# pswpswpsw/nif

Hardware: AMD Instinct MI355X
Metric: train-step points/sec (1D-wave, batch=1M per GPU) (higher is better)
Workload: dtype f32

## Files before the change

### nif_amd/csrc/k_nets.hip

```cpp
#include "nif_internal.h"
#include "k_pnet_bf16.h"


__global__ void k_pack(const float* __restrict__ theta, MatRef m, int NBI, int NBO, float* __restrict__ WF,
                       float* __restrict__ WB) {
  const long per_plane = (long)NBI * NBO * 1024;
  const long total = per_plane * (m.r + 1);
  for (long idx = (long)blockIdx.x * blockDim.x + threadIdx.x; idx < total; idx += (long)gridDim.x * blockDim.x) {
    const int k = (int)(idx / per_plane);
    long rem = idx - (long)k * per_plane;
    const int c = rem & 3;
    const int lane = (rem >> 2) & 63;
    const int vq = (rem >> 8) & 3;
    const int blk = (int)(rem >> 10);
    const int v = 4 * vq + c;
    {
      const int ob = blk / NBI, ib = blk % NBI;
      const int in = 32 * ib + fmap(v, lane >> 5), out = 32 * ob + (lane & 31);
      WF[idx] = (in < m.nin && out < m.nout) ? theta[matref_index(m, k, in, out)] : 0.f;
    }
    {
      const int ib = blk / NBO, ob = blk % NBO;
      const int in = 32 * ib + (lane & 31), out = 32 * ob + fmap(v, lane >> 5);
      WB[idx] = (in < m.nin && out < m.nout) ? theta[matref_index(m, k, in, out)] : 0.f;
    }
  }
}

void launch_pack(const float* theta, const MatRef& m, int NBI, int NBO, f32x4* WF, f32x4* WB, hipStream_t st) {
  const long total = (long)NBI * NBO * 1024 * (m.r + 1);
  int grid = (int)((total + 255) / 256);
  if (grid > 2048) grid = 2048;
  hipLaunchKernelGGL(k_pack, dim3(grid), dim3(256), 0, st, theta, m, NBI, NBO, (float*)WF, (float*)WB);
}

template <int NB>
__device__ __forceinline__ void pnet_first(const PNetArgs& A, long ptc, int hf, f32x16 (&h)[NB], f32x16 (&d)[NB]) {
  const float* prow = A.xin + ptc * A.ncol + A.col0;
#pragma unroll
  for (int b = 0; b < NB; ++b)
#pragma unroll
    for (int v = 0; v < 16; ++v) {
      const int f = 32 * b + fmap(v, hf);
      float a = 0.f;
      if (f < A.nst) {
        float acc = 0.f;
        for (int dd = 0; dd < A.pi; ++dd) acc = fmaf(prow[dd], A.theta[A.first_w + (long)dd * A.nst + f], acc);
        a = A.omega * acc + A.theta[A.first_b + f];
      }
      h[b][v] = a;
    }
  act_tile<NB>(A.act, h, h, d, A.nst, hf);
}

__host__ __device__ inline int pnet_plane_floats(const PNetArgs& A, int NB) {
  const int nm = A.lst * (A.res ? 2 : 1);
  return NB == 1 ? nm * PBF_FWD_U4 * 4 : ((NB == 2 && A.pbf2) ? nm * 4 * PBF_FWD_U4 * 4 : 0);
}
__host__ __device__ inline int pnet_tail_floats(const PNetArgs& A) { return A.r + (A.ll_kind ? A.r + A.r * A.r : 0); }

template <int NB, bool TRAIN, int ACT>
__global__ __launch_bounds__(256) void k_pnet(PNetArgs A) {
  const int lane = threadIdx.x & 63, wid = threadIdx.x >> 6;
  const int p = lane & 31, hf = lane >> 5;
  const long ntiles = (A.B + 31) / 32;
  const int nm = A.lst * (A.res ? 2 : 1);
  const long plane = (long)NB * NB * 256;
  extern __shared__ __attribute__((aligned(16))) float pn_lds[];
  float* zl_lds = pn_lds;
  float* tailv = pn_lds + (A.ll_kind ? 4 * A.r * 32 : 0) + ((psmall_floats(A, NB) + 3) & ~3) + pnet_plane_floats(A, NB);
  for (int e = threadIdx.x; e < A.r; e += 256) tailv[e] = A.theta[A.bott_b + e];
  if (A.ll_kind) {
    for (int e = threadIdx.x; e < A.r; e += 256) tailv[A.r + e] = A.theta[A.last_b + e];
    for (int e = threadIdx.x; e < A.r * A.r; e += 256) tailv[2 * A.r + e] = A.theta[A.last_w + e];
  }
  const PSmall S = psmall_stage<NB>(A, pn_lds + (A.ll_kind ? 4 * A.r * 32 : 0), threadIdx.x, 256);
  pbf16x8* bpl = reinterpret_cast<pbf16x8*>(pn_lds + (A.ll_kind ? 4 * A.r * 32 : 0) + ((psmall_floats(A, NB) + 3) & ~3));
  const bool bf2 = NB == 2 && A.pbf2;
  if constexpr (NB == 1) {
    for (int m = 0; m < nm; ++m) {
      const long w_off = A.res ? ((m & 1) ? A.hid_w2[m >> 1] : A.hid_w[m >> 1]) : A.hid_w[m];
      pbf_build(bpl + m * PBF_FWD_U4, nullptr, A.theta, w_off, A.nst, threadIdx.x, 256);
    }
  } else if constexpr (NB == 2) {
    if (bf2)
      for (int m = 0; m < nm; ++m) {
        const long w_off = A.res ? ((m & 1) ? A.hid_w2[m >> 1] : A.hid_w[m >> 1]) : A.hid_w[m];
        pbfn_build_fwd<2>(bpl + m * 4 * PBF_FWD_U4, A.theta, w_off, A.nst, threadIdx.x, 256);
      }
  }
  __syncthreads();
  for (long tile = (long)blockIdx.x * 4 + wid; tile < ntiles; tile += (long)gridDim.x * 4) {
  long pt = tile * 32 + p;
  const long ptc = pt < A.B ? pt : A.B - 1;

  f32x16 h[NB], d[NB], T[NB];
  {
    const float* prow = A.xin + ptc * A.ncol + A.col0;
#pragma unroll
    for (int b = 0; b < NB; ++b) {
      f32x16 acc;
#pragma unroll
      for (int v = 0; v < 16; ++v) acc[v] = 0.f;
      for (int dd = 0; dd < A.pi; ++dd) acc += prow[dd] * psmall_get(S.fw + dd * NB * 32, b, hf);
      h[b] = A.omega * acc + psmall_get(S.fb, b, hf);
    }
    act_tile_sel<NB, ACT>(A.act, h, h, d, A.nst, hf);
  }
  if (TRAIN) stash_store<NB>(A.stash + (long)(nm + 1) * A.slot_stride, tile, d, p, hf);

  for (int i = 0; i < A.lst; ++i) {
    if (!A.res) {
      if (TRAIN) stash_store<NB>(A.stash + (long)i * A.slot_stride, tile, h, p, hf);
      if constexpr (NB == 1) pbf_dense_fwd(bpl + i * PBF_FWD_U4, h[0], T[0], lane);
      else if (NB == 2 && bf2) pbfn_dense_fwd<NB>(bpl + i * (NB * NB * PBF_FWD_U4), h, T, lane);
      else dense_mfma<NB, NB>(A.WF + (long)i * plane, h, T, lane);
#pragma unroll
      for (int b = 0; b < NB; ++b) T[b] = A.omega * T[b] + psmall_get(S.hb + i * NB * 32, b, hf);
      act_tile_sel<NB, ACT>(A.act, T, T, d, A.nst, hf);
#pragma unroll
      for (int b = 0; b < NB; ++b) h[b] = A.siren ? T[b] : h[b] + T[b];
      if (TRAIN) stash_store<NB>(A.stash + (long)(nm + 2 + i) * A.slot_stride, tile, d, p, hf);
    } else {
      f32x16 t[NB];
      if (TRAIN) stash_store<NB>(A.stash + (long)(2 * i) * A.slot_stride, tile, h, p, hf);
      if constexpr (NB == 1) pbf_dense_fwd(bpl + (2 * i) * PBF_FWD_U4, h[0], T[0], lane);
      else if (NB == 2 && bf2) pbfn_dense_fwd<NB>(bpl + (2 * i) * (NB * NB * PBF_FWD_U4), h, T, lane);
      else dense_mfma<NB, NB>(A.WF + (long)(2 * i) * plane, h, T, lane);
#pragma unroll
      for (int b = 0; b < NB; ++b) T[b] = A.omega * T[b] + psmall_get(S.hb + i * NB * 32, b, hf);
      act_tile_sel<NB, ACT>(A.act, T, t, d, A.nst, hf);
      if (TRAIN) {
        stash_store<NB>(A.stash + (long)(nm + 2 + 2 * i) * A.slot_stride, tile, d, p, hf);
        stash_store<NB>(A.stash + (long)(2 * i + 1) * A.slot_stride, tile, t, p, hf);
      }
      if constexpr (NB == 1) pbf_dense_fwd(bpl + (2 * i + 1) * PBF_FWD_U4, t[0], T[0], lane);
      else if (NB == 2 && bf2) pbfn_dense_fwd<NB>(bpl + (2 * i + 1) * (NB * NB * PBF_FWD_U4), t, T, lane);
      else dense_mfma<NB, NB>(A.WF + (long)(2 * i + 1) * plane, t, T, lane);
#pragma unroll
      for (int b = 0; b < NB; ++b) {
        const f32x16 lin = A.omega * T[b] + psmall_get(S.hb2 + i * NB * 32, b, hf);
        T[b] = A.siren ? lin : h[b] + lin;
      }
      act_tile_sel<NB, ACT>(A.act, T, T, d, A.nst, hf);
#pragma unroll
      for (int b = 0; b < NB; ++b) h[b] = A.siren ? 0.5f * (h[b] + T[b]) : T[b];
      if (TRAIN) stash_store<NB>(A.stash + (long)(nm + 2 + 2 * i + 1) * A.slot_stride, tile, d, p, hf);
    }
  }
  if (TRAIN) stash_store<NB>(A.stash + (long)nm * A.slot_stride, tile, h, p, hf);
  float* zl = zl_lds + (long)wid * A.r * 32;
  for (int c = 0; c < A.r; ++c) {
    float s = 0.f;
#pragma unroll
    for (int b = 0; b < NB; ++b) {
      const f32x16 w = psmall_get(S.bw + c * NB * 32, b, hf);
#pragma unroll
      for (int v = 0; v < 16; ++v) s = fmaf(h[b][v], w[v], s);
    }
    s += __shfl_xor(s, 32);
    s += tailv[c];
    if (A.ll_kind) {
      if (hf == 0) { zl[c * 32 + p] = s; A.ZL[(tile * A.zl_rows + c) * 32 + p] = s; }
    } else if (hf == 0) {
      A.Z[(tile * A.r + c) * 32 + p] = s;
    }
  }
  if (A.ll_kind) {
    const float* lw = tailv + 2 * A.r;
    for (int c = hf; c < A.r; c += 2) {
      float s = tailv[A.r + c];
#pragma unroll 4
      for (int kk = 0; kk < A.r; ++kk) s = fmaf(zl[kk * 32 + p], lw[kk * A.r + c], s);
      A.Z[(tile * A.r + c) * 32 + p] = s;
    }
  }
  }
}

template <int NB>
__global__ __launch_bounds__(256) void k_pnet_bwd(PNetArgs A) {
  const int lane = threadIdx.x & 63, wid = threadIdx.x >> 6;
  const int p = lane & 31, hf = lane >> 5;
  const long ntiles = (A.B + 31) / 32;
  const long tile = (long)blockIdx.x * 4 + wid;
  if (tile >= ntiles) return;
  const int nm = A.lst * (A.res ? 2 : 1);
  const long plane = (long)NB * NB * 256;

  f32x16 gh[NB], d[NB], ga[NB], U[NB];
#pragma unroll
  for (int b = 0; b < NB; ++b)
#pragma unroll
    for (int v = 0; v < 16; ++v) gh[b][v] = 0.f;
  for (int c = 0; c < A.r; ++c) {
    const float dz = A.DZ[(tile * A.r + c) * 32 + p];
#pragma unroll
    for (int b = 0; b < NB; ++b)
#pragma unroll
      for (int v = 0; v < 16; ++v) {
        const int f = 32 * b + fmap(v, hf);
        if (f < A.nst) gh[b][v] = fmaf(dz, A.theta[A.bott_w + (long)f * A.r + c], gh[b][v]);
      }
  }
  for (int i = A.lst - 1; i >= 0; --i) {
    if (!A.res) {
      float* da = A.stash + (long)(nm + 2 + i) * A.slot_stride;
      stash_load<NB>(da, tile, d, p, hf);
#pragma unroll
      for (int b = 0; b < NB; ++b) ga[b] = gh[b] * d[b];
      stash_store<NB>(da, tile, ga, p, hf);
      dense_mfma<NB, NB>(A.WB + (long)i * plane, ga, U, lane);
#pragma unroll
      for (int b = 0; b < NB; ++b) gh[b] = A.siren ? A.omega * U[b] : gh[b] + A.omega * U[b];
    } else {
      float* da2 = A.stash + (long)(nm + 2 + 2 * i + 1) * A.slot_stride;
      float* da1 = A.stash + (long)(nm + 2 + 2 * i) * A.slot_stride;
      stash_load<NB>(da2, tile, d, p, hf);
      const float half = A.siren ? 0.5f : 1.0f;
#pragma unroll
      for (int b = 0; b < NB; ++b) ga[b] = half * gh[b] * d[b];
      stash_store<NB>(da2, tile, ga, p, hf);
      dense_mfma<NB, NB>(A.WB + (long)(2 * i + 1) * plane, ga, U, lane);
      f32x16 skip[NB];
#pragma unroll
      for (int b = 0; b < NB; ++b) skip[b] = A.siren ? 0.5f * gh[b] : ga[b];
      stash_load<NB>(da1, tile, d, p, hf);
#pragma unroll
      for (int b = 0; b < NB; ++b) ga[b] = A.omega * U[b] * d[b];
      stash_store<NB>(da1, tile, ga, p, hf);
      dense_mfma<NB, NB>(A.WB + (long)(2 * i) * plane, ga, U, lane);
#pragma unroll
      for (int b = 0; b < NB; ++b) gh[b] = skip[b] + A.omega * U[b];
    }
  }
  float* da0 = A.stash + (long)(nm + 1) * A.slot_stride;
  stash_load<NB>(da0, tile, d, p, hf);
#pragma unroll
  for (int b = 0; b < NB; ++b) ga[b] = gh[b] * d[b];
  stash_store<NB>(da0, tile, ga, p, hf);
}

void launch_pnet(const PNetArgs& a_, int NSTB, bool train, hipStream_t st) {
  PNetArgs a = a_;
  const long ntiles = (a.B + 31) / 32;
  long nblk = (ntiles + 3) / 4;
  static const long cap = [] { const char* e = getenv("NIF_PNET_BLOCKS"); return e ? atol(e) : 2048L; }();
  if (nblk > cap) nblk = cap;
  const int nmat = a.lst * (a.res ? 2 : 1);
  const size_t shm0 = ((a.ll_kind ? (size_t)4 * a.r * 32 : 0) + (size_t)((psmall_floats(a, NSTB) + 3) & ~3)) * sizeof(float);
  static const bool bf2_on = [] { const char* e = getenv("NIF_PNET_BF2"); return !(e && e[0] == '0'); }();
  const size_t tailb = (size_t)pnet_tail_floats(a) * sizeof(float);
  a.pbf2 = (NSTB == 2 && bf2_on && shm0 + tailb + (size_t)nmat * 4 * PBF_FWD_U4 * 16 <= 64u * 1024u) ? 1 : 0;
  if (a.pbf2 && nblk > 512) nblk = 512;
  dim3 grid((unsigned)nblk), block(256);
  const size_t shm = shm0 + (size_t)pnet_plane_floats(a, NSTB) * sizeof(float) + tailb;
#define PNL(NB_, TR_, ACT_)                                                                                             \
  {                                                                                                                     \
    if (shm > 48 * 1024)                                                                                                \
      (void)hipFuncSetAttribute((const void*)k_pnet<NB_, TR_, ACT_>, hipFuncAttributeMaxDynamicSharedMemorySize, (int)shm); \
    hipLaunchKernelGGL((k_pnet<NB_, TR_, ACT_>), grid, block, shm, st, a);                                              \
  }
#define PNA(NB_, TR_)                              \
  if (a.act == ACT_SWISH) PNL(NB_, TR_, ACT_SWISH) \
  else if (a.act == ACT_SINE) PNL(NB_, TR_, ACT_SINE) \
  else PNL(NB_, TR_, -1)
#define PN(NB_) \
  if (train) { PNA(NB_, true) } else { PNA(NB_, false) }
  if (NSTB == 1) { PN(1) } else if (NSTB == 2) { PN(2) } else { PN(4) }
#undef PN
#undef PNA
#undef PNL
}
void launch_pnet_bwd(const PNetArgs& a, int NSTB, hipStream_t st) {
  const long ntiles = (a.B + 31) / 32;
  dim3 grid((unsigned)((ntiles + 3) / 4)), block(256);
  if (NSTB == 1) hipLaunchKernelGGL((k_pnet_bwd<1>), grid, block, 0, st, a);
  else if (NSTB == 2) hipLaunchKernelGGL((k_pnet_bwd<2>), grid, block, 0, st, a);
  else hipLaunchKernelGGL((k_pnet_bwd<4>), grid, block, 0, st, a);
}

__device__ __forceinline__ float hyp(const SNetArgs& A, int k, long slot) {
  return k < A.r ? A.theta[A.off_Wh + (long)k * A.po + slot] : A.theta[A.off_bh + slot];
}

template <int NB, bool TRAIN, int ACT>
__global__ __launch_bounds__(256, (NB <= 2 ? 2 : 1)) void k_snet(SNetArgs A) {
  extern __shared__ float smem[];
  const int lane = threadIdx.x & 63, wid = threadIdx.x >> 6;
  const int p = lane & 31, hf = lane >> 5;
  const long ntiles = (A.B + 31) / 32;
  const long tile = (long)blockIdx.x * 4 + wid;
  const bool active = tile < ntiles;
  float loss_lane = 0.f;
  float* dzs = smem + (long)wid * (2 * A.r * 64);
  float* sks = dzs + A.r * 64;
  float* lsum = smem + 4L * (2 * A.r * 64);

  if (active) {
    const long pt = tile * 32 + p;
    const bool valid = pt < A.B;
    const long ptc = valid ? pt : A.B - 1;
    const long plane = (long)NB * NB * 256;
    const int n = A.n, r = A.r;
    const float* xrow = A.xin + ptc * A.ncol + A.col0;
    const float* zt_base = A.Z + tile * r * 32 + p;
    float* IN0 = A.stash;
    float* DA0 = A.stash + (long)(A.nh + 1) * A.slot_stride;
    if (TRAIN)
      for (int k = 0; k < r; ++k) dzs[k * 64 + lane] = 0.f;

    f32x16 h[NB], d[NB], acc[NB], T[NB], ublk[NB];
#pragma unroll
    for (int b = 0; b < NB; ++b)
#pragma unroll
      for (int v = 0; v < 16; ++v) acc[b][v] = 0.f;
    for (int k = 0; k <= r; ++k) {
      const float zt = k < r ? zt_base[k * 32] : 1.0f;
#pragma unroll
      for (int b = 0; b < NB; ++b)
#pragma unroll
        for (int v = 0; v < 16; ++v) {
          const int f = 32 * b + fmap(v, hf);
          if (f < n) {
            float s = 0.f;
            for (int dd = 0; dd < A.si; ++dd) s = fmaf(xrow[dd], hyp(A, k, slot_w1(A) + (long)dd * n + f), s);
            acc[b][v] = fmaf(zt, fmaf(A.omega, s, hyp(A, k, slot_b1(A) + f)), acc[b][v]);
          }
        }
    }
    act_tile_sel<NB, ACT>(A.act, acc, h, d, n, hf);
    if (TRAIN) stash_store<NB>(DA0, tile, d, p, hf);

    for (int j = 0; j < A.nh; ++j) {
      if (TRAIN) stash_store<NB>(IN0 + (long)j * A.slot_stride, tile, h, p, hf);
#pragma unroll
      for (int b = 0; b < NB; ++b)
#pragma unroll
        for (int v = 0; v < 16; ++v) acc[b][v] = 0.f;
      for (int k = 0; k <= r; ++k) {
        const float zt = k < r ? zt_base[k * 32] : 1.0f;
        dense_mfma<NB, NB>(A.WF + ((long)j * (r + 1) + k) * plane, h, T, lane);
#pragma unroll
        for (int b = 0; b < NB; ++b)
#pragma unroll
          for (int v = 0; v < 16; ++v) {
            const int f = 32 * b + fmap(v, hf);
            const float hb = f < n ? hyp(A, k, slot_bh(A, j) + f) : 0.f;
            acc[b][v] = fmaf(zt, fmaf(A.omega, T[b][v], hb), acc[b][v]);
          }
      }
      const bool res_first = A.res && !(j & 1);
      const bool res_second = A.res && (j & 1);
      if (res_first) {
#pragma unroll
        for (int b = 0; b < NB; ++b) ublk[b] = h[b];
      }
      act_tile_sel<NB, ACT>(A.act, acc, T, d, n, hf);
#pragma unroll
      for (int b = 0; b < NB; ++b) {
        f32x16 hn = T[b];
        if (A.nif_skip) hn += h[b];
        if (res_second) hn = 0.5f * (ublk[b] + hn);
        h[b] = hn;
      }
      if (TRAIN) stash_store<NB>(DA0 + (long)(j + 1) * A.slot_stride, tile, d, p, hf);
    }

    if (TRAIN) stash_store<NB>(IN0 + (long)A.nh * A.slot_stride, tile, h, p, hf);
    f32x16 gh[NB];
#pragma unroll
    for (int b = 0; b < NB; ++b)
#pragma unroll
      for (int v = 0; v < 16; ++v) gh[b][v] = 0.f;
    const float wsamp = (valid ? (A.sw ? A.sw[ptc] : 1.0f) : 0.0f);
    float se = 0.f;
    for (int o = 0; o < A.so; ++o) {
      f32x16 wg[NB];
#pragma unroll
      for (int b = 0; b < NB; ++b)
#pragma unroll
        for (int v = 0; v < 16; ++v) wg[b][v] = 0.f;
      float part = 0.f, bias = 0.f;
      for (int k = 0; k <= r; ++k) {
        const float zt = k < r ? zt_base[k * 32] : 1.0f;
        float sk = 0.f;
#pragma unroll
        for (int b = 0; b < NB; ++b)
#pragma unroll
          for (int v = 0; v < 16; ++v) {
            const int f = 32 * b + fmap(v, hf);
            const float w = f < n ? hyp(A, k, slot_wl(A) + (long)f * A.so + o) : 0.f;
            sk = fmaf(h[b][v], w, sk);
            wg[b][v] = fmaf(zt, w, wg[b][v]);
          }
        part = fmaf(zt, sk, part);
        bias = fmaf(zt, hyp(A, k, slot_bl(A) + o), bias);
        if (TRAIN && k < r) sks[k * 64 + lane] = sk;
      }
      part += __shfl_xor(part, 32);
      const float uo = part + bias;
      if (valid && hf == 0 && A.u_out) A.u_out[pt * A.so + o] = uo;
      if (TRAIN) {
        const float e = uo - A.y[ptc * A.so + o];
        NIF_LOSS_ACC(A.loss_kind, e, se, dfac)
        const float du = dfac * wsamp * A.inv_bg / (float)A.so;
        if (hf == 0) A.DU[(tile * A.so + o) * 32 + p] = du;
#pragma unroll
        for (int b = 0; b < NB; ++b) gh[b] += du * wg[b];
        for (int k = 0; k < r; ++k) {
          float t = du * sks[k * 64 + lane];
          if (hf == 0) t = fmaf(du, A.theta[A.off_Wh + (long)k * A.po + slot_bl(A) + o], t);
          dzs[k * 64 + lane] += t;
        }
// ... 95 lines not shown
```

### nif_amd/csrc/k_pnetbw.hip

```cpp
#include "nif_internal.h"
#include "k_pnet_bf16.h"

struct PbwArgs {
  PNetArgs p;
  float* partial; long pstride;
  const float* touch; long touch_floats;
};

__device__ __forceinline__ f32x4 lds4(const float* q) { return *reinterpret_cast<const f32x4*>(q); }

__device__ __forceinline__ int pswz(int f, int p) { return f * 32 + ((((p >> 2) ^ (f & 7))) << 2) + (p & 3); }
__device__ __forceinline__ int pswz4(int f, int c) { return f * 32 + ((c ^ (f & 7)) << 2); }
__device__ __forceinline__ void tile_store(float* __restrict__ t, const f32x16& h, int p, int hf) {
#pragma unroll
  for (int v = 0; v < 16; ++v) t[pswz(fmap(v, hf), p)] = h[v];
}

typedef __bf16 pbw_bf16x8 __attribute__((ext_vector_type(8)));
__device__ __forceinline__ void grad_mfma(const float* IN, const float* DA, f32x16& C, int i, int hf, int in_rows = 32) {
  f32x4 a[4], b[4];
#pragma unroll
  for (int q = 0; q < 4; ++q) {
    a[q] = lds4(IN + pswz4(i < in_rows ? i : 0, 4 * hf + q));
    if (i >= in_rows) { a[q][0] = 0.f; a[q][1] = 0.f; a[q][2] = 0.f; a[q][3] = 0.f; }
    b[q] = lds4(DA + pswz4(i, 4 * hf + q));
  }
#pragma unroll
  for (int hh = 0; hh < 2; ++hh) {
    pbw_bf16x8 ah, al, bh, bl;
#pragma unroll
    for (int e = 0; e < 8; ++e) {
      const float x = a[2 * hh + (e >> 2)][e & 3], y = b[2 * hh + (e >> 2)][e & 3];
      const __bf16 x0 = (__bf16)x, y0 = (__bf16)y;
      ah[e] = x0; al[e] = (__bf16)(x - (float)x0);
      bh[e] = y0; bl[e] = (__bf16)(y - (float)y0);
    }
    C = __builtin_amdgcn_mfma_f32_32x32x16_bf16(ah, bl, C, 0, 0, 0);
    C = __builtin_amdgcn_mfma_f32_32x32x16_bf16(al, bh, C, 0, 0, 0);
    C = __builtin_amdgcn_mfma_f32_32x32x16_bf16(ah, bh, C, 0, 0, 0);
  }
}
__device__ __forceinline__ float col_sum(const float* DA, int i, int hf) {
  float s = 0.f;
#pragma unroll
  for (int q = 0; q < 4; ++q) { const f32x4 b = lds4(DA + pswz4(i, 4 * hf + q)); s += (b[0] + b[1]) + (b[2] + b[3]); }
  return s;
}

#ifndef NIF_PBW_DZR
#define NIF_PBW_DZR 8
#endif
#ifndef NIF_PBW_WAVES
#define NIF_PBW_WAVES 8
#endif
template <int NM, bool RES, int ACT, bool SMALL>
__global__ __launch_bounds__(64 * NIF_PBW_WAVES) void k_pnet_bwg(PbwArgs G) {
  const PNetArgs& A = G.p;
  extern __shared__ __attribute__((aligned(16))) float lds[];
  constexpr int WV = NIF_PBW_WAVES;
  __shared__ float red[(WV - 1) * 64];
  const int lane = threadIdx.x & 63, wid = threadIdx.x >> 6;
  const int p = lane & 31, hf = lane >> 5, i = p;
  const long ntiles = (A.B + 31) / 32;
  constexpr int WLDS = (NM + 2) * 1024 + 256;
  float* hs = lds + (long)wid * WLDS;
  float* gaT = hs + (NM + 1) * 1024;
  float* xT = gaT + 1024;

  f32x16 C[NM], C1, Cb, CB1;
  float gbh[NM], gb0 = 0.f, gbb = 0.f;
#pragma unroll
  for (int e = 0; e < 16; ++e) { C1[e] = 0.f; Cb[e] = 0.f; CB1[e] = 0.f; }
#pragma unroll
  for (int m = 0; m < NM; ++m) {
    gbh[m] = 0.f;
#pragma unroll
    for (int e = 0; e < 16; ++e) C[m][e] = 0.f;
  }
  for (int q = lane; q < 256; q += 64) xT[q] = 0.f;
  const PSmall S = psmall_stage<1>(A, lds + (long)WV * WLDS, threadIdx.x, 64 * WV);
  f32x4* wpl = reinterpret_cast<f32x4*>(lds + (long)WV * WLDS + ((psmall_floats(A, 1) + 3) & ~3));
  pbf16x8* bpl = reinterpret_cast<pbf16x8*>(wpl);
#pragma unroll
  for (int m = 0; m < NM; ++m) {
    const long w_off = RES ? (m == 0 ? A.hid_w[0] : A.hid_w2[0]) : A.hid_w[m];
    pbf_build(bpl + m * (PBF_FWD_U4 + PBF_BWD_U4), bpl + m * (PBF_FWD_U4 + PBF_BWD_U4) + PBF_FWD_U4, A.theta, w_off, A.nst,
              threadIdx.x, 64 * WV);
  }
  auto dense_f = [&](int m, const f32x16 (&x)[1], f32x16 (&y)[1]) { pbf_dense_fwd(bpl + m * (PBF_FWD_U4 + PBF_BWD_U4), x[0], y[0], lane); };
  auto dense_b = [&](int m, const f32x16 (&x)[1], f32x16 (&y)[1]) { pbf_dense_bwd(bpl + m * (PBF_FWD_U4 + PBF_BWD_U4) + PBF_FWD_U4, x[0], y[0], lane); };
  __syncthreads();

  for (long tile = (long)blockIdx.x * WV + wid; tile < ntiles; tile += (long)gridDim.x * WV) {
    const long pt = tile * 32 + p;
    const long ptc = pt < A.B ? pt : A.B - 1;
    const float* prow = A.xin + ptc * A.ncol + A.col0;
    float dzr[NIF_PBW_DZR];
    if (!SMALL) {
      const float* dzg = A.DZ + tile * A.r * 32;
      const int nd = A.r * 32;
#pragma unroll
      for (int q = 0; q < NIF_PBW_DZR; ++q) { const int e = lane + 64 * q; dzr[q] = e < nd ? dzg[e] : 0.f; }
    }
    f32x16 h[1], T[1], d[NM + 1][1];
    {
      f32x16 acc;
#pragma unroll
      for (int v = 0; v < 16; ++v) acc[v] = 0.f;
      for (int dd = 0; dd < A.pi; ++dd) acc += prow[dd] * psmall_get(S.fw + dd * 32, 0, hf);
      h[0] = A.omega * acc + psmall_get(S.fb, 0, hf);
    }
    act_tile_sel<1, ACT>(A.act, h, h, d[0], A.nst, hf);
    float* park = hs + NM * 1024;
    if (SMALL) {
#pragma unroll
      for (int v = 0; v < 16; ++v) park[v * 64 + lane] = d[0][0][v];
    }
    if (!SMALL && hf == 0) {
      for (int dd = 0; dd < A.pi; ++dd) xT[pswz(dd, p)] = prow[dd];
      xT[pswz(A.pi, p)] = 1.0f;
    }
    if (!RES) {
#pragma unroll
      for (int m = 0; m < NM; ++m) {
        tile_store(hs + m * 1024, h[0], p, hf);
        dense_f(m, h, T);
        T[0] = A.omega * T[0] + psmall_get(S.hb + m * 32, 0, hf);
        act_tile_sel<1, ACT>(A.act, T, T, d[m + 1], A.nst, hf);
        h[0] = A.siren ? T[0] : h[0] + T[0];
      }
    } else {
      f32x16 t[1];
      tile_store(hs, h[0], p, hf);
      dense_f(0, h, T);
      T[0] = A.omega * T[0] + psmall_get(S.hb, 0, hf);
      act_tile_sel<1, ACT>(A.act, T, t, d[1], A.nst, hf);
      tile_store(hs + 1024, t[0], p, hf);
      dense_f(1, t, T);
      {
        const f32x16 lin = A.omega * T[0] + psmall_get(S.hb2, 0, hf);
        T[0] = A.siren ? lin : h[0] + lin;
      }
      act_tile_sel<1, ACT>(A.act, T, T, d[NM], A.nst, hf);
      h[0] = A.siren ? 0.5f * (h[0] + T[0]) : T[0];
    }
    if (!SMALL) tile_store(hs + NM * 1024, h[0], p, hf);
    f32x16 gh[1], ga[1], U[1];
#pragma unroll
    for (int v = 0; v < 16; ++v) gh[0][v] = 0.f;
    if (!SMALL) {
#pragma unroll
      for (int q = 0; q < NIF_PBW_DZR; ++q) gaT[pswz(2 * q + hf, p)] = dzr[q];
#pragma unroll
      for (int q = NIF_PBW_DZR; q < 16; ++q) {
        const int e = lane + 64 * q;
        gaT[pswz(2 * q + hf, p)] = e < A.r * 32 ? A.DZ[tile * A.r * 32 + e] : 0.f;
      }
      for (int c = 0; c < A.r; ++c) gh[0] += gaT[pswz(c, p)] * psmall_get(S.bw + c * 32, 0, hf);
    } else {
      gh[0] += A.DZ[tile * 32 + p] * psmall_get(S.bw, 0, hf);
    }
    if (SMALL) {
      const float dz = A.DZ[tile * 32 + p];
      Cb += dz * h[0];
      gbb += hf == 0 ? dz : 0.f;
    } else {
      grad_mfma(hs + NM * 1024, gaT, Cb, i, hf);
      gbb += col_sum(gaT, i, hf);
    }
    float tv[4] = {0.f, 0.f, 0.f, 0.f};
    if (G.touch) {
      const float* tb = G.touch + tile * G.touch_floats + lane * 16;
#pragma unroll
      for (int q = 0; q < 4; ++q) tv[q] = tb[q * 1024 < G.touch_floats ? q * 1024 : 0];
    }
    if (!RES) {
#pragma unroll
      for (int m = NM - 1; m >= 0; --m) {
        ga[0] = gh[0] * d[m + 1][0];
        tile_store(gaT, ga[0], p, hf);
        grad_mfma(hs + m * 1024, gaT, C[m], i, hf);
        gbh[m] += col_sum(gaT, i, hf);
        dense_b(m, ga, U);
        gh[0] = A.siren ? A.omega * U[0] : gh[0] + A.omega * U[0];
      }
    } else {
      const float half = A.siren ? 0.5f : 1.0f;
      ga[0] = half * gh[0] * d[NM][0];
      tile_store(gaT, ga[0], p, hf);
      grad_mfma(hs + 1024, gaT, C[NM - 1], i, hf);
      gbh[NM - 1] += col_sum(gaT, i, hf);
      dense_b(1, ga, U);
      f32x16 skip;
      skip = A.siren ? 0.5f * gh[0] : ga[0];
      ga[0] = A.omega * U[0] * d[1][0];
      tile_store(gaT, ga[0], p, hf);
      grad_mfma(hs, gaT, C[0], i, hf);
      gbh[0] += col_sum(gaT, i, hf);
      dense_b(0, ga, U);
      gh[0] = skip + A.omega * U[0];
    }
    if (SMALL) {
#pragma unroll
      for (int v = 0; v < 16; ++v) ga[0][v] = gh[0][v] * park[v * 64 + lane];
    } else {
      ga[0] = gh[0] * d[0][0];
    }
    if (SMALL) {
      C1 += prow[0] * ga[0];
      CB1 += ga[0];
    } else {
      tile_store(gaT, ga[0], p, hf);
      grad_mfma(xT, gaT, C1, i, hf, 8);
    }
    asm volatile("" ::"v"(tv[0]), "v"(tv[1]), "v"(tv[2]), "v"(tv[3]));
  }

  float* prow_out = G.partial + (long)blockIdx.x * G.pstride;
  auto sum8 = [&](float v) -> float {
    if (wid > 0) red[(wid - 1) * 64 + lane] = v;
    __syncthreads();
    if (wid == 0) {
#pragma unroll
      for (int w = 0; w < WV - 1; ++w) v += red[w * 64 + lane];
    }
    __syncthreads();
    return v;
  };
  __syncthreads();
  auto sum16 = [&](f32x16 v) -> f32x16 {
    if (wid > 0) {
#pragma unroll
      for (int e = 0; e < 16; ++e) lds[((wid - 1) * 16 + e) * 64 + lane] = v[e];
    }
    __syncthreads();
    if (wid == 0) {
#pragma unroll
      for (int w = 0; w < WV - 1; ++w)
#pragma unroll
        for (int e = 0; e < 16; ++e) v[e] += lds[(w * 16 + e) * 64 + lane];
    }
    __syncthreads();
    return v;
  };
#pragma unroll
  for (int m = 0; m < NM; ++m) {
    const long w_off = RES ? (m == 0 ? A.hid_w[0] : A.hid_w2[0]) : A.hid_w[m];
    const long b_off = RES ? (m == 0 ? A.hid_b[0] : A.hid_b2[0]) : A.hid_b[m];
    {
      const f32x16 vs = sum16(C[m]);
#pragma unroll
      for (int e = 0; e < 16; ++e) {
        const int in = fmap(e, hf), out = i;
        if (wid == 0 && in < A.nst && out < A.nst) prow_out[w_off + (long)in * A.nst + out] = A.omega * vs[e];
      }
    }
    float vb = gbh[m];
    vb += __shfl_xor(vb, 32);
    vb = sum8(vb);
    if (wid == 0 && hf == 0 && i < A.nst) prow_out[b_off + i] = vb;
  }
  if (SMALL) {
    auto lanes32 = [&](f32x16 v) -> f32x16 {
#pragma unroll
      for (int off = 16; off > 0; off >>= 1)
#pragma unroll
        for (int e = 0; e < 16; ++e) v[e] += __shfl_xor(v[e], off);
      return v;
    };
    const f32x16 s1 = sum16(lanes32(C1)), s0 = sum16(lanes32(CB1)), sb = sum16(lanes32(Cb));
#pragma unroll
    for (int e = 0; e < 16; ++e) {
      const int f = fmap(e, hf);
      if (wid == 0 && p == 0 && f < A.nst) {
        prow_out[A.first_w + f] = A.omega * s1[e];
        prow_out[A.first_b + f] = s0[e];
        prow_out[A.bott_w + f] = sb[e];
      }
    }
    float v = gbb;
#pragma unroll
    for (int off = 32; off > 0; off >>= 1) v += __shfl_xor(v, off);
    v = sum8(v);
    if (wid == 0 && lane == 0) prow_out[A.bott_b] = v;
    return;
  }
  const f32x16 s1 = sum16(C1), sb = sum16(Cb);
#pragma unroll
  for (int e = 0; e < 16; ++e) {
    const float v1 = s1[e];
    const float vb = sb[e];
    const int row = fmap(e, hf);
    if (wid == 0) {
      if (row < A.pi && i < A.nst) prow_out[A.first_w + (long)row * A.nst + i] = A.omega * v1;
      if (row == A.pi && i < A.nst) prow_out[A.first_b + i] = v1;
      if (row < A.nst && i < A.r) prow_out[A.bott_w + (long)row * A.r + i] = vb;
    }
  }
  (void)gb0;
  {
    float v = gbb;
    v += __shfl_xor(v, 32);
    v = sum8(v);
    if (wid == 0 && hf == 0 && i < A.r) prow_out[A.bott_b + i] = v;
  }
}

bool pnet_bwg_supported(const PNetArgs& a) {
  const int nm = a.lst * (a.res ? 2 : 1);
  return a.nst <= 32 && a.pi <= 6 && a.r <= 32 && nm >= 1 && nm <= 2 && (!a.res || a.lst == 1);
}

void launch_pnet_bwg(const PNetArgs& a, float* partial, long pstride, int rows, hipStream_t st, const float* touch,
                     long touch_floats) {
  PbwArgs G; G.p = a; G.partial = partial; G.pstride = pstride; G.touch = touch; G.touch_floats = touch_floats;
  const int nm = a.lst * (a.res ? 2 : 1);
  dim3 grid(rows), block(64 * NIF_PBW_WAVES);
  const size_t shm = ((size_t)NIF_PBW_WAVES * ((nm + 2) * 1024 + 256) + (size_t)((psmall_floats(a, 1) + 3) & ~3) +
                      (size_t)nm * 2560) * sizeof(float);
#define PBW1(NM_, RES_, ACT_, SM_)                                                                                  \
  {                                                                                                                 \
    (void)hipFuncSetAttribute((const void*)k_pnet_bwg<NM_, RES_, ACT_, SM_>, hipFuncAttributeMaxDynamicSharedMemorySize, (int)shm); \
    hipLaunchKernelGGL((k_pnet_bwg<NM_, RES_, ACT_, SM_>), grid, block, shm, st, G);                                \
  }
#define PBW(NM_, RES_, ACT_)                                                                                        \
  {                                                                                                                 \
    if (a.pi == 1 && a.r == 1) PBW1(NM_, RES_, ACT_, true) else PBW1(NM_, RES_, ACT_, false)                        \
  }
#define PBWA(NM_, RES_)                                                       \
  if (a.act == ACT_SWISH) PBW(NM_, RES_, ACT_SWISH)                           \
  else if (a.act == ACT_SINE) PBW(NM_, RES_, ACT_SINE)                        \
  else PBW(NM_, RES_, -1)
  if (a.res) { PBWA(2, true) }
  else if (nm == 1) { PBWA(1, false) }
  else { PBWA(2, false) }
#undef PBWA
#undef PBW
#undef PBW1
}
```

### nif_amd/csrc/k_snet4.hip

```cpp
#include "k_snet4_dev.h"

__global__ void k_pack16b(const float* __restrict__ theta, MatRef m, long mstride, int NBL, __bf16* __restrict__ WF,
                          __bf16* __restrict__ WB, long fstride, long bstride, float scale, int mode, const float* __restrict__ pscale) {
  m.base_k += (long)blockIdx.y * mstride; m.base_last += (long)blockIdx.y * mstride;
  WF += (long)blockIdx.y * fstride; WB += (long)blockIdx.y * bstride;
  const int NCH = NBL / 2;
  const int nsf = mode == 3 ? 2 : (mode ? 1 : 3), nsb = (mode == 1 || mode == 2) ? 1 : 2;
  const long fwd_plane = (long)NCH * NBL * nsf * 64 * 8, bwd_plane = (long)NCH * NBL * nsb * 64 * 8;
  const long total_f = fwd_plane * (m.r + 1), total_b = bwd_plane * (m.r + 1);
  for (long idx = (long)blockIdx.x * blockDim.x + threadIdx.x; idx < total_f + total_b; idx += (long)gridDim.x * blockDim.x) {
    const bool fwd = idx < total_f;
    const long e = fwd ? idx : idx - total_f;
    const int ns = fwd ? nsf : nsb;
    const long per_plane = fwd ? fwd_plane : bwd_plane;
    const int k = (int)(e / per_plane);
    long rem = e - (long)k * per_plane;
    const int t = rem & 7; rem >>= 3;
    const int lane = rem & 63; rem >>= 6;
    const int s = (int)(rem % ns); rem /= ns;
    const int blk = (int)(rem % NBL);
    const int ks = (int)(rem / NBL);
    const int slot = 16 * (2 * ks + (t >> 2)) + 4 * (lane >> 4) + (t & 3);
    const int row = 16 * blk + (lane & 15);
    const int in = fwd ? slot : row, out = fwd ? row : slot;
    float x = (in < m.nin && out < m.nout) ? scale * theta[matref_index(m, k, in, out)] : 0.f;
    if (mode == 3) {
      x *= pscale[(blockIdx.y * (m.r + 1) + k) * 2];
      const _Float16 h0 = (_Float16)__builtin_amdgcn_fmed3f(x, -65504.0f, 65504.0f);
      const _Float16 h1 = (_Float16)(x - (float)h0);
      reinterpret_cast<_Float16*>(fwd ? WF : WB)[e] = s == 0 ? h0 : h1;
      continue;
    }
    if (mode == 2) {
      reinterpret_cast<_Float16*>(fwd ? WF : WB)[e] = (_Float16)__builtin_amdgcn_fmed3f(x, -65504.0f, 65504.0f);
      continue;
    }
    const __bf16 x0 = (__bf16)x;
    const float r1 = x - (float)x0;
    const __bf16 x1 = (__bf16)r1;
    const __bf16 x2 = (__bf16)(r1 - (float)x1);
    (fwd ? WF : WB)[e] = s == 0 ? x0 : (s == 1 ? x1 : x2);
  }
}
__global__ void k_plane_scales(const float* __restrict__ theta, MatRef m, long mstride, float scale, float* __restrict__ pscale) {
  m.base_k += (long)blockIdx.y * mstride; m.base_last += (long)blockIdx.y * mstride;
  const int k = blockIdx.x;
  float mx = 0.f;
  for (int idx = threadIdx.x; idx < m.nin * m.nout; idx += blockDim.x) {
    const int in = idx / m.nout, out = idx - in * m.nout;
    mx = fmaxf(mx, fabsf(scale * theta[matref_index(m, k, in, out)]));
  }
  __shared__ float red[256];
  red[threadIdx.x] = mx;
  __syncthreads();
  for (int o = 128; o > 0; o >>= 1) {
    if ((int)threadIdx.x < o) red[threadIdx.x] = fmaxf(red[threadIdx.x], red[threadIdx.x + o]);
    __syncthreads();
  }
  if (threadIdx.x == 0) {
    mx = red[0];
    int ex = 0;
    if (mx > 0.f && mx < 3.0e38f) (void)frexpf(mx, &ex); else ex = 14;
    int sh = 14 - ex;
    sh = sh > 60 ? 60 : (sh < -60 ? -60 : sh);
    pscale[(blockIdx.y * (m.r + 1) + k) * 2] = ldexpf(1.0f, sh);
    pscale[(blockIdx.y * (m.r + 1) + k) * 2 + 1] = ldexpf(1.0f, -sh);
  }
}
__global__ __launch_bounds__(256) void k_pack16b_dual(const float* __restrict__ theta, MatRef m, long mstride, int NBL,
                                                     __bf16* __restrict__ WF, __bf16* __restrict__ WB, long fstride, long bstride,
                                                     _Float16* __restrict__ WFx, _Float16* __restrict__ WBx, long fxstride, long bxstride,
                                                     float scale, float* __restrict__ pscale) {
  m.base_k += (long)blockIdx.y * mstride; m.base_last += (long)blockIdx.y * mstride;
  WF += (long)blockIdx.y * fstride; WB += (long)blockIdx.y * bstride;
  WFx += (long)blockIdx.y * fxstride; WBx += (long)blockIdx.y * bxstride;
  const int NCH = NBL / 2;
  const long fwd0 = (long)NCH * NBL * 3 * 64 * 8, bwd0 = (long)NCH * NBL * 2 * 64 * 8, px = bwd0;
  const long tot0 = (fwd0 + bwd0) * (m.r + 1), totx = 2 * px * (m.r + 1);
  __shared__ float red[256];
  int k_have = -1;
  float s_have = 1.0f;
  for (long idx = (long)blockIdx.x * blockDim.x + threadIdx.x; idx < tot0 + totx; idx += (long)gridDim.x * blockDim.x) {
    const bool half = idx >= tot0;
    const long i2 = half ? idx - tot0 : idx;
    const long tf = half ? px * (m.r + 1) : fwd0 * (m.r + 1);
    const bool fwd = i2 < tf;
    const long e = fwd ? i2 : i2 - tf;
    const int ns = half ? 2 : (fwd ? 3 : 2);
    const long per_plane = half ? px : (fwd ? fwd0 : bwd0);
    const int k = (int)(e / per_plane);
    long rem = e - (long)k * per_plane;
    const int t = rem & 7; rem >>= 3;
    const int lane = rem & 63; rem >>= 6;
    const int s = (int)(rem % ns); rem /= ns;
    const int blk = (int)(rem % NBL);
    const int ks = (int)(rem / NBL);
    const int slot = 16 * (2 * ks + (t >> 2)) + 4 * (lane >> 4) + (t & 3);
    const int row = 16 * blk + (lane & 15);
    const int in = fwd ? slot : row, out = fwd ? row : slot;
    float x = (in < m.nin && out < m.nout) ? scale * theta[matref_index(m, k, in, out)] : 0.f;
    if (half) {
      if (k != k_have) {
        float mx = 0.f;
        for (int q = threadIdx.x; q < m.nin * m.nout; q += 256) {
          const int qi = q / m.nout, qo = q - qi * m.nout;
          mx = fmaxf(mx, fabsf(scale * theta[matref_index(m, k, qi, qo)]));
        }
        __syncthreads();
        red[threadIdx.x] = mx;
        __syncthreads();
        for (int o = 128; o > 0; o >>= 1) {
          if ((int)threadIdx.x < o) red[threadIdx.x] = fmaxf(red[threadIdx.x], red[threadIdx.x + o]);
          __syncthreads();
        }
        mx = red[0];
        int ex = 0;
        if (mx > 0.f && mx < 3.0e38f) (void)frexpf(mx, &ex); else ex = 14;
        int sh = 14 - ex;
        sh = sh > 60 ? 60 : (sh < -60 ? -60 : sh);
        s_have = ldexpf(1.0f, sh); k_have = k;
        if (fwd && e == (long)k * per_plane && pscale) {
          pscale[(blockIdx.y * (m.r + 1) + k) * 2] = s_have;
          pscale[(blockIdx.y * (m.r + 1) + k) * 2 + 1] = ldexpf(1.0f, -sh);
        }
      }
      x *= s_have;
      const _Float16 h0 = (_Float16)__builtin_amdgcn_fmed3f(x, -65504.0f, 65504.0f);
      const _Float16 h1 = (_Float16)(x - (float)h0);
      (fwd ? WFx : WBx)[e] = s == 0 ? h0 : h1;
      continue;
    }
    const __bf16 x0 = (__bf16)x;
    const float r1 = x - (float)x0;
    const __bf16 x1 = (__bf16)r1;
    const __bf16 x2 = (__bf16)(r1 - (float)x1);
    (fwd ? WF : WB)[e] = s == 0 ? x0 : (s == 1 ? x1 : x2);
  }
}
void launch_pack16b_dual(const float* theta, const MatRef& m0, long mstride, int nmat, int NBL, void* WF, void* WB, long fstride_elems,
                         long bstride_elems, void* WFx, void* WBx, long fxstride_elems, long bxstride_elems, float scale, float* pscale,
                         hipStream_t st) {
  const long total = (long)(NBL / 2) * NBL * (5 + 4) * 64 * 8 * (m0.r + 1);
  int grid = (int)((total + 255) / 256);
  if (grid > 4096) grid = 4096;
  hipLaunchKernelGGL(k_pack16b_dual, dim3(grid, nmat), dim3(256), 0, st, theta, m0, mstride, NBL, (__bf16*)WF, (__bf16*)WB, fstride_elems,
                     bstride_elems, (_Float16*)WFx, (_Float16*)WBx, fxstride_elems, bxstride_elems, scale, pscale);
}
void launch_pack16b(const float* theta, const MatRef& m, int NBL, void* WF, void* WB, float scale, hipStream_t st, int mode) {
  launch_pack16b_batch(theta, m, 0, 1, NBL, WF, WB, 0, 0, scale, st, mode);
}
void launch_pack16b_batch(const float* theta, const MatRef& m0, long mstride, int nmat, int NBL, void* WF, void* WB,
                          long fstride_elems, long bstride_elems, float scale, hipStream_t st, int mode, float* pscale) {
  const long total = (long)(NBL / 2) * NBL * 5 * 64 * 8 * (m0.r + 1);
  int grid = (int)((total + 255) / 256);
  if (grid > 4096) grid = 4096;
  if (mode == 3) hipLaunchKernelGGL(k_plane_scales, dim3(m0.r + 1, nmat), dim3(256), 0, st, theta, m0, mstride, scale, pscale);
  hipLaunchKernelGGL(k_pack16b, dim3(grid, nmat), dim3(256), 0, st, theta, m0, mstride, NBL, (__bf16*)WF, (__bf16*)WB,
                     fstride_elems, bstride_elems, scale, mode, pscale);
}

__global__ void k_pack_phi(const float* __restrict__ theta, long w_off, int n, int sop, int NBL, __bf16* __restrict__ WPF,
                           __bf16* __restrict__ WPB) {
  const int NCH = NBL / 2;
  const long total_f = (long)NCH * 2 * 3 * 64 * 8, total_b = (long)NBL * 2 * 64 * 8;
  for (long idx = (long)blockIdx.x * blockDim.x + threadIdx.x; idx < total_f + total_b; idx += (long)gridDim.x * blockDim.x) {
    const bool fwd = idx < total_f;
    long rem = fwd ? idx : idx - total_f;
    const int t = rem & 7; rem >>= 3;
    const int lane = rem & 63; rem >>= 6;
    const int ns = fwd ? 3 : 2;
    const int sp = (int)(rem % ns); rem /= ns;
    int in, out;
    if (fwd) {
      const int ob = (int)(rem % 2), ks = (int)(rem / 2);
      in = 16 * (2 * ks + (t >> 2)) + 4 * (lane >> 4) + (t & 3);
      out = 16 * ob + (lane & 15);
    } else {
      const int ib = (int)rem;
      in = 16 * ib + (lane & 15);
      out = 16 * (t >> 2) + 4 * (lane >> 4) + (t & 3);
    }
    const float x = (in < n && out < sop) ? theta[w_off + (long)in * sop + out] : 0.f;
    const __bf16 x0 = (__bf16)x;
    const float r1 = x - (float)x0;
    const __bf16 x1 = (__bf16)r1;
    const __bf16 x2 = (__bf16)(r1 - (float)x1);
    (fwd ? WPF : WPB)[fwd ? idx : idx - total_f] = sp == 0 ? x0 : (sp == 1 ? x1 : x2);
  }
}
long snet4_phi_fwd_elems(int n) { return (long)(snet3_nbl(n) / 2) * 2 * 3 * 64 * 8; }
long snet4_phi_bwd_elems(int n) { return (long)snet3_nbl(n) * 2 * 64 * 8; }
void launch_pack_phi(const float* theta, long w_off, int n, int sop, void* WPF, void* WPB, hipStream_t st) {
  hipLaunchKernelGGL(k_pack_phi, dim3(64), dim3(256), 0, st, theta, w_off, n, sop, snet3_nbl(n), (__bf16*)WPF, (__bf16*)WPB);
}

int snet4_nsm_ll(int si, int sop, int nh, int n, int sou, int rl) {
  return snet3_nsm(si, sop, nh, n) + ((sou + 3) & ~3) + ((rl * rl + 3) & ~3);
}
__global__ void k_ll_slots(const float* __restrict__ theta, LLSlotMap m, float* __restrict__ slots) {
  for (int sgi = blockIdx.y; sgi < m.nseg; sgi += gridDim.y)
    for (long e = (long)blockIdx.x * blockDim.x + threadIdx.x; e < m.seg[sgi].len; e += (long)gridDim.x * blockDim.x)
      slots[m.seg[sgi].dst + e] = theta[m.seg[sgi].src + e];
}
void launch_ll_slots(const float* theta, const LLSlotMap& m, float* slots, hipStream_t st) {
  hipLaunchKernelGGL(k_ll_slots, dim3(16, m.nseg), dim3(256), 0, st, theta, m, slots);
}
bool snet4_supported(const SNetArgs& a) {
  const int NBL = snet3_nbl(a.n);
  if (a.n > 128 || (NBL & 1) || a.nh < 1) return false;
  if (a.ll && a.so > 32) return false;
  return snet4_shmem(a, NBL) <= 160u * 1024u;
}
long snet4_fwd_elems(int n, int r) { const int NBL = snet3_nbl(n); return (long)(NBL / 2) * NBL * 3 * 64 * 8 * (r + 1); }
long snet4_bwd_elems(int n, int r) { const int NBL = snet3_nbl(n); return (long)(NBL / 2) * NBL * 2 * 64 * 8 * (r + 1); }

bool snet4_sign_ring(const SNetArgs& a) { return !a.nif_skip; }
bool snet4_writes_da_bf16(const SNetArgs& a) { return a.da_bf16 != 0 && a.prec == 1 && snet3_nbl(a.n) != 6; }
bool snet4_writes_h_ph16(const SNetArgs& a) { return a.h_ph16 != 0 && a.prec == 1 && snet3_nbl(a.n) == 8 && !a.res && !a.nif_skip; }
int launch_snet4(const SNetArgs& a, bool train, bool query_only, hipStream_t st) {
  const int NBL = snet3_nbl(a.n);
  const long nt16 = 2 * ((a.B + 31) / 32);
  const long ngroups = (nt16 + 3) / 4;
  long cap = NBL <= 4 ? 256 * NIF_S4_OCC : 256 * NIF_S4_OCC_WIDE;
  if (NBL == 8 && a.ll && train && !a.res) cap = 256 * NIF_S4_OCC_LL8;
  if (a.wg_cap > 0 && a.wg_cap < cap) cap = a.wg_cap;
  const int nblk = (int)(ngroups < cap ? ngroups : cap);
  if (query_only) return nblk;
  dim3 grid(nblk), block(256);
  const size_t shm = snet4_shmem(a, NBL);
  SNetArgs h = a;
  const int pr = snet4_pr(a);
  if (a.prec != 0) { h.WF4 = a.WF4h; h.WB4 = a.WB4h; }
  if (pr == 2) {
    launch_snet4_f16(h, train, nblk, shm, st);
    return nblk;
  }
  if (pr == 3) {
    h.WF4 = a.WF4x; h.WB4 = a.WB4x;
    launch_snet4_x16(h, train, nblk, shm, st);
    return nblk;
  }
#define S4L(NBL_, TR_, ACT_, MODE_, SGN_, LL_, PR_)                                                                    \
  {                                                                                                                 \
    if (shm > 48 * 1024)                                                                                            \
      (void)hipFuncSetAttribute((const void*)k_snet4<NBL_, TR_, ACT_, MODE_, SGN_, LL_, PR_>,                            \
                                hipFuncAttributeMaxDynamicSharedMemorySize, (int)shm);                              \
    hipLaunchKernelGGL((k_snet4<NBL_, TR_, ACT_, MODE_, SGN_, LL_, PR_>), grid, block, shm, st, h);                      \
  }
#define S4M(NBL_, LL_, PR_)                                                                                         \
  if (a.nif_skip) { if (train) S4L(NBL_, true, -1, 2, false, LL_, PR_) else S4L(NBL_, false, -1, 2, false, LL_, PR_) }    \
  else if (a.res) { if (train) S4L(NBL_, true, ACT_SINE, 1, true, LL_, PR_) else S4L(NBL_, false, ACT_SINE, 1, false, LL_, PR_) } \
  else if (train) S4L(NBL_, true, ACT_SINE, 0, true, LL_, PR_)                                                      \
  else S4L(NBL_, false, ACT_SINE, 0, false, LL_, PR_)
#define S4N(NBL_, LL_, PR_)                                                 \
  if (a.res) { if (train) S4L(NBL_, true, ACT_SINE, 1, true, LL_, PR_) else S4L(NBL_, false, ACT_SINE, 1, false, LL_, PR_) } \
  else if (train) S4L(NBL_, true, ACT_SINE, 0, true, LL_, PR_)                                                      \
  else S4L(NBL_, false, ACT_SINE, 0, false, LL_, PR_)
#define S4(NBL_)                                                            \
  if (a.ll && a.prec == 1) { S4N(NBL_, true, true) }                        \
  else if (a.prec == 1) { S4M(NBL_, false, true) }                          \
  else if (a.nif_skip) { if (train) S4L(NBL_, true, -1, 2, false, false, false) else S4L(NBL_, false, -1, 2, false, false, false) } \
  else return -1;
#ifdef NIF_S4_DEV
  if (train) S4L(4, true, ACT_SINE, 0, true, false, false) else S4L(4, false, ACT_SINE, 0, false, false, false)
#else
  switch (NBL) {
    case 2: S4(2) break;
    case 4: S4(4) break;
    case 6: S4(6) break;
    default: S4(8) break;
  }
#endif
#undef S4
#undef S4N
#undef S4M
#undef S4L
  return nblk;
}
```

### nif_amd/csrc/nif_api.hip

```cpp
#include "../../include/nif_hip.h"
#include "nif_internal.h"
#include <cstdlib>

#include <cmath>
#include <cstdio>
#include <cstring>
#include <memory>
#include <string>
#include <vector>

#include "nif_ctx.h"

#define NIF_ACT_SLABS 32
static inline bool act_on(const nif_ctx* c) { return c->act_l1 != 0.f || c->act_l2 != 0.f; }
struct RegsOff {
  nif_ctx* c; float jac_l1, act_l1, act_l2;
  RegsOff(nif_ctx* c_, bool on) : c(on ? c_ : nullptr) {
    if (!c) return;
    jac_l1 = c->jac_l1; act_l1 = c->act_l1; act_l2 = c->act_l2;
    c->jac_l1 = 0.f; c->act_l1 = 0.f; c->act_l2 = 0.f;
  }
  ~RegsOff() { if (c) { c->jac_l1 = jac_l1; c->act_l1 = act_l1; c->act_l2 = act_l2; } }
  RegsOff(const RegsOff&) = delete;
  RegsOff& operator=(const RegsOff&) = delete;
};
static int jac_reg_pass(nif_ctx* c, const float* xin, long B, long Bg, const int* mu_blk = nullptr);
struct SobPlan { int ns, nsc; int seeds[3]; int par[3]; int gcol[3]; bool any_par;
                 int gstride, nx_all, ny, no_primal; unsigned ymask;
                 int hess; };
static int sob_par_pass(nif_ctx* c, const float* xin, long B, long Bg, const SobPlan& sp, const SNetArgs& sa);
static int fill_snet_ll_sob(nif_ctx* c, SNetArgs& sa, const float* xin, long B, bool f32_planes = false);

#ifndef NIF_PIPE_CHUNK_DEFAULT
#define NIF_PIPE_CHUNK_DEFAULT 131072L
#endif

static thread_local std::string g_err;
int nif_fail(int code, const std::string& msg) { g_err = msg; return code; }

extern "C" const char* nif_last_error(void) { return g_err.c_str(); }
extern "C" int nif_abi_version(void) { return NIF_ABI_VERSION; }
extern "C" int nif_device_count(void) {
  int n = 0;
  if (hipGetDeviceCount(&n) != hipSuccess) return 0;
  return n;
}

static void add_desc(nif_ctx* c, const char* name, long& off, int rows, int cols) {
  nif_tensor_desc d;
  memset(&d, 0, sizeof(d));
  snprintf(d.name, sizeof(d.name), "%s", name);
  d.offset = off; d.rows = rows; d.cols = cols;
  c->layout.push_back(d);
  off += (long)rows * (cols ? cols : 1);
}

static int build_layout(nif_ctx* c) {
  long off = 0;
  char nm[48];
  c->first_w = off; add_desc(c, "pnet_first_w", off, c->pi, c->nst);
  c->first_b = off; add_desc(c, "pnet_first_b", off, c->nst, 0);
  for (int i = 0; i < c->lst; ++i) {
    snprintf(nm, sizeof(nm), "pnet_h%d_w", i); c->hid_w[i] = off; add_desc(c, nm, off, c->nst, c->nst);
    snprintf(nm, sizeof(nm), "pnet_h%d_b", i); c->hid_b[i] = off; add_desc(c, nm, off, c->nst, 0);
    if (c->cfg.p_resblock) {
      snprintf(nm, sizeof(nm), "pnet_h%d_w2", i); c->hid_w2[i] = off; add_desc(c, nm, off, c->nst, c->nst);
      snprintf(nm, sizeof(nm), "pnet_h%d_b2", i); c->hid_b2[i] = off; add_desc(c, nm, off, c->nst, 0);
    }
  }
  c->bott_w = off; add_desc(c, "pnet_bottleneck_w", off, c->nst, c->r);
  c->bott_b = off; add_desc(c, "pnet_bottleneck_b", off, c->r, 0);
  c->last_w = off; add_desc(c, "pnet_last_w", off, c->r, (int)c->po);
  c->last_b = off; add_desc(c, "pnet_last_b", off, (int)c->po, 0);
  if (c->kind == NIF_KIND_LASTLAYER) {
    const int nout = (int)c->po * c->so;
    c->s_first_w = off; add_desc(c, "snet_first_w", off, c->si, c->n);
    c->s_first_b = off; add_desc(c, "snet_first_b", off, c->n, 0);
    for (int i = 0; i < c->L; ++i) {
      snprintf(nm, sizeof(nm), "snet_h%d_w", i); c->s_hid_w[i] = off; add_desc(c, nm, off, c->n, c->n);
      snprintf(nm, sizeof(nm), "snet_h%d_b", i); c->s_hid_b[i] = off; add_desc(c, nm, off, c->n, 0);
      if (c->cfg.s_resblock) {
        snprintf(nm, sizeof(nm), "snet_h%d_w2", i); c->s_hid_w2[i] = off; add_desc(c, nm, off, c->n, c->n);
        snprintf(nm, sizeof(nm), "snet_h%d_b2", i); c->s_hid_b2[i] = off; add_desc(c, nm, off, c->n, 0);
      }
    }
    c->s_bott_w = off; add_desc(c, "snet_bottleneck_w", off, c->n, nout);
    c->s_bott_b = off; add_desc(c, "snet_bottleneck_b", off, nout, 0);
    c->ll_bias = off; add_desc(c, "last_layer_bias", off, c->so, 0);
  }
  c->P = off;
  return 0;
}

static int create_buffers(nif_ctx* c) {
  const int nh = c->nh, nm = c->nm;
  HIPCHK(hipSetDevice(c->dev));
  HIPCHK(hipStreamCreateWithFlags(&c->st, hipStreamNonBlocking));
  const long pn = c->P + 2;
  for (DevBuf<float>* b : {&c->theta, &c->grad, &c->m, &c->v}) { const int rc = b->alloc(pn); if (rc) return rc; }
  for (float* b : {c->m.p, c->v.p, c->grad.p}) HIPCHK(hipMemset(b, 0, sizeof(float) * (size_t)pn));
  int rc = NIF_OK;
  const long pk_p = (long)(nm > 0 ? nm : 1) * c->NSTB * c->NSTB * 256;
  long pk_s = (long)(nh > 0 ? nh : 1) * (c->r + 1) * c->NB * c->NB * 256;
  {
    const long pk16 = (long)(nh > 0 ? nh : 1) * (c->r + 1) * snet3_plane_floats(c->n) / 4;
    if (pk16 > pk_s) pk_s = pk16;
  }
  if (!rc) rc = c->pWF.alloc(pk_p);
  if (!rc) rc = c->pWB.alloc(pk_p);
  if (!rc) rc = c->sWF.alloc(pk_s);
  if (!rc) rc = c->sWB.alloc(pk_s);
  if (nh > 0 && !(snet3_nbl(c->n) & 1) && c->n <= 128) {
    const int rr = c->kind == NIF_KIND_LASTLAYER ? 0 : c->r;
    if (!rc) rc = c->sWF4.alloc((long)nh * snet4_fwd_elems(c->n, rr) * 2);
    if (!rc) rc = c->sWB4.alloc((long)nh * snet4_bwd_elems(c->n, rr) * 2);
    if (c->kind != NIF_KIND_NIF) {
      if (!rc) rc = c->sWF4x.alloc((long)nh * snet4_bwd_elems(c->n, rr) * 2);
      if (!rc) rc = c->sWB4x.alloc((long)nh * snet4_bwd_elems(c->n, rr) * 2);
      if (!rc) rc = c->sWscale.alloc((long)nh * (rr + 1) * 2);
    }
    if (c->cfg.mixed_policy != NIF_POLICY_FLOAT32) {
      if (!rc) rc = c->sWF4h.alloc((long)nh * (snet4_fwd_elems(c->n, rr) / 3) * 2);
      if (!rc) rc = c->sWB4h.alloc((long)nh * (snet4_bwd_elems(c->n, rr) / 2) * 2);
    }
    if (c->kind == NIF_KIND_LASTLAYER && !rc) rc = c->ll_wpf.alloc((long)snet4_phi_fwd_elems(c->n) * 2);
    if (c->kind == NIF_KIND_LASTLAYER && !rc) rc = c->ll_wpb.alloc((long)snet4_phi_bwd_elems(c->n) * 2);
  }
  if (c->kind == NIF_KIND_LASTLAYER && nh > 0 && c->n <= 128 && !rc)
    rc = c->ll_slots.alloc((long)c->si * c->n + (long)nh * c->n * c->n + (long)c->n * c->so * c->r +
                           c->n + (long)nh * c->n + c->so * c->r + c->so + c->r * c->r + 64);
  const long pk_l = (long)(nh > 0 ? nh : 1) * c->NB * c->NB * 256;
  if (!rc && c->kind == NIF_KIND_LASTLAYER) rc = c->lWF.alloc(pk_l);
  if (!rc && c->kind == NIF_KIND_LASTLAYER) rc = c->lWB.alloc(pk_l);
  return rc;
}

extern "C" int nif_create(const nif_cfg* cfg, int device_id, nif_ctx** out) {
  if (!cfg || !out) return fail(NIF_ERR_INVALID, "null argument");
  if (cfg->abi_version != NIF_ABI_VERSION) return fail(NIF_ERR_INVALID, "abi_version mismatch");
  int ndev = 0;
  if (hipGetDeviceCount(&ndev) != hipSuccess || ndev <= 0)
    return fail(NIF_ERR_NODEVICE, "no HIP device visible: libnif_hip has no CPU fallback");
  if (device_id < 0 || device_id >= ndev) return fail(NIF_ERR_INVALID, "device_id out of range");
  hipDeviceProp_t prop;
  HIPCHK(hipGetDeviceProperties(&prop, device_id));
  if (strncmp(prop.gcnArchName, "gfx950", 6) != 0)
    return fail(NIF_ERR_NODEVICE, std::string("device is ") + prop.gcnArchName + ", libnif_hip is built for gfx950 only");
  if (cfg->kind != NIF_KIND_NIF && cfg->kind != NIF_KIND_MULTISCALE && cfg->kind != NIF_KIND_LASTLAYER)
    return fail(NIF_ERR_INVALID, "unknown model kind");
  if (cfg->mixed_policy != NIF_POLICY_FLOAT32 && cfg->mixed_policy != NIF_POLICY_MIXED_BF16 && cfg->mixed_policy != NIF_POLICY_MIXED_F16)
    return fail(NIF_ERR_INVALID, "unknown mixed_policy");
  for (int i = 0; i < 7; ++i) if (cfg->reserved[i] != 0) return fail(NIF_ERR_INVALID, "reserved fields must be zero");
  if (cfg->p_act < 0 || cfg->p_act > NIF_ACT_HARD_SIGMOID || cfg->s_act < 0 || cfg->s_act > NIF_ACT_HARD_SIGMOID)
    return fail(NIF_ERR_INVALID, "unknown activation id (nif_act)");
  if (cfg->kind == NIF_KIND_LASTLAYER && cfg->latent_dim * cfg->so_dim > 64)
    return fail(NIF_ERR_INVALID, "last-layer class: latent_dim * output_dim must be <= 64");
  if (cfg->pi_dim < 1 || cfg->si_dim < 1 || cfg->so_dim < 1 || cfg->latent_dim < 1)
    return fail(NIF_ERR_INVALID, "dims must be >= 1");
  if (cfg->n_sx < 1 || cfg->n_sx > 128 || cfg->n_st < 1 || cfg->n_st > 128)
    return fail(NIF_ERR_INVALID, "units must be in [1,128]");
  if (cfg->latent_dim > 64) return fail(NIF_ERR_INVALID, "latent_dim must be <= 64");
  if (cfg->pi_dim > 16 || cfg->si_dim > 16 || cfg->so_dim > 16)
    return fail(NIF_ERR_INVALID, "input/output dims must be <= 16");
  const int nh = cfg->l_sx * (cfg->s_resblock ? 2 : 1);
  const int nm = cfg->l_st * (cfg->p_resblock ? 2 : 1);
  if (cfg->l_sx < 0 || nh > NIF_MAX_HID || cfg->l_st < 0 || cfg->l_st > NIF_MAX_HID)
    return fail(NIF_ERR_INVALID, "too many layers");
  if (cfg->kind == NIF_KIND_NIF && (cfg->s_resblock || cfg->p_resblock || cfg->p_act == NIF_ACT_SINE))
    return fail(NIF_ERR_INVALID, "class NIF has no resblock / sine ParameterNet");
  if (cfg->p_resblock && cfg->kind == NIF_KIND_NIF) return fail(NIF_ERR_INVALID, "bad cfg");

  std::unique_ptr<nif_ctx> own(new nif_ctx());
  nif_ctx* c = own.get();
  c->cfg = *cfg;
  { const char* e = getenv("NIF_FP32_MFMA"); c->opt_fp32_mfma = e && e[0] == '1'; }
  { const char* e = getenv("NIF_FUSE_GW"); c->opt_fuse_gw = !(e && e[0] == '0'); }
  { const char* e = getenv("NIF_SMALL_STEP"); c->opt_small_step = !(e && e[0] == '0'); }
  { const char* e = getenv("NIF_FUSE_TAIL"); c->opt_fuse_tail = !(e && e[0] == '0'); }
  { const char* e = getenv("NIF_PIPE_CHUNK"); if (e && e[0]) c->opt_pipe_chunk = atol(e); }
  { const char* e = getenv("NIF_SIDE_PNET"); if (e && e[0]) c->opt_side_pnet = e[0] != '0'; }
  { const char* e = getenv("NIF_PIPE_WGS"); if (e && e[0]) c->opt_pipe_wgs = atoi(e); }
  c->dev = device_id;
  c->kind = cfg->kind; c->pi = cfg->pi_dim; c->si = cfg->si_dim; c->so = cfg->so_dim;
  c->n = cfg->n_sx; c->L = cfg->l_sx; c->nst = cfg->n_st; c->lst = cfg->l_st; c->r = cfg->latent_dim;
  c->nh = nh; c->nm = nm;
  c->NB = c->n <= 32 ? 1 : (c->n <= 64 ? 2 : 4);
  c->NSTB = c->nst <= 32 ? 1 : (c->nst <= 64 ? 2 : 4);
  c->po = (long)nh * c->n * c->n + (long)(c->si + c->so + 1 + nh) * c->n + c->so;
  if (c->kind == NIF_KIND_LASTLAYER) c->po = c->r;
  c->RB = (c->r + 31) / 32;
  build_layout(c);
  c->pstride = (c->P + 1 + 63) / 64 * 64;
  if (create_buffers(c) != NIF_OK) return fail(NIF_ERR_HIP, "nif_create: " + g_err);
  *out = own.release();
  return NIF_OK;
}

nif_ctx::~nif_ctx() {
  (void)hipSetDevice(dev);
  nif_f64_release(this);
  if (comm) (void)nif_comm_destroy(this);
  for (hipStream_t s : {st2, st_copy, st}) if (s) { (void)hipStreamSynchronize(s); (void)hipStreamDestroy(s); }
  for (hipEvent_t e : {ev_copied[0], ev_copied[1], ev_consumed[0], ev_consumed[1], ev_start, ev_done, t0, t1}) if (e) (void)hipEventDestroy(e);
  for (hipEvent_t e : ev_chunk) (void)hipEventDestroy(e);
  for (hipEvent_t e : ev_pool) (void)hipEventDestroy(e);
  for (const Rec& r : recs) { (void)hipEventDestroy(r.a); (void)hipEventDestroy(r.b); }
  for (hipGraphExec_t ex : graphs) if (ex) (void)hipGraphExecDestroy(ex);
}
extern "C" int nif_destroy(nif_ctx* c) {
  if (!c) return NIF_OK;
  hipSetDevice(c->dev);
  if (c->st) hipStreamSynchronize(c->st);
  delete c;
  return NIF_OK;
}

extern "C" int nif_param_count(nif_ctx* c, int64_t* n) { if (!c || !n) return fail(NIF_ERR_INVALID, "null"); *n = c->P; return NIF_OK; }
extern "C" int nif_po_dim(nif_ctx* c, int64_t* po) { if (!c || !po) return fail(NIF_ERR_INVALID, "null"); *po = c->po; return NIF_OK; }
extern "C" int nif_param_layout(nif_ctx* c, nif_tensor_desc* descs, int32_t* n_inout) {
  if (!c || !n_inout) return fail(NIF_ERR_INVALID, "null");
  const int need = (int)c->layout.size();
  if (!descs || *n_inout < need) { *n_inout = need; return descs ? fail(NIF_ERR_INVALID, "descs too small") : NIF_OK; }
  memcpy(descs, c->layout.data(), sizeof(nif_tensor_desc) * need);
  *n_inout = need;
  return NIF_OK;
}

extern "C" int nif_set_params(nif_ctx* c, const float* host, int64_t n) {
  if (!c || !host) return fail(NIF_ERR_INVALID, "null");
  if (n != c->P) return fail(NIF_ERR_INVALID, "parameter count mismatch");
  HIPCHK(hipSetDevice(c->dev));
  TAIL_FLUSH(c)
  HIPCHK(hipMemcpyAsync(c->theta, host, sizeof(float) * n, hipMemcpyHostToDevice, c->st));
  HIPCHK(hipStreamSynchronize(c->st));
  c->have_params = true; c->packed = false; c->packed32 = false; c->packed_p32 = false;
  return NIF_OK;
}
extern "C" int nif_get_params(nif_ctx* c, float* host, int64_t n) {
  if (!c || !host) return fail(NIF_ERR_INVALID, "null");
  if (n != c->P) return fail(NIF_ERR_INVALID, "parameter count mismatch");
  HIPCHK(hipSetDevice(c->dev));
  TAIL_FLUSH(c)
  HIPCHK(hipMemcpyAsync(host, c->theta, sizeof(float) * n, hipMemcpyDeviceToHost, c->st));
  HIPCHK(hipStreamSynchronize(c->st));
  return NIF_OK;
}
extern "C" int nif_get_opt_state(nif_ctx* c, float* mh, float* vh, int64_t n, int64_t* step) {
  if (!c || !mh || !vh || !step) return fail(NIF_ERR_INVALID, "null");
  if (n != c->P) return fail(NIF_ERR_INVALID, "parameter count mismatch");
  HIPCHK(hipSetDevice(c->dev));
  TAIL_FLUSH(c)
  HIPCHK(hipMemcpyAsync(mh, c->m, sizeof(float) * n, hipMemcpyDeviceToHost, c->st));
  HIPCHK(hipMemcpyAsync(vh, c->v, sizeof(float) * n, hipMemcpyDeviceToHost, c->st));
  HIPCHK(hipStreamSynchronize(c->st));
  *step = c->step;
  return NIF_OK;
}
extern "C" int nif_set_opt_state(nif_ctx* c, const float* mh, const float* vh, int64_t n, int64_t step) {
  if (!c || !mh || !vh) return fail(NIF_ERR_INVALID, "null");
  if (n != c->P) return fail(NIF_ERR_INVALID, "parameter count mismatch");
  HIPCHK(hipSetDevice(c->dev));
  TAIL_FLUSH(c)
  HIPCHK(hipMemcpyAsync(c->m, mh, sizeof(float) * n, hipMemcpyHostToDevice, c->st));
  HIPCHK(hipMemcpyAsync(c->v, vh, sizeof(float) * n, hipMemcpyHostToDevice, c->st));
  HIPCHK(hipStreamSynchronize(c->st));
  c->step = step;
  c->slots_fresh = step == 0;
  for (int64_t i = 0; i < n && c->slots_fresh; ++i) c->slots_fresh = mh[i] == 0.f && vh[i] == 0.f;
  return NIF_OK;
}

extern "C" int nif_dev_alloc(nif_ctx* c, int64_t bytes, void** dptr) {
  if (!c || !dptr || bytes < 0) return fail(NIF_ERR_INVALID, "bad argument");
  HIPCHK(hipSetDevice(c->dev));
  TAIL_FLUSH(c)
  HIPCHK(hipMalloc(dptr, bytes > 0 ? (size_t)bytes : 4));
  return NIF_OK;
}
extern "C" int nif_dev_free(nif_ctx* c, void* dptr) {
  if (!c) return fail(NIF_ERR_INVALID, "null");
  HIPCHK(hipSetDevice(c->dev));
  TAIL_FLUSH(c)
  HIPCHK(hipStreamSynchronize(c->st));
  if (dptr) HIPCHK(hipFree(dptr));
  return NIF_OK;
}
extern "C" int nif_h2d(nif_ctx* c, void* dst, const void* src, int64_t bytes) {
  if (!c || !dst || !src) return fail(NIF_ERR_INVALID, "null");
  HIPCHK(hipSetDevice(c->dev));
  TAIL_FLUSH(c)
  HIPCHK(hipMemcpyAsync(dst, src, (size_t)bytes, hipMemcpyHostToDevice, c->st));
  HIPCHK(hipStreamSynchronize(c->st));
  return NIF_OK;
}
extern "C" int nif_d2h(nif_ctx* c, void* dst, const void* src, int64_t bytes) {
  if (!c || !dst || !src) return fail(NIF_ERR_INVALID, "null");
  HIPCHK(hipSetDevice(c->dev));
  TAIL_FLUSH(c)
  HIPCHK(hipMemcpyAsync(dst, src, (size_t)bytes, hipMemcpyDeviceToHost, c->st));
  HIPCHK(hipStreamSynchronize(c->st));
  return NIF_OK;
}
extern "C" int nif_sync(nif_ctx* c) {
  if (!c) return fail(NIF_ERR_INVALID, "null");
  HIPCHK(hipSetDevice(c->dev));
  TAIL_FLUSH(c)
  HIPCHK(hipStreamSynchronize(c->st));
  return NIF_OK;
}
extern "C" int nif_host_alloc(nif_ctx* c, int64_t bytes, void** hptr) {
  if (!c || !hptr || bytes < 0) return fail(NIF_ERR_INVALID, "bad argument");
  HIPCHK(hipSetDevice(c->dev));
  TAIL_FLUSH(c)
  HIPCHK(hipHostMalloc(hptr, bytes > 0 ? (size_t)bytes : 4, hipHostMallocDefault));
  return NIF_OK;
}
extern "C" int nif_host_free(nif_ctx* c, void* hptr) {
  if (!c) return fail(NIF_ERR_INVALID, "null");
  HIPCHK(hipSetDevice(c->dev));
  TAIL_FLUSH(c)
  if (c->st_copy) HIPCHK(hipStreamSynchronize(c->st_copy));
  if (hptr) HIPCHK(hipHostFree(hptr));
  return NIF_OK;
}
static int ensure_copy_stream(nif_ctx* c) {
  if (c->st_copy) return NIF_OK;
  HIPCHK(hipStreamCreateWithFlags(&c->st_copy, hipStreamNonBlocking));
  for (int s = 0; s < 2; ++s) {
    HIPCHK(hipEventCreateWithFlags(&c->ev_copied[s], hipEventDisableTiming));
// ... 63 lines not shown
    DevBuf<float>* ws[] = {&c->Z, &c->DZ, &c->DU, &c->ZL, &c->PHI, &c->DPHI, &c->DA, &c->DZL};
    const long wsz[] = {(long)c->r * newcap, (long)c->r * newcap, (long)c->so * newcap, (long)32 * c->RB * newcap,
                        (long)c->r * c->so * newcap, (long)c->r * c->so * newcap, (long)c->r * newcap, (long)c->r * newcap};
    int rc = NIF_OK;
    for (int i = 0; i < (ll ? 8 : 4) && !rc; ++i) rc = ws[i]->reserve(c, wsz[i]);
    if (!rc && newcap > c->cap) { rc = c->stash_s.release(c); if (!rc) rc = c->stash_p.release(c); }
    if (!rc && train) {
      c->slot_s = (long)c->NB * 32 * newcap;
      c->slot_p = (long)c->NSTB * 32 * newcap;
      long s_floats = c->slot_s * 2 * (c->nh + 1);
      const long ring6 = snet6_ring_floats(newcap, c->nh);
      if (ring6 > s_floats) s_floats = ring6;
      rc = c->stash_s.reserve(c, s_floats);
      if (!rc) rc = c->stash_p.reserve(c, c->slot_p * (2 * c->nm + 2));
      if (!rc && c->NB * 32 > ((c->n + 15) / 16) * 16)
        rc = hipMemsetAsync(c->stash_s, 0, sizeof(float) * (size_t)s_floats, c->st) == hipSuccess ? NIF_OK : fail(NIF_ERR_HIP, "hipMemsetAsync(stash_s)");
    }
    if (rc) {
      for (DevBuf<float>* b : ws) b->drop();
      c->stash_s.drop(); c->stash_p.drop();
      c->cap = 0;
      return rc;
    }
    c->cap = newcap;
  }
  return train ? ensure_rows(c, B) : NIF_OK;
}

static MatRef dense_ref(long w_off, int nin, int nout) { MatRef m; m.r = 0; m.base_k = 0; m.kstride = 0; m.base_last = w_off; m.ld = nout; m.nin = nin; m.nout = nout; return m; }
static MatRef vec_ref(long b_off, int nout) { MatRef m; m.r = 0; m.base_k = 0; m.kstride = 0; m.base_last = b_off; m.ld = 0; m.nin = 1; m.nout = nout; return m; }
static MatRef hyper_ref(const nif_ctx* c, long slot, int ld, int nin, int nout) {
  MatRef m; m.r = c->r; m.base_k = c->last_w + slot; m.kstride = c->po; m.base_last = c->last_b + slot; m.ld = ld; m.nin = nin; m.nout = nout; return m;
}
static long hyper_wslot(const nif_ctx* c, int l) { return l == 0 ? 0 : (long)c->si * c->n + (long)(l - 1) * c->n * c->n; }
static long hyper_bslot(const nif_ctx* c, int l) { return hyper_wslot(c, c->nh + 1) + (long)c->n * c->so + (long)l * c->n; }
static MatRef hyper_w(const nif_ctx* c, int l) {
  const int nin = l == 0 ? c->si : c->n, nout = l == c->nh + 1 ? c->so : c->n;
  return hyper_ref(c, hyper_wslot(c, l), nout, nin, nout);
}
static MatRef hyper_b(const nif_ctx* c, int l) { return hyper_ref(c, hyper_bslot(c, l), 0, 1, l == c->nh + 1 ? c->so : c->n); }

static void mlp_mat(bool res, const long* w, const long* b, const long* w2, const long* b2, int j, long* w_off, long* b_off) {
  const int i = res ? j / 2 : j;
  const bool second = res && (j & 1);
  *w_off = second ? w2[i] : w[i]; *b_off = second ? b2[i] : b[i];
}
static void pnet_mat(const nif_ctx* c, int j, long* w_off, long* b_off) { mlp_mat(c->cfg.p_resblock, c->hid_w, c->hid_b, c->hid_w2, c->hid_b2, j, w_off, b_off); }
static void snet_mat(const nif_ctx* c, int j, long* w_off, long* b_off) { mlp_mat(c->cfg.s_resblock, c->s_hid_w, c->s_hid_b, c->s_hid_w2, c->s_hid_b2, j, w_off, b_off); }
static int policy_prec(const nif_ctx* c) { return c->cfg.mixed_policy == NIF_POLICY_MIXED_BF16 ? 1 : (c->cfg.mixed_policy == NIF_POLICY_MIXED_F16 ? 2 : 0); }

static void fill_pnet(const nif_ctx* c, PNetArgs& a, const float* xin, long B) {
  memset(&a, 0, sizeof(a));
  a.theta = c->theta; a.xin = xin; a.ncol = c->pi + c->si; a.col0 = 0; a.B = B;
  a.pi = c->pi; a.nst = c->nst; a.lst = c->lst; a.r = c->r;
  a.act = c->cfg.p_act; a.res = c->cfg.p_resblock; a.siren = (c->cfg.p_act == NIF_ACT_SINE);
  a.omega = a.siren ? c->cfg.p_omega0 : 1.0f;
  a.first_w = c->first_w; a.first_b = c->first_b;
  for (int i = 0; i < c->lst; ++i) { a.hid_w[i] = c->hid_w[i]; a.hid_b[i] = c->hid_b[i]; a.hid_w2[i] = c->hid_w2[i]; a.hid_b2[i] = c->hid_b2[i]; }
  a.bott_w = c->bott_w; a.bott_b = c->bott_b; a.last_w = c->last_w; a.last_b = c->last_b;
  a.ll_kind = (c->kind == NIF_KIND_LASTLAYER); a.zl_rows = 32 * c->RB;
  a.WF = c->pWF; a.WB = c->pWB; a.stash = c->stash_p; a.slot_stride = c->slot_p;
  a.Z = c->Z; a.DZ = a.ll_kind ? c->DZL : c->DZ; a.ZL = c->ZL;
}
static void ensure_ll_mlp_planes(nif_ctx* c) {
  if (c->ll_mlp_packed) return;
  const long plane_l = (long)c->NB * c->NB * 256;
  for (int j = 0; j < c->nh; ++j) {
    long w_off, b_off; snet_mat(c, j, &w_off, &b_off);
    launch_pack(c->theta, dense_ref(w_off, c->n, c->n), c->NB, c->NB, c->lWF + j * plane_l, c->lWB + j * plane_l, c->st);
  }
  c->ll_mlp_packed = true;
}
static void fill_snet_mlp(const nif_ctx* c, PNetArgs& a, const float* xin, int ncol, int col0, long B) {
  memset(&a, 0, sizeof(a));
  a.theta = c->theta; a.xin = xin; a.ncol = ncol; a.col0 = col0; a.B = B;
  a.pi = c->si; a.nst = c->n; a.lst = c->L; a.r = c->r * c->so;
  a.act = NIF_ACT_SINE; a.res = c->cfg.s_resblock; a.siren = 1; a.omega = c->cfg.s_omega0;
  a.first_w = c->s_first_w; a.first_b = c->s_first_b;
  for (int i = 0; i < c->L; ++i) { a.hid_w[i] = c->s_hid_w[i]; a.hid_b[i] = c->s_hid_b[i]; a.hid_w2[i] = c->s_hid_w2[i]; a.hid_b2[i] = c->s_hid_b2[i]; }
  a.bott_w = c->s_bott_w; a.bott_b = c->s_bott_b; a.ll_kind = 0;
  a.WF = c->lWF; a.WB = c->lWB; a.stash = c->stash_s; a.slot_stride = c->slot_s;
  a.Z = c->PHI; a.DZ = c->DPHI; a.ZL = nullptr;
}
static void fill_ll(const nif_ctx* c, LLArgs& a, long B) {
  memset(&a, 0, sizeof(a));
  a.theta = c->theta; a.bias_off = c->ll_bias; a.last_w = c->last_w; a.loss_kind = c->loss_kind;
  a.PHI = c->PHI; a.Z = c->Z; a.B = B; a.r = c->r; a.so = c->so;
  a.DU = c->DU; a.DPHI = c->DPHI; a.DA = c->DA; a.DZL = c->DZL; a.loss_partial = c->loss_partial;
}
static void fill_snet_ll(const nif_ctx* c, SNetArgs& a, const float* xin, int ncol, int col0, long B) {
  memset(&a, 0, sizeof(a));
  const int sop = c->so * c->r;
  a.theta = c->ll_slots; a.xin = xin; a.ncol = ncol; a.col0 = col0; a.B = B; a.loss_kind = c->loss_kind;
  a.si = c->si; a.so = sop; a.n = c->n; a.nh = c->nh; a.r = 0; a.po = 0;
  a.act = NIF_ACT_SINE; a.res = c->cfg.s_resblock; a.nif_skip = 0; a.omega = c->cfg.s_omega0;
  a.off_Wh = 0; a.off_bh = 0;
  a.Z = c->Z; a.WF4 = c->sWF4; a.WB4 = c->sWB4; a.stash = c->stash_s; a.slot_stride = c->slot_s;
  a.DU = c->DU; a.DZ = nullptr; a.dring = c->dring;
  a.ll = 1; a.rl = c->r; a.so_u = c->so; a.DPHI = c->DPHI; a.DA_ll = c->DA; a.DZL = c->DZL;
  a.WPF = c->ll_wpf; a.WPB = c->ll_wpb;
  a.prec = c->opt_fp32_mfma ? 0 : policy_prec(c);
  a.WF4h = c->sWF4h; a.WB4h = c->sWB4h;
  a.WF4x = c->sWF4x; a.WB4x = c->sWB4x; a.wscale = c->sWscale;
  a.nsm = snet4_nsm_ll(c->si, sop, c->nh, c->n, c->so, c->r);
  a.tl = c->tl;
}
static void fill_snet(const nif_ctx* c, SNetArgs& a, const float* xin, int ncol, int col0, long B) {
  memset(&a, 0, sizeof(a));
  a.theta = c->theta; a.xin = xin; a.ncol = ncol; a.col0 = col0; a.B = B; a.loss_kind = c->loss_kind;
  a.si = c->si; a.so = c->so; a.n = c->n; a.nh = c->nh; a.r = c->r; a.po = c->po;
  a.act = c->kind == NIF_KIND_NIF ? c->cfg.s_act : NIF_ACT_SINE;
  a.res = c->cfg.s_resblock; a.nif_skip = (c->kind == NIF_KIND_NIF);
  a.omega = c->kind == NIF_KIND_NIF ? 1.0f : c->cfg.s_omega0;
  a.off_Wh = c->last_w; a.off_bh = c->last_b;
  a.Z = c->Z; a.WF = c->sWF; a.WB = c->sWB; a.stash = c->stash_s; a.slot_stride = c->slot_s;
  a.DU = c->DU; a.DZ = c->DZ;
  a.nsm = snet3_nsm(c->si, c->so, c->nh, c->n);
  a.WF4 = c->use_snet4 ? c->sWF4 : nullptr; a.WB4 = c->use_snet4 ? c->sWB4 : nullptr;
  a.WF4x = c->use_snet4 ? c->sWF4x : nullptr; a.WB4x = c->use_snet4 ? c->sWB4x : nullptr; a.wscale = c->sWscale;
  a.prec = c->opt_fp32_mfma ? 0 : policy_prec(c);
  if (!c->use_snet4) a.prec = a.prec == 2 ? 0 : a.prec;
  a.WF4h = c->use_snet4 ? c->sWF4h : nullptr; a.WB4h = c->use_snet4 ? c->sWB4h : nullptr;
  a.dring = c->dring;
  a.tl = c->tl;
}

static int ensure_packed32(nif_ctx* c) {
  if (c->packed32 || c->kind == NIF_KIND_LASTLAYER) return NIF_OK;
  ProfScope ps_(c, NIF_PROF_PACK);
  const bool fmt16 = c->use_snet3 || c->jac_ok;
  const long plane_s = fmt16 ? snet3_plane_floats(c->n) / 4 : (long)c->NB * c->NB * 256;
  for (int j = 0; j < c->nh; ++j) {
    f32x4* wf = c->sWF + (long)j * (c->r + 1) * plane_s;
    f32x4* wb = c->sWB + (long)j * (c->r + 1) * plane_s;
    if (fmt16) launch_pack16(c->theta, hyper_w(c, 1 + j), snet3_nbl(c->n), wf, wb, c->st);
    else launch_pack(c->theta, hyper_w(c, 1 + j), c->NB, c->NB, wf, wb, c->st);
  }
  HIPCHK(hipGetLastError());
  c->packed32 = true;
  return NIF_OK;
}
static int ensure_packed_p32(nif_ctx* c) {
  if (c->packed_p32) return NIF_OK;
  ProfScope ps_(c, NIF_PROF_PACK);
  const long plane_p = (long)c->NSTB * c->NSTB * 256;
  for (int j = 0; j < c->nm; ++j) {
    long w_off, b_off; pnet_mat(c, j, &w_off, &b_off);
    launch_pack(c->theta, dense_ref(w_off, c->nst, c->nst), c->NSTB, c->NSTB, c->pWF + j * plane_p, c->pWB + j * plane_p, c->st);
  }
  HIPCHK(hipGetLastError());
  c->packed_p32 = true;
  return NIF_OK;
}
static int ensure_packed(nif_ctx* c) {
  if (!c->have_params) return fail(NIF_ERR_STATE, "parameters not set (call nif_set_params first)");
  if (c->packed) return NIF_OK;
  c->packed_p32 = false;
  if (c->NSTB > 1) { const int rcp = ensure_packed_p32(c); if (rcp) return rcp; }
  ProfScope ps_(c, NIF_PROF_PACK);
  if (c->kind == NIF_KIND_LASTLAYER) {
    c->ll_packed32 = false;
    c->ll_mlp_packed = false;
    {
      SNetArgs probe; fill_snet_ll(c, probe, nullptr, 0, 0, 32);
      static const bool ll_old = [] { const char* e = getenv("NIF_LL_MLP"); return e && e[0] == '1'; }();
      c->use_ll4 = c->sWF4 && c->ll_slots && c->ll_wpf && c->ll_wpb && !ll_old && snet4_supported(probe);
    }
    if (c->ll_slots) {
      const int n = c->n, nh = c->nh, sop = c->so * c->r;
      LLSlotMap m; m.nseg = 0;
      auto seg = [&](long src, long dst, long len) { m.seg[m.nseg].src = src; m.seg[m.nseg].dst = dst; m.seg[m.nseg].len = len; ++m.nseg; };
      const long s_wl = (long)c->si * n + (long)nh * n * n, s_b1 = s_wl + (long)n * sop, s_bh = s_b1 + n, s_bl = s_bh + (long)nh * n;
      seg(c->s_first_w, 0, (long)c->si * n);
      seg(c->s_bott_w, s_wl, (long)n * sop);
      seg(c->s_first_b, s_b1, n);
      for (int j = 0; j < nh; ++j) {
        long w_off, b_off; snet_mat(c, j, &w_off, &b_off);
        seg(b_off, s_bh + (long)j * n, n);
        if (c->use_ll4 && c->sWF4x)
          launch_pack16b_dual(c->theta, dense_ref(w_off, n, n), 0, 1, snet3_nbl(n),
                              (char*)c->sWF4 + (size_t)j * snet4_fwd_elems(n, 0) * 2, (char*)c->sWB4 + (size_t)j * snet4_bwd_elems(n, 0) * 2, 0, 0,
                              (char*)c->sWF4x + (size_t)j * snet4_bwd_elems(n, 0) * 2, (char*)c->sWB4x + (size_t)j * snet4_bwd_elems(n, 0) * 2,
                              0, 0, c->cfg.s_omega0, c->sWscale + (size_t)j * 2, c->st);
        else if (c->use_ll4)
          launch_pack16b(c->theta, dense_ref(w_off, n, n), snet3_nbl(n),
                         (char*)c->sWF4 + (size_t)j * snet4_fwd_elems(n, 0) * 2, (char*)c->sWB4 + (size_t)j * snet4_bwd_elems(n, 0) * 2,
                         c->cfg.s_omega0, c->st);
        if (c->use_ll4 && c->sWF4h)
          launch_pack16b(c->theta, dense_ref(w_off, n, n), snet3_nbl(n),
                         (char*)c->sWF4h + (size_t)j * (snet4_fwd_elems(n, 0) / 3) * 2, (char*)c->sWB4h + (size_t)j * (snet4_bwd_elems(n, 0) / 2) * 2,
                         c->cfg.s_omega0, c->st, policy_prec(c));
      }
      seg(c->s_bott_b, s_bl, sop);
      seg(c->ll_bias, s_bl + sop, c->so);
      seg(c->last_w, s_bl + sop + c->so, (long)c->r * c->r);
      launch_ll_slots(c->theta, m, c->ll_slots, c->st);
      if (c->use_ll4) launch_pack_phi(c->theta, c->s_bott_w, n, sop, c->ll_wpf, c->ll_wpb, c->st);
    }
    HIPCHK(hipGetLastError());
    c->packed = true;
    return NIF_OK;
  }
  SNetArgs probe; fill_snet(c, probe, nullptr, 0, 0, 32);
  c->use_snet3 = snet3_supported(probe);
  c->jac_ok = jac_supported(probe);
  const bool fp32_only = c->opt_fp32_mfma;
  c->use_snet4 = c->sWF4 && !fp32_only && snet4_supported(probe);
  c->packed32 = false;
  if (c->use_snet4 && c->nh > 0 && c->sWF4x)
    launch_pack16b_dual(c->theta, hyper_w(c, 1), hyper_wslot(c, 2) - hyper_wslot(c, 1), c->nh, snet3_nbl(c->n),
                        c->sWF4, c->sWB4, snet4_fwd_elems(c->n, c->r), snet4_bwd_elems(c->n, c->r),
                        c->sWF4x, c->sWB4x, snet4_bwd_elems(c->n, c->r), snet4_bwd_elems(c->n, c->r), probe.omega, c->sWscale, c->st);
  else if (c->use_snet4 && c->nh > 0)
    launch_pack16b_batch(c->theta, hyper_w(c, 1), hyper_wslot(c, 2) - hyper_wslot(c, 1), c->nh, snet3_nbl(c->n),
                         c->sWF4, c->sWB4, snet4_fwd_elems(c->n, c->r), snet4_bwd_elems(c->n, c->r), probe.omega, c->st);
  if (c->use_snet4 && c->nh > 0 && c->sWF4h)
    launch_pack16b_batch(c->theta, hyper_w(c, 1), hyper_wslot(c, 2) - hyper_wslot(c, 1), c->nh, snet3_nbl(c->n),
                         c->sWF4h, c->sWB4h, snet4_fwd_elems(c->n, c->r) / 3, snet4_bwd_elems(c->n, c->r) / 2, probe.omega, c->st,
                         policy_prec(c));
  HIPCHK(hipGetLastError());
  c->packed = true;
  if (!c->use_snet4) return ensure_packed32(c);
  return NIF_OK;
}

extern "C" int nif_forward_dev(nif_ctx* c, const float* xin, int64_t B, float* u) {
  if (!c || !xin || !u || B <= 0) return fail(NIF_ERR_INVALID, "bad argument");
  HIPCHK(hipSetDevice(c->dev));
  TAIL_FLUSH(c)
  int rc = ensure_packed(c); if (rc) return rc;
  rc = ensure_capacity(c, B, false); if (rc) return rc;
  PNetArgs pa; fill_pnet(c, pa, xin, B);
  { ProfScope p_(c, NIF_PROF_PNET_FWD); launch_pnet(pa, c->NSTB, false, c->st); }
  if (c->kind == NIF_KIND_LASTLAYER) {
    ProfScope p_(c, NIF_PROF_SNET_FWD);
    if (c->use_ll4) {
      SNetArgs sa; fill_snet_ll(c, sa, xin, c->pi + c->si, c->pi, B);
      sa.u_out = u;
      if (launch_snet4(sa, false, false, c->st) < 0) return fail(NIF_ERR_STATE, "internal: no k_snet4 form for this net (SIREN planes not packed as half pairs)");
      HIPCHK(hipGetLastError());
      return NIF_OK;
    }
    ensure_ll_mlp_planes(c); PNetArgs ma; fill_snet_mlp(c, ma, xin, c->pi + c->si, c->pi, B);
    launch_pnet(ma, c->NB, false, c->st);
    LLArgs la; fill_ll(c, la, B); la.u_out = u;
    launch_ll_out(la, false, c->st);
    HIPCHK(hipGetLastError());
    return NIF_OK;
  }
  SNetArgs sa; fill_snet(c, sa, xin, c->pi + c->si, c->pi, B);
  sa.u_out = u;
  {
    ProfScope p_(c, NIF_PROF_SNET_FWD);
    if (c->use_snet4) { if (launch_snet4(sa, false, false, c->st) < 0) return fail(NIF_ERR_STATE, "internal: no k_snet4 form for this net (SIREN planes not packed as half pairs)"); }
    else if (c->use_snet3) launch_snet3(sa, false, false, nullptr, c->st);
    else launch_snet(sa, c->NB, false, c->st);
  }
  HIPCHK(hipGetLastError());
  return NIF_OK;
}

static int stage(nif_ctx* c, DevBuf<float>& buf, const float* host, long n) {
  int rc = buf.reserve(c, n); if (rc) return rc;
  if (host) HIPCHK(hipMemcpyAsync(buf, host, sizeof(float) * (size_t)n, hipMemcpyHostToDevice, c->st));
  return NIF_OK;
}

extern "C" int nif_forward(nif_ctx* c, const float* xin, int64_t B, float* u) {
  if (!c || !xin || !u || B <= 0) return fail(NIF_ERR_INVALID, "bad argument");
  HIPCHK(hipSetDevice(c->dev));
  TAIL_FLUSH(c)
  HIPCHK(hipStreamSynchronize(c->st));
  int rc = stage(c, c->d_a, xin, B * (c->pi + c->si)); if (rc) return rc;
  rc = stage(c, c->d_d, nullptr, B * c->so); if (rc) return rc;
  rc = nif_forward_dev(c, c->d_a, B, c->d_d); if (rc) return rc;
  HIPCHK(hipMemcpyAsync(u, c->d_d, sizeof(float) * (size_t)(B * c->so), hipMemcpyDeviceToHost, c->st));
  HIPCHK(hipStreamSynchronize(c->st));
  return NIF_OK;
}

extern "C" int nif_jacobian(nif_ctx* c, const float* xin, int64_t B, const int32_t* y_idx, int32_t ny,
                            const int32_t* x_idx, int32_t nx, float* y_out, float* dydx_out) {
  if (!c || !xin || !y_idx || !x_idx || !y_out || !dydx_out || B <= 0 || ny <= 0 || nx <= 0)
    return fail(NIF_ERR_INVALID, "bad argument");
  for (int i = 0; i < ny; ++i)
    if (y_idx[i] < 0 || y_idx[i] >= c->so) return fail(NIF_ERR_INVALID, "y_index out of range");
  for (int j = 0; j < nx; ++j)
    if (x_idx[j] < 0 || x_idx[j] >= c->pi + c->si) return fail(NIF_ERR_INVALID, "x_index out of range");
  HIPCHK(hipSetDevice(c->dev));
  TAIL_FLUSH(c)
  HIPCHK(hipStreamSynchronize(c->st));
  int rc = ensure_packed(c); if (rc) return rc;
  rc = ensure_packed32(c); if (rc) return rc;
  rc = ensure_packed_p32(c); if (rc) return rc;
  const bool ll = c->kind == NIF_KIND_LASTLAYER;
  if (!ll && !c->jac_ok) return fail(NIF_ERR_INVALID, "JacobianLayer: one weight plane and the small hyper-vectors of this shape exceed the 160 KB LDS of a CU");
  rc = ensure_capacity(c, B, false); if (rc) return rc;
  const long ntiles = (B + 31) / 32;
  const int ncol = c->pi + c->si;
  rc = stage(c, c->d_a, xin, B * ncol); if (rc) return rc;
  rc = stage(c, c->d_d, nullptr, B * c->so); if (rc) return rc;
  rc = stage(c, c->d_b, nullptr, B * c->so * nx); if (rc) return rc;
  const long zd_sz = ntiles * 32 * (long)c->r * (ll ? c->so : 1);
  rc = c->d_c.reserve(c, 3 * zd_sz); if (rc) return rc;
  PNetArgs pa; fill_pnet(c, pa, c->d_a, B);
  if (ll) {
    rc = nif_forward_dev(c, c->d_a, B, c->d_d); if (rc) return rc;
    ensure_ll_mlp_planes(c); PNetArgs ma; fill_snet_mlp(c, ma, c->d_a, ncol, c->pi, B);
    if (c->use_ll4) launch_pnet(ma, c->NB, false, c->st);
    for (int j = 0; j < nx; ++j) {
      if (x_idx[j] >= c->pi) {
        PNetArgs mj = ma; mj.Z = c->DPHI;
        launch_mlp_jac(mj, c->NB, x_idx[j] - c->pi, c->d_c, c->st);
        launch_ll_jac_out(c->PHI, c->Z, c->d_c, nullptr, B, c->r, c->so, nx, j, c->d_b, c->st);
      } else {
        PNetArgs pj = pa; pj.Z = c->DA;
        launch_mlp_jac(pj, c->NSTB, x_idx[j], c->d_c, c->st);
        launch_ll_jac_out(c->PHI, c->Z, nullptr, c->d_c, B, c->r, c->so, nx, j, c->d_b, c->st);
      }
    }
  } else {
    launch_pnet(pa, c->NSTB, false, c->st);
    SNetArgs sa; fill_snet(c, sa, c->d_a, ncol, c->pi, B);
    for (int x0 = 0; x0 < nx; x0 += 3) {
      int seeds[3] = {0, 0, 0};
      const float* zd[3] = {nullptr, nullptr, nullptr};
      const int ns = nx - x0 < 3 ? nx - x0 : 3;
      for (int d = 0; d < ns; ++d) {
        const int col = x_idx[x0 + d];
        if (col >= c->pi) { seeds[d] = col - c->pi; }
        else {
          seeds[d] = -1;
          PNetArgs pj = pa; pj.Z = c->DZ;
          launch_mlp_jac(pj, c->NSTB, col, c->d_c + d * zd_sz, c->st);
          zd[d] = c->d_c + d * zd_sz;
        }
      }
      sa.u_out = x0 == 0 ? c->d_d : nullptr;
      launch_jac(sa, ns, seeds, zd, nx, x0, c->d_b, c->st);
    }
  }
  HIPCHK(hipGetLastError());
  std::vector<float> full((size_t)B * c->so * nx);
  HIPCHK(hipMemcpyAsync(y_out, c->d_d, sizeof(float) * (size_t)(B * c->so), hipMemcpyDeviceToHost, c->st));
  HIPCHK(hipMemcpyAsync(full.data(), c->d_b, sizeof(float) * full.size(), hipMemcpyDeviceToHost, c->st));
  HIPCHK(hipStreamSynchronize(c->st));
  for (int64_t a_ = 0; a_ < B; ++a_)
    for (int i = 0; i < ny; ++i)
      for (int j = 0; j < nx; ++j) dydx_out[(a_ * ny + i) * nx + j] = full[((size_t)a_ * c->so + y_idx[i]) * nx + j];
  return NIF_OK;
}

static int hessian_core(nif_ctx* c, const float* xin_dev, int64_t B, const int32_t* y_idx, int32_t ny, const int32_t* x_idx,
                        int32_t nx, float* y_dev, float* dydx_dev, float* d2_dev) {
  bool anyp = false;
  for (int j = 0; j < nx; ++j) anyp = anyp || x_idx[j] < c->pi;
  int rc = ensure_packed(c); if (rc) return rc;
  rc = ensure_capacity(c, B, false); if (rc) return rc;
  const int ncol = c->pi + c->si;
  const long ntl = (B + 31) / 32;
  HessIdx I; I.ny = ny;
  for (int i = 0; i < 16; ++i) I.y_idx[i] = i < ny ? y_idx[i] : 0;
  PNetArgs pa; fill_pnet(c, pa, xin_dev, B);
  launch_pnet(pa, c->NSTB, false, c->st);
  std::vector<int> xc, xp;
  for (int j = 0; j < nx; ++j) (x_idx[j] >= c->pi ? xc : xp).push_back(j);
// ... 344 lines not shown
      spar.zl_rows = 32 * c->RB;
      for (int e = 0; e < nhead; ++e) { spar.parc[e] = sp->par[nsc + e]; spar.pcol[e] = sp->gcol[nsc + e]; }
    }
    ProfScope p_(c, NIF_PROF_SNET);
    launch_sob(sa, true, nsc, sp->seeds, gt, wj, c->dring, nullptr, false, c->st, &spar);
  } else if (c->use_ll4) {
    SNetArgs sa; fill_snet_ll(c, sa, xin, ncol, c->pi, B);
    sa.y = y; sa.sw = sw; sa.loss_partial = c->loss_partial; sa.inv_bg = 1.0f / (float)Bg;
    {
      const int nbl = snet3_nbl(c->n);
      ll_dab = sa.prec == 1 && (nbl == 2 || nbl == 4 || nbl == 8) && gw_da_bf16_ok(c->NB, c->NB, 0);
      sa.da_bf16 = ll_dab ? 1 : 0;
      if (snet4_writes_da_bf16(sa) != ll_dab) return fail(NIF_ERR_STATE, "internal: dL/da stash format of producer and plan disagree");
      sa.h_ph16 = (ll_dab && nbl == 8 && !c->cfg.s_resblock && gw_in_ph16_ok(c->NB, c->NB, 0)) ? 1 : 0;
      ll_ph = snet4_writes_h_ph16(sa);
      if (ll_ph != (sa.h_ph16 != 0)) return fail(NIF_ERR_STATE, "internal: layer-input stash format of producer and plan disagree");
    }
    int rc = ll4_plan(c, sa, &nloss); if (rc) return rc;
    ProfScope p_(c, NIF_PROF_SNET);
    if (launch_snet4(sa, true, false, c->st) < 0) return fail(NIF_ERR_STATE, "internal: no k_snet4 form for this net (SIREN planes not packed as half pairs)");
  } else {
    ProfScope p_(c, NIF_PROF_SNET);
    launch_pnet(ma, c->NB, true, c->st);
    launch_ll_out(la, true, c->st);
    launch_pnet_bwd(ma, c->NB, c->st);
  }
  int n_act = 0;
  if (act_on(c)) {
    const long nlp = (B + 255) / 256;
    int rc = c->act_loss.reserve(c, nlp); if (rc) return rc;
    const bool l1 = c->act_l2 == 0.f;
    n_act = launch_ll_actreg(c->Z, c->theta + c->last_w, c->r, B, (l1 ? c->act_l1 : c->act_l2) / (float)Bg, l1, c->DA, c->DZL, c->act_loss, c->st);
  }
  const int rows = rows_for(c, ntiles);
  { ProfScope p_(c, NIF_PROF_PNET_BWD);
    if (fused_p) launch_pnet_bwg(pa, c->partial, c->pstride, rows, c->st);
    else launch_pnet_bwd(pa, c->NSTB, c->st); }
  {
    ProfScope p_(c, NIF_PROF_GW);
    const GwArgs base = gw_base(c, ntiles, B, c->partial);
    GwArgs sbase = base;
    if (nsc > 0) gw_add_tangents(sbase, nsc, sp->seeds);
    const int nms = c->nh;
    float* sST = c->stash_s;
    GwArgs g = sbase;
    g.DA = sST + (long)(nms + 1) * c->slot_s; g.xin = xin; g.ncol = ncol; g.col0 = c->pi; g.nd = c->si; g.scale = ma.omega;
    if (ns > 0 && sp->hess) g.ntiles = ntiles * 3;
    g.W = dense_ref(c->s_first_w, c->si, c->n); g.Bv = vec_ref(c->s_first_b, c->n);
    launch_gw_first(g, c->NB, rows, c->st);
    for (int mi = 0; mi < nms; ++mi) {
      g = sbase; g.IN = sST + (long)mi * c->slot_s; g.DA = sST + (long)(nms + 2 + mi) * c->slot_s; g.scale = ma.omega;
      long w_off, b_off; snet_mat(c, mi, &w_off, &b_off);
      g.W = dense_ref(w_off, c->n, c->n); g.Bv = vec_ref(b_off, c->n);
      g.da_bf16 = ll_dab ? 1 : 0;
      g.in_ph16 = ll_ph ? 1 : 0;
      if (launch_gw_mfma(g, c->NB, c->NB, rows, c->st) < 0) return fail(NIF_ERR_STATE, "internal: bf16 dL/da stash rows without a reader of that form");
    }
    g = sbase; g.IN = sST + (long)nms * c->slot_s; g.SM = c->DPHI; g.nc = c->r * c->so;
    g.W = dense_ref(c->s_bott_w, c->n, c->r * c->so); g.Bv = vec_ref(c->s_bott_b, c->r * c->so);
    launch_gw_out(g, c->NB, rows, c->st);
    g = base; g.IN = sST + (long)nms * c->slot_s; g.SM = c->DU; g.nc = c->so;
    g.W = dense_ref(0, 0, c->so); g.Bv = vec_ref(c->ll_bias, c->so);
    launch_gw_out(g, c->NB, rows, c->st);
    if (!fused_p) gw_pnet_stack(c, base, xin, c->stash_p, c->DZL, pa.omega, rows, c->st);
    g = base; g.IN = c->ZL; g.SM = c->DA; g.nc = c->r;
    g.W = dense_ref(c->last_w, c->r, c->r); g.Bv = vec_ref(c->last_b, c->r);
    launch_gw_out(g, c->RB, rows, c->st);
  }
  {
    ProfScope pr_(c, NIF_PROF_REDUCE);
    launch_reduce(c->partial, c->pstride, rows, c->loss_partial, nloss, c->grad, c->P, c->st);
  }
  if (n_act > 0) launch_add_sum(c->act_loss, n_act, c->grad + c->P, c->st);
  if (c->jac_l1 != 0.f) { int rc = jac_reg_pass(c, xin, B, Bg); if (rc) return rc; }
  if (nhead > 0) {
    { const int rca = ensure_jac_tmp(c); if (rca) return rca; }
    MuBlk mu;
    const long rr = (long)c->r * c->r;
    for (int e = 0; e < nhead; ++e) {
      mu.blk[sp->par[nsc + e]] = e;
      GwArgs g = gw_base(c, ntiles, B, c->partial);
      g.IN = c->ztl_par + (long)e * ntiles * 32 * 32 * c->RB; g.SM = c->dat_par + (long)e * ntiles * 32 * c->r; g.nc = c->r;
      g.W = dense_ref(c->last_w, c->r, c->r); g.Bv = vec_ref(c->last_b, c->r);
      launch_gw_out(g, c->RB, rows, c->st);
      launch_reduce(c->partial + c->last_w, c->pstride, rows, nullptr, 0, c->jac_tmp, rr, c->st);
      launch_axpy_cols(c->grad + c->last_w, c->jac_tmp, rr, c->P - c->last_w, c->st);
    }
    HIPCHK(hipGetLastError());
    return jac_reg_pass(c, xin, B, Bg, mu.blk);
  }
  HIPCHK(hipGetLastError());
  return NIF_OK;
}

static int snet_plan(nif_ctx* c, SNetArgs& sa, int ns, const int* seeds, int* nloss, const SobPlan* sp = nullptr) {
  int rc;
  if (ns > 0) {
    SobPar spq{};
    if (sp) spq = sob_par_of(*sp);
    const int nblk = launch_sob(sa, true, ns, seeds, nullptr, 0.f, nullptr, nullptr, true, c->st, sp ? &spq : nullptr);
    if (nblk < 0)
      return fail(NIF_ERR_INVALID, "Sobolev step: the kernel's working set of this shape (units, latent_dim, parameter columns) does not fit the 160 KB LDS of a CU");
    const long need = (long)nblk * 4 * sob_ring_floats_per_wave(c->n, c->nh);
    rc = c->dring.reserve(c, need); if (rc) return rc;
    *nloss = nblk;
  } else if (c->use_snet3 || c->use_snet4) {
    int waves = 4;
    const int nblk = c->use_snet4 ? launch_snet4(sa, true, true, c->st) : launch_snet3(sa, true, true, &waves, c->st);
    const long need = (long)nblk * waves * snet3_ring_floats_per_wave(c->n, c->nh);
    rc = c->dring.reserve(c, need); if (rc) return rc;
    *nloss = nblk;
  }
  sa.dring = c->dring;
  return NIF_OK;
}

static long pipe_chunk_points(const nif_ctx* c, long B) {
  long ch = c->opt_pipe_chunk;
  if (ch < 0) ch = 0;
  if (ch <= 0) return 0;
  ch = (ch + 2047) / 2048 * 2048;
  return ch;
}

static int ensure_pipe(nif_ctx* c, int nchunk) {
  if (!c->st2) {
    HIPCHK(hipStreamCreateWithFlags(&c->st2, hipStreamNonBlocking));
    HIPCHK(hipEventCreateWithFlags(&c->ev_start, hipEventDisableTiming));
    HIPCHK(hipEventCreateWithFlags(&c->ev_done, hipEventDisableTiming));
  }
  while ((int)c->ev_chunk.size() < nchunk) {
    hipEvent_t e;
    HIPCHK(hipEventCreateWithFlags(&e, hipEventDisableTiming));
    c->ev_chunk.push_back(e);
  }
  return c->chunk_grad.reserve(c, (long)nchunk * c->pstride);
}

static int step_chunk(nif_ctx* c, const float* xin0, const float* y0, const float* sw0, long off, long B, long Bg, int ns,
                      const int* seeds, const float* gt, float wj, hipStream_t sa_st, hipStream_t sb_st, hipStream_t pb_st,
                      float* partial, float* loss_partial, int* nloss_out, int chunk_idx, bool whole, SNetArgs* sa_out = nullptr,
                      const SobPlan* sp = nullptr) {
  int rc;
  const int ncol = c->pi + c->si;
  const long ntiles = (B + 31) / 32, t0 = off / 32;
  const float* xin = xin0 + off * ncol;
  const float* y = y0 + off * c->so;
  const float* sw = sw0 ? sw0 + off : nullptr;
  PNetArgs pa; fill_pnet(c, pa, xin, B);
  pa.Z = c->Z + t0 * 32 * c->r; pa.DZ = c->DZ + t0 * 32 * c->r;
  if (pa.stash) pa.stash += t0 * 32 * 32 * c->NSTB;
  const bool fused_p = !pnet_force_stash() && pnet_bwg_supported(pa);
  if (!fused_p) { const int rcp = ensure_packed_p32(c); if (rcp) return rcp; }
  { ProfScope p_(c, NIF_PROF_PNET_FWD, sa_st); launch_pnet(pa, c->NSTB, !fused_p, sa_st); }
  SNetArgs sa; fill_snet(c, sa, xin, ncol, c->pi, B);
  sa.Z = pa.Z; sa.DZ = pa.DZ; sa.DU = c->DU + t0 * 32 * c->so;
  sa.stash = c->stash_s + t0 * 32 * 32 * c->NB;
  sa.y = y; sa.sw = sw; sa.u_out = nullptr; sa.loss_partial = loss_partial; sa.inv_bg = 1.0f / (float)Bg;
  if (!whole) sa.wg_cap = c->opt_pipe_wgs;
  int nloss = (int)((ntiles + 3) / 4);
  rc = snet_plan(c, sa, ns, seeds, &nloss, sp); if (rc) return rc;
  const bool fused_gw = ns == 0 && whole && c->use_snet4 && c->opt_fuse_gw && snet6_supported(sa) &&
                        snet6_rows(sa) == rows_for(c, ntiles);
  if (fused_gw) nloss = snet6_rows(sa);
  *nloss_out = nloss;
  {
    const int nbl = snet3_nbl(c->n);
    bool dab = sa.prec == 1 && (nbl == 2 || nbl == 4 || nbl == 8) && gw_da_bf16_ok(c->NB, c->NB, c->r);
    if (ns > 0) dab = dab && sobw_supported(sa, ns, sp && sp->any_par);
    else dab = dab && c->use_snet4 && !fused_gw;
    sa.da_bf16 = dab ? 1 : 0;
    sa.h_ph16 = (dab && ns == 0 && nbl == 8 && !c->cfg.s_resblock && !sa.nif_skip && gw_in_ph16_ok(c->NB, c->NB, c->r)) ? 1 : 0;
  }
  const bool wrote_da_bf16 = ns > 0 ? sob_writes_da_bf16(sa, ns, sp && sp->any_par)
                                    : (!fused_gw && c->use_snet4 && snet4_writes_da_bf16(sa));
  if (wrote_da_bf16 != (sa.da_bf16 != 0)) return fail(NIF_ERR_STATE, "internal: dL/da stash format of producer and plan disagree");
  const bool wrote_h_ph16 = ns == 0 && !fused_gw && c->use_snet4 && snet4_writes_h_ph16(sa);
  if (wrote_h_ph16 != (sa.h_ph16 != 0)) return fail(NIF_ERR_STATE, "internal: layer-input stash format of producer and plan disagree");
  {
    ProfScope p_(c, NIF_PROF_SNET, sa_st);
    if (ns > 0) {
      SobPar spar{};
      if (sp) spar = sob_par_of(*sp);
      if (sp && sp->any_par) { spar.ZT = c->zt_par; spar.DZT = c->dzt_par; }
      launch_sob(sa, true, ns, seeds, gt, wj, c->dring, nullptr, false, sa_st, sp ? &spar : nullptr);
    }
    else if (fused_gw) launch_snet6(sa, partial, c->pstride, sa_st);
    else if (c->use_snet4) { if (launch_snet4(sa, true, false, sa_st) < 0) return fail(NIF_ERR_STATE, "internal: no k_snet4 form for this net (SIREN planes not packed as half pairs)"); }
    else if (c->use_snet3) launch_snet3(sa, true, false, nullptr, sa_st);
    else launch_snet(sa, c->NB, true, sa_st);
  }
  if (act_on(c)) {
    const long nlp = (B + 255) / 256;
    rc = c->act_loss.reserve(c, nlp); if (rc) return rc;
    const bool l1 = c->act_l2 == 0.f;
    launch_actreg_points(l1, c->theta, c->last_w, c->last_b, c->r, c->po, sa.Z, B, (l1 ? c->act_l1 : c->act_l2) / (float)Bg, sa.DZ,
                         c->act_loss, sa_st);
  }
  if (sb_st != sa_st || pb_st != sa_st) {
    HIPCHK(hipEventRecord(c->ev_chunk[chunk_idx], sa_st));
    if (sb_st != sa_st) HIPCHK(hipStreamWaitEvent(sb_st, c->ev_chunk[chunk_idx], 0));
    if (pb_st != sa_st && pb_st != sb_st) HIPCHK(hipStreamWaitEvent(pb_st, c->ev_chunk[chunk_idx], 0));
  }
  const int rows = rows_for(c, ntiles);
  { ProfScope p_(c, NIF_PROF_PNET_BWD, pb_st);
    static const bool touch_on = [] { const char* e = getenv("NIF_PBW_TOUCH"); return !(e && e[0] == '0'); }();
    const float* touch = (touch_on && whole && pb_st == sb_st && !fused_gw) ? sa.stash + (long)(c->nh + 1) * c->slot_s : nullptr;
    if (fused_p) launch_pnet_bwg(pa, partial, c->pstride, rows, pb_st, touch, (long)c->NB * 1024);
    else launch_pnet_bwd(pa, c->NSTB, pb_st); }
  ProfScope pgw(c, NIF_PROF_GW, sb_st);
  const GwArgs base = gw_base(c, ntiles, B, partial);
  if (!fused_gw) {
    GwArgs sbase = base;
    gw_add_tangents(sbase, ns, seeds);
    long first_ntiles = sbase.ntiles;
    if (sp) first_ntiles = ntiles * (1 + sp->nsc);
    if (sp && sp->hess) first_ntiles = ntiles * 3;
    if (gw_hyper_snet_stack(c, sbase, sa, xin, sa.Z, 0, first_ntiles, wrote_da_bf16, wrote_h_ph16, rows, sb_st) < 0)
      return fail(NIF_ERR_STATE, "internal: bf16 dL/da stash rows without a reader of that form");
  }
  if (!fused_p) gw_pnet_stack(c, base, xin, pa.stash, pa.DZ, pa.omega, rows, pb_st);
  if (sa_out) *sa_out = sa;
  HIPCHK(hipGetLastError());
  return NIF_OK;
}

static int ensure_small_tables(nif_ctx* c, const PNetArgs& pa, const SNetArgs& sa) {
  if (c->small_idx) return NIF_OK;
  if (c->capturing) return fail(NIF_ERR_STATE, "small-batch step tables inside a graph capture (nif_graph_begin builds them)");
  std::vector<int> idx, desc;
  small_tables(pa, sa, idx, desc);
  DevBuf<int> d_idx, d_desc;
  int rc = d_idx.alloc((long)idx.size()); if (rc) return rc;
  rc = d_desc.alloc((long)desc.size()); if (rc) return rc;
  HIPCHK(hipMemcpy(d_idx, idx.data(), idx.size() * sizeof(int), hipMemcpyHostToDevice));
  HIPCHK(hipMemcpy(d_desc, desc.data(), desc.size() * sizeof(int), hipMemcpyHostToDevice));
  c->small_idx = std::move(d_idx); c->small_desc = std::move(d_desc);
  return NIF_OK;
}
int nif_tail_flush(nif_ctx* c) {
  if (!c || !c->tail_pending) return NIF_OK;
  c->tail_pending = false;
  HIPCHK(hipSetDevice(c->dev));
  launch_reduce(c->partial, c->pstride, c->tail_rows, c->loss_partial, c->tail_nloss, c->grad, c->P, c->st);
  HIPCHK(hipGetLastError());
  return NIF_OK;
}
static bool tail_can_defer(const nif_ctx* c) {
  if (!c->opt_fuse_tail || c->comm || c->capturing || c->prof_on) return false;
  if ((c->reg_l1 != 0.f || c->reg_l2 != 0.f) && c->reg_hi > c->reg_lo) return false;
  if (c->sreg_l1 != 0.f || c->sreg_l2 != 0.f) return false;
  return true;
}
int nif_metric_flush(nif_ctx* c) {
  if (!c || !c->metric_pending) return NIF_OK;
  HIPCHK(hipSetDevice(c->dev));
  TAIL_FLUSH(c)
  c->metric_pending = false;
  launch_metric(c->grad, c->P, c->metric_pending_w, c->metric, c->st);
  HIPCHK(hipGetLastError());
  return NIF_OK;
}
static int loss_grad_core(nif_ctx* c, const float* xin, const float* y, const float* sw, int64_t B, int64_t Bg, int ns,
                          const int* seeds, const float* gt, float wj, const SobPlan* sp = nullptr) {
  HIPCHK(hipSetDevice(c->dev));
  TAIL_FLUSH(c)
  c->last_step_small = false;
  if (ns == 0 && c->opt_small_step && B <= NIF_SMALL_MAX_B && c->kind != NIF_KIND_LASTLAYER && !act_on(c) && !c->opt_fp32_mfma) {
    if (!c->have_params) return fail(NIF_ERR_STATE, "parameters not set (call nif_set_params first)");
    PNetArgs pa; fill_pnet(c, pa, xin, B);
    SNetArgs sa; fill_snet(c, sa, xin, c->pi + c->si, c->pi, B);
    if (small_supported(pa, sa) && small_rows(B) <= 256) {
      int rc = ensure_rows(c, B); if (rc) return rc;
      const int rows = small_rows(B);
      if (rows > c->rows_cap()) return fail(NIF_ERR_STATE, "internal: partial-row buffer too small for the small-batch step");
      if (rows > c->loss_partial.n) return fail(NIF_ERR_STATE, "internal: loss partial buffer too small for the small-batch step");
      c->reg_applied = false;
      sa.y = y; sa.sw = sw; sa.loss_partial = c->loss_partial; sa.inv_bg = 1.0f / (float)Bg;
      rc = ensure_small_tables(c, pa, sa); if (rc) return rc;
      const bool mp = c->metric_pending && c->metric != nullptr;
      { ProfScope p_(c, NIF_PROF_SNET);
        launch_small(pa, sa, c->partial, c->pstride, c->P, c->small_idx, c->small_desc, mp ? c->metric : nullptr, c->metric_pending_w,
                     c->grad + c->P, c->st); }
      if (mp) c->metric_pending = false;
      c->last_step_small = true;
      if (c->jac_l1 == 0.f && tail_can_defer(c)) { c->tail_pending = true; c->tail_rows = rows; c->tail_nloss = rows; }
      else { ProfScope pr_(c, NIF_PROF_REDUCE); launch_reduce(c->partial, c->pstride, rows, c->loss_partial, rows, c->grad, c->P, c->st); }
      if (c->jac_l1 != 0.f) { rc = jac_reg_pass(c, xin, B, Bg); if (rc) return rc; }
      HIPCHK(hipGetLastError());
      return NIF_OK;
    }
  }
  int rc = nif_metric_flush(c); if (rc) return rc;
  rc = ensure_packed(c); if (rc) return rc;
  const long ntiles = (B + 31) / 32;
  if (ns > 0) { rc = ensure_packed32(c); if (rc) return rc; }
  if (ns > 0) {
    if (c->kind != NIF_KIND_LASTLAYER && !c->jac_ok)
      return fail(NIF_ERR_INVALID, "Sobolev training: one weight plane and the small hyper-vectors of this shape exceed the 160 KB LDS of a CU");
    if (c->cfg.s_resblock && (c->nh & 1)) return fail(NIF_ERR_INVALID, "resblock ShapeNet with an odd matrix count");
  }
  rc = ensure_capacity(c, ntiles * 32 * (1 + ns), true); if (rc) return rc;
  if (sp && sp->any_par) {
    PNetArgs pa; fill_pnet(c, pa, xin, B);
    rc = ensure_zt_par(c, pa, ntiles, true); if (rc) return rc;
  }
  c->reg_applied = false;
  if (c->kind == NIF_KIND_LASTLAYER) return loss_grad_ll(c, xin, y, sw, B, Bg, ns, sp, gt, wj);
  const long chunk = (ns == 0 && c->use_snet3 && !act_on(c) && c->jac_l1 == 0.f) ? pipe_chunk_points(c, B) : 0;
  if (chunk <= 0 || chunk >= B) {
    int nloss = 0;
    SNetArgs sae;
    const bool side = c->opt_side_pnet && B >= 65536;
    if (side) { rc = ensure_pipe(c, 1); if (rc) return rc; }
    rc = step_chunk(c, xin, y, sw, 0, B, Bg, ns, seeds, gt, wj, c->st, c->st, side ? c->st2 : c->st, c->partial, c->loss_partial,
                    &nloss, 0, true, &sae, sp);
    if (rc) return rc;
    if (side) {
      HIPCHK(hipEventRecord(c->ev_done, c->st2));
      HIPCHK(hipStreamWaitEvent(c->st, c->ev_done, 0));
    }
    const int rows = rows_for(c, ntiles);
    if (ns == 0 && !act_on(c) && c->jac_l1 == 0.f && !(sp && sp->any_par) && tail_can_defer(c)) {
      c->tail_pending = true; c->tail_rows = rows; c->tail_nloss = nloss;
      HIPCHK(hipGetLastError());
      return NIF_OK;
    }
    ProfScope pr_(c, NIF_PROF_REDUCE);
    launch_reduce(c->partial, c->pstride, rows, c->loss_partial, nloss, c->grad, c->P, c->st);
    if (act_on(c)) {
      const long need = (long)NIF_ACT_SLABS * (c->r + 1) * c->po;
      rc = c->act_part.reserve(c, need); if (rc) return rc;
      const bool l1 = c->act_l2 == 0.f;
      launch_actreg_planes(l1, c->theta, c->last_w, c->last_b, c->r, c->po, c->Z, B, NIF_ACT_SLABS, c->act_part, c->st);
      launch_actreg_apply(c->act_part, NIF_ACT_SLABS, c->r, c->po, (l1 ? c->act_l1 : c->act_l2) / (float)Bg, c->last_w, c->last_b,
                          c->act_loss, (int)((B + 255) / 256), c->grad, c->P, c->st);
    }
    if (c->jac_l1 != 0.f) { rc = jac_reg_pass(c, xin, B, Bg); if (rc) return rc; }
    if (sp && sp->any_par) { rc = sob_par_pass(c, xin, B, Bg, *sp, sae); if (rc) return rc; }
    HIPCHK(hipGetLastError());
    return NIF_OK;
  }
  const int nchunk = (int)((B + chunk - 1) / chunk);
  rc = ensure_pipe(c, nchunk); if (rc) return rc;
  HIPCHK(hipEventRecord(c->ev_start, c->st));
  HIPCHK(hipStreamWaitEvent(c->st2, c->ev_start, 0));
  const long lp_stride = c->loss_partial.n / nchunk;
  for (int i = 0; i < nchunk; ++i) {
    const long off = (long)i * chunk;
    const long Bc = B - off < chunk ? B - off : chunk;
    int nloss = 0;
    rc = step_chunk(c, xin, y, sw, off, Bc, Bg, 0, nullptr, nullptr, 0.f, c->st, c->st2, c->st2, c->partial,
                    c->loss_partial + i * lp_stride, &nloss, i, false);
    if (rc) return rc;
    if (nloss > lp_stride) return fail(NIF_ERR_STATE, "loss partial buffer too small for the chunk pipeline");
    const int rows = rows_for(c, (Bc + 31) / 32);
    launch_reduce(c->partial, c->pstride, rows, c->loss_partial + i * lp_stride, nloss, c->chunk_grad + (long)i * c->pstride, c->P, c->st2);
  }
  HIPCHK(hipEventRecord(c->ev_done, c->st2));
  HIPCHK(hipStreamWaitEvent(c->st, c->ev_done, 0));
  {
    ProfScope pr_(c, NIF_PROF_REDUCE);
    launch_reduce(c->chunk_grad, c->pstride, nchunk, nullptr, 0, c->grad, c->P + 1, c->st);
  }
  HIPCHK(hipGetLastError());
  return NIF_OK;
}

extern "C" int nif_loss_grad_dev(nif_ctx* c, const float* xin, const float* y, const float* sw, int64_t B, int64_t Bg) {
  if (!c || !xin || !y || B <= 0 || Bg < B) return fail(NIF_ERR_INVALID, "bad argument");
  return loss_grad_core(c, xin, y, sw, B, Bg, 0, nullptr, nullptr, 0.f);
}

extern "C" int nif_reserve(nif_ctx* c, int64_t B_max, int32_t n_tangents) {
  if (!c || B_max <= 0 || n_tangents < 0 || n_tangents > 16) return fail(NIF_ERR_INVALID, "bad argument");
  if (n_tangents > 3) n_tangents = 3;
  HIPCHK(hipSetDevice(c->dev));
  TAIL_FLUSH(c)
  int rc = ensure_packed(c); if (rc) return rc;
  const long ntiles = (B_max + 31) / 32;
  rc = ensure_capacity(c, ntiles * 32 * (1 + n_tangents), true); if (rc) return rc;
  if (c->kind == NIF_KIND_LASTLAYER) {
    if (c->use_ll4) {
      SNetArgs sa; fill_snet_ll(c, sa, nullptr, c->pi + c->si, c->pi, B_max);
      int nblk = 0;
      rc = ll4_plan(c, sa, &nblk); if (rc) return rc;
    }
    return NIF_OK;
  }
  SNetArgs sa; fill_snet(c, sa, nullptr, c->pi + c->si, c->pi, B_max);
  int nloss = 0;
  const int seeds[3] = {0, 0, 0};
  rc = snet_plan(c, sa, n_tangents, seeds, &nloss); if (rc) return rc;
  const long chunk = (n_tangents == 0 && c->use_snet3) ? pipe_chunk_points(c, B_max) : 0;
  if (chunk > 0 && chunk < B_max) { rc = ensure_pipe(c, (int)((B_max + chunk - 1) / chunk)); if (rc) return rc; }
  return NIF_OK;
}

static int sobolev_plan(nif_ctx* c, const int32_t* x_idx, int32_t nx, SobPlan* sp) {
  if (!x_idx || nx < 1 || nx > 3) return fail(NIF_ERR_INVALID, "internal: a Sobolev pass carries 1..3 columns");
  memset(sp, 0, sizeof(*sp));
  sp->ns = nx;
  for (int d = 0; d < nx; ++d) {
    if (x_idx[d] < 0 || x_idx[d] >= c->pi + c->si) return fail(NIF_ERR_INVALID, "Sobolev x_index out of range (0 <= i < pi_dim + si_dim)");
    for (int e = 0; e < d; ++e)
      if (x_idx[e] == x_idx[d]) return fail(NIF_ERR_INVALID, "Sobolev x_index lists a column twice");
  }
  int q = 0;
  for (int d = 0; d < nx; ++d)
    if (x_idx[d] >= c->pi) { sp->seeds[q] = x_idx[d] - c->pi; sp->par[q] = -1; sp->gcol[q] = d; ++q; }
  sp->nsc = q;
  for (int d = 0; d < nx; ++d)
    if (x_idx[d] < c->pi) { sp->seeds[q] = 0; sp->par[q] = x_idx[d]; sp->gcol[q] = d; ++q; sp->any_par = true; }
  for (; q < 3; ++q) { sp->seeds[q] = 0; sp->par[q] = -1; sp->gcol[q] = q; }
  return NIF_OK;
}
static int sobolev_check(nif_ctx* c, const int32_t* x_idx, int32_t nx, const int32_t* y_idx, int32_t ny, unsigned* ymask, int* ny_out) {
  if (!x_idx || nx < 1 || nx > 16) return fail(NIF_ERR_INVALID, "Sobolev training takes 1..16 input columns in x_index");
  for (int d = 0; d < nx; ++d) {
    if (x_idx[d] < 0 || x_idx[d] >= c->pi + c->si) return fail(NIF_ERR_INVALID, "Sobolev x_index out of range (0 <= i < pi_dim + si_dim)");
    for (int e = 0; e < d; ++e)
      if (x_idx[e] == x_idx[d]) return fail(NIF_ERR_INVALID, "Sobolev x_index lists a column twice");
  }
  *ymask = 0; *ny_out = 0;
  if (y_idx) {
    if (ny < 1 || ny > c->so) return fail(NIF_ERR_INVALID, "Sobolev y_index: 1..output_dim distinct outputs");
    for (int i = 0; i < ny; ++i) {
      if (y_idx[i] < 0 || y_idx[i] >= c->so) return fail(NIF_ERR_INVALID, "Sobolev y_index out of range");
      if (*ymask & (1u << y_idx[i])) return fail(NIF_ERR_INVALID, "Sobolev y_index lists an output twice");
      *ymask |= 1u << y_idx[i];
    }
    *ny_out = ny;
  }
  return NIF_OK;
}
static int sob_cols_per_pass(nif_ctx* c, const int32_t* x_idx, int nx) {
  if (c->kind == NIF_KIND_LASTLAYER) return 3;
  if (ensure_packed(c) != NIF_OK) return 3;
  for (int gs = 3; gs > 1; --gs) {
    bool ok = true;
    for (int g0 = 0; g0 < nx && ok; g0 += gs) {
      const int ng = nx - g0 < gs ? nx - g0 : gs;
      SobPlan sp;
      if (sobolev_plan(c, x_idx + g0, ng, &sp) != NIF_OK) return 3;
      SNetArgs sa; fill_snet(c, sa, nullptr, c->pi + c->si, c->pi, 64);
      const SobPar spq = sob_par_of(sp);
      ok = launch_sob(sa, true, ng, sp.seeds, nullptr, 0.f, nullptr, nullptr, true, c->st, &spq) >= 0;
// ... 560 lines not shown
extern "C" int nif_graph_launch_opt(nif_ctx* c, int32_t graph_id, const nif_opt* opt) {
  if (!c || !opt || !graph_ok(c, graph_id)) return fail(NIF_ERR_INVALID, "bad argument");
  const int rc = opt_check(opt); if (rc) return rc;
  const int rk = c->graph_kind[graph_id];
  if (rk >= 0 && (rk != opt_kk(opt) || (c->graph_ams[graph_id] != 0) != opt_ams(opt)))
    return fail(NIF_ERR_INVALID, "nif_graph_launch_opt: the graph was recorded with another optimizer kind / amsgrad flag (or centered / decoupled weight decay flag)");
  return graph_replay(c, graph_id, opt, "nif_graph_launch_opt");
}
extern "C" int nif_get_opt_slot(nif_ctx* c, int32_t slot, float* host, int64_t n) {
  if (!c || !host || slot < 0 || slot > 2) return fail(NIF_ERR_INVALID, "bad argument (slot: 0 m, 1 v, 2 vhat)");
  if (n != c->P) return fail(NIF_ERR_INVALID, "parameter count mismatch");
  HIPCHK(hipSetDevice(c->dev));
  TAIL_FLUSH(c)
  float* src = slot == 0 ? c->m : slot == 1 ? c->v : c->vhat;
  if (!src) { memset(host, 0, sizeof(float) * (size_t)n); return NIF_OK; }
  HIPCHK(hipMemcpyAsync(host, src, sizeof(float) * (size_t)n, hipMemcpyDeviceToHost, c->st));
  HIPCHK(hipStreamSynchronize(c->st));
  return NIF_OK;
}
extern "C" int nif_set_opt_slot(nif_ctx* c, int32_t slot, const float* host, int64_t n) {
  if (!c || !host || slot < 0 || slot > 2) return fail(NIF_ERR_INVALID, "bad argument (slot: 0 m, 1 v, 2 vhat)");
  if (n != c->P) return fail(NIF_ERR_INVALID, "parameter count mismatch");
  if (c->capturing) return fail(NIF_ERR_STATE, "nif_set_opt_slot while capturing");
  HIPCHK(hipSetDevice(c->dev));
  TAIL_FLUSH(c)
  if (slot == 2) { const int rc = ensure_vhat(c); if (rc) return rc; }
  float* dst = slot == 0 ? c->m : slot == 1 ? c->v : c->vhat;
  HIPCHK(hipMemcpyAsync(dst, host, sizeof(float) * (size_t)n, hipMemcpyHostToDevice, c->st));
  HIPCHK(hipStreamSynchronize(c->st));
  c->slots_fresh = false;
  return NIF_OK;
}

static void prune_free(nif_ctx* c) {
  c->prune_segs_dev.drop(); c->prune_mask.drop(); c->prune_thr.drop(); c->prune_hist.drop(); c->prune_sel.drop();
  c->prune_segs.clear(); c->prune_nblk = 0; c->prune_lo = 0; c->prune_hi = 0;
}
static int prune_enter(nif_ctx* c, bool need_config) {
  if (c->capturing) return fail(NIF_ERR_STATE, "nif_prune_*: not inside a graph capture");
  if (need_config && c->prune_segs.empty()) return fail(NIF_ERR_STATE, "pruning is not configured (nif_prune_config)");
  HIPCHK(hipSetDevice(c->dev));
  TAIL_FLUSH(c)
  return nif_metric_flush(c);
}
extern "C" int nif_prune_config(nif_ctx* c, int32_t n, const int64_t* offsets, const int64_t* sizes) {
  if (!c || n < 0 || (n > 0 && (!offsets || !sizes))) return fail(NIF_ERR_INVALID, "bad argument");
  std::vector<PruneSeg> segs((size_t)n);
  long nblk = 0, end = 0;
  for (int i = 0; i < n; ++i) {
    const long off = (long)offsets[i], sz = (long)sizes[i];
    if (off < end || sz < 1 || sz > 0x7fffffffL || off + sz > c->P)
      return fail(NIF_ERR_INVALID, "nif_prune_config: segments must be non-empty, below 2^31 floats, inside theta, increasing and disjoint");
    segs[i].off = off; segs[i].size = sz; segs[i].k = sz; segs[i].blk0 = nblk;
    nblk += (sz + PRUNE_CHUNK - 1) / PRUNE_CHUNK;
    end = off + sz;
  }
  int rc = prune_enter(c, false); if (rc) return rc;
  HIPCHK(hipStreamSynchronize(c->st));
  prune_free(c);
  if (n == 0) return NIF_OK;
  DevBuf<PruneSeg> segs_dev; DevBuf<unsigned char> mask; DevBuf<float> thr; DevBuf<unsigned> hist; DevBuf<PruneSel> sel;
  rc = segs_dev.alloc(n); if (rc) return rc;
  rc = mask.alloc(c->P + 16); if (rc) return rc;
  rc = thr.alloc(n); if (rc) return rc;
  rc = hist.alloc((long)PRUNE_BINS * n); if (rc) return rc;
  rc = sel.alloc(n); if (rc) return rc;
  HIPCHK(hipMemcpy(segs_dev, segs.data(), sizeof(PruneSeg) * (size_t)n, hipMemcpyHostToDevice));
  HIPCHK(hipMemsetAsync(mask, 1, (size_t)c->P + 16, c->st));
  HIPCHK(hipMemsetAsync(thr, 0, sizeof(float) * (size_t)n, c->st));
  HIPCHK(hipMemsetAsync(hist, 0, sizeof(unsigned) * PRUNE_BINS * (size_t)n, c->st));
  HIPCHK(hipStreamSynchronize(c->st));
  c->prune_segs_dev = std::move(segs_dev); c->prune_mask = std::move(mask); c->prune_thr = std::move(thr);
  c->prune_hist = std::move(hist); c->prune_sel = std::move(sel);
  c->prune_segs = segs; c->prune_nblk = nblk; c->prune_lo = segs.front().off; c->prune_hi = end;
  return NIF_OK;
}
extern "C" int nif_prune_update(nif_ctx* c, const int64_t* k) {
  if (!c || !k) return fail(NIF_ERR_INVALID, "null");
  if (!c->have_params) return fail(NIF_ERR_STATE, "parameters not set");
  int rc = prune_enter(c, true); if (rc) return rc;
  const int n = (int)c->prune_segs.size();
  for (int i = 0; i < n; ++i)
    if (k[i] < 1 || k[i] > c->prune_segs[i].size) return fail(NIF_ERR_INVALID, "nif_prune_update: 1 <= k <= the segment's size");
  HIPCHK(hipStreamSynchronize(c->st));
  for (int i = 0; i < n; ++i) c->prune_segs[i].k = (long)k[i];
  HIPCHK(hipMemcpyAsync(c->prune_segs_dev, c->prune_segs.data(), sizeof(PruneSeg) * (size_t)n, hipMemcpyHostToDevice, c->st));
  launch_prune_update(c->theta, c->prune_segs_dev, n, c->prune_nblk, c->prune_hist, c->prune_sel, c->prune_thr, c->prune_mask, c->st);
  HIPCHK(hipGetLastError());
  return NIF_OK;
}
extern "C" int nif_prune_apply(nif_ctx* c) {
  if (!c) return fail(NIF_ERR_INVALID, "null");
  if (!c->have_params) return fail(NIF_ERR_STATE, "parameters not set");
  int rc = prune_enter(c, true); if (rc) return rc;
  launch_prune_apply(c->theta, c->prune_mask, c->prune_lo, c->prune_hi, c->P, c->st);
  HIPCHK(hipGetLastError());
  c->packed = false; c->packed32 = false; c->packed_p32 = false;
  return NIF_OK;
}
static long prune_total(const nif_ctx* c) {
  long t = 0;
  for (const PruneSeg& s : c->prune_segs) t += s.size;
  return t;
}
extern "C" int nif_get_prune_state(nif_ctx* c, float* masks, int64_t n_mask, float* thr, int32_t n_seg) {
  if (!c || !masks || !thr) return fail(NIF_ERR_INVALID, "null");
  int rc = prune_enter(c, true); if (rc) return rc;
  if (n_mask != prune_total(c) || n_seg != (int32_t)c->prune_segs.size()) return fail(NIF_ERR_INVALID, "nif_get_prune_state: size mismatch");
  std::vector<unsigned char> h((size_t)c->P);
  HIPCHK(hipMemcpyAsync(h.data(), c->prune_mask, (size_t)c->P, hipMemcpyDeviceToHost, c->st));
  HIPCHK(hipMemcpyAsync(thr, c->prune_thr, sizeof(float) * (size_t)n_seg, hipMemcpyDeviceToHost, c->st));
  HIPCHK(hipStreamSynchronize(c->st));
  long o = 0;
  for (const PruneSeg& s : c->prune_segs)
    for (long i = 0; i < s.size; ++i) masks[o++] = h[(size_t)(s.off + i)] ? 1.f : 0.f;
  return NIF_OK;
}
extern "C" int nif_set_prune_state(nif_ctx* c, const float* masks, int64_t n_mask, const float* thr, int32_t n_seg) {
  if (!c || !masks || !thr) return fail(NIF_ERR_INVALID, "null");
  int rc = prune_enter(c, true); if (rc) return rc;
  if (n_mask != prune_total(c) || n_seg != (int32_t)c->prune_segs.size()) return fail(NIF_ERR_INVALID, "nif_set_prune_state: size mismatch");
  std::vector<unsigned char> h((size_t)c->P + 16, 1);
  long o = 0;
  for (const PruneSeg& s : c->prune_segs)
    for (long i = 0; i < s.size; ++i, ++o) {
      if (masks[o] != 0.f && masks[o] != 1.f) return fail(NIF_ERR_INVALID, "nif_set_prune_state: mask values are 0 or 1");
      h[(size_t)(s.off + i)] = masks[o] != 0.f ? 1 : 0;
    }
  HIPCHK(hipMemcpyAsync(c->prune_mask, h.data(), h.size(), hipMemcpyHostToDevice, c->st));
  HIPCHK(hipMemcpyAsync(c->prune_thr, thr, sizeof(float) * (size_t)n_seg, hipMemcpyHostToDevice, c->st));
  HIPCHK(hipStreamSynchronize(c->st));
  return NIF_OK;
}

extern "C" int nif_zero_grad(nif_ctx* c) {
  if (!c) return fail(NIF_ERR_INVALID, "null");
  HIPCHK(hipSetDevice(c->dev));
  TAIL_FLUSH(c)
  { const int rcf = nif_metric_flush(c); if (rcf) return rcf; }
  c->last_step_small = false;
  HIPCHK(hipMemsetAsync(c->grad, 0, sizeof(float) * (size_t)(c->P + 1), c->st));
  c->reg_applied = false;
  return NIF_OK;
}

extern "C" int nif_device_pci_bus_id(int32_t dev, char* out, int32_t cap) {
  if (!out || cap < 16) return fail(NIF_ERR_INVALID, "bad argument");
  HIPCHK(hipDeviceGetPCIBusId(out, cap, dev));
  return NIF_OK;
}

extern "C" int nif_set_option(nif_ctx* c, const char* key, int32_t value) {
  if (!c || !key) return fail(NIF_ERR_INVALID, "null");
  if (strcmp(key, "fuse_gw") == 0) { c->opt_fuse_gw = value != 0; return NIF_OK; }
  if (strcmp(key, "fuse_tail") == 0) { c->opt_fuse_tail = value != 0; return NIF_OK; }
  if (strcmp(key, "small_step") == 0) { c->opt_small_step = value != 0; return NIF_OK; }
  if (strcmp(key, "fp32_mfma") == 0) {
    c->opt_fp32_mfma = value != 0;
    c->packed = false; c->packed32 = false; c->packed_p32 = false;
    return NIF_OK;
  }
  if (strcmp(key, "side_pnet") == 0) { c->opt_side_pnet = value != 0; return NIF_OK; }
  if (strcmp(key, "pipe_chunk") == 0) { c->opt_pipe_chunk = value; return NIF_OK; }
  if (strcmp(key, "pipe_wgs") == 0) { c->opt_pipe_wgs = value; return NIF_OK; }
  return fail(NIF_ERR_INVALID, std::string("unknown option ") + key);
}

extern "C" int nif_grad_read(nif_ctx* c, float* loss, float* grad) {
  if (!c) return fail(NIF_ERR_INVALID, "null");
  HIPCHK(hipSetDevice(c->dev));
  TAIL_FLUSH(c)
  { const int rcr_ = apply_reg(c); if (rcr_) return rcr_; }
  if (grad) HIPCHK(hipMemcpyAsync(grad, c->grad, sizeof(float) * (size_t)c->P, hipMemcpyDeviceToHost, c->st));
  if (loss) HIPCHK(hipMemcpyAsync(loss, c->grad + c->P, sizeof(float), hipMemcpyDeviceToHost, c->st));
  HIPCHK(hipStreamSynchronize(c->st));
  return NIF_OK;
}

extern "C" int nif_f64_set_params(nif_ctx* c, const double* host, int64_t n) {
  if (!c || !host) return fail(NIF_ERR_INVALID, "null");
  return nif_f64_set_params_impl(c, host, n);
}
extern "C" int nif_f64_get_params(nif_ctx* c, double* host, int64_t n) {
  if (!c || !host) return fail(NIF_ERR_INVALID, "null");
  return nif_f64_get_params_impl(c, host, n);
}
extern "C" int nif_f64_forward_dev(nif_ctx* c, const double* xin, int64_t B, double* u) {
  if (!c || !xin || !u || B <= 0) return fail(NIF_ERR_INVALID, "bad argument");
  return nif_f64_forward_dev_impl(c, xin, B, u);
}
extern "C" int nif_f64_loss_grad_dev(nif_ctx* c, const double* xin, const double* y, const double* sw, int64_t B, int64_t Bg) {
  if (!c || !xin || !y || B <= 0 || Bg < B) return fail(NIF_ERR_INVALID, "bad argument");
  return nif_f64_loss_grad_dev_impl(c, xin, y, sw, B, Bg);
}
extern "C" int nif_f64_grad_read(nif_ctx* c, double* loss, double* grad) {
  if (!c) return fail(NIF_ERR_INVALID, "null");
  return nif_f64_grad_read_impl(c, loss, grad);
}
extern "C" int nif_last_loss(nif_ctx* c, float* loss) {
  if (!c || !loss) return fail(NIF_ERR_INVALID, "null");
  HIPCHK(hipSetDevice(c->dev));
  TAIL_FLUSH(c)
  HIPCHK(hipMemcpyAsync(loss, c->grad + c->P, sizeof(float), hipMemcpyDeviceToHost, c->st));
  HIPCHK(hipStreamSynchronize(c->st));
  return NIF_OK;
}

static int stage_batch(nif_ctx* c, const float* xin, const float* y, const float* sw, long B) {
  HIPCHK(hipStreamSynchronize(c->st));
  int rc = stage(c, c->d_a, xin, B * (c->pi + c->si)); if (rc) return rc;
  rc = stage(c, c->d_b, y, B * c->so); if (rc) return rc;
  if (sw) { rc = stage(c, c->d_c, sw, B); if (rc) return rc; }
  return NIF_OK;
}
int nif_stage_batch(nif_ctx* c, const float* xin, const float* y, const float* sw, int64_t B, float** dx, float** dy, float** dsw) {
  HIPCHK(hipSetDevice(c->dev));
  int rc = stage_batch(c, xin, y, sw, B); if (rc) return rc;
  *dx = c->d_a; *dy = c->d_b; *dsw = sw ? c->d_c : nullptr;
  return NIF_OK;
}

extern "C" int nif_loss_and_grad(nif_ctx* c, const float* xin, const float* y, const float* sw, int64_t B, float* loss,
                                 float* grad) {
  if (!c || !xin || !y || B <= 0) return fail(NIF_ERR_INVALID, "bad argument");
  HIPCHK(hipSetDevice(c->dev));
  TAIL_FLUSH(c)
  int rc = stage_batch(c, xin, y, sw, B); if (rc) return rc;
  rc = nif_loss_grad_dev(c, c->d_a, c->d_b, sw ? c->d_c : nullptr, B, B); if (rc) return rc;
  TAIL_FLUSH(c)
  { const int rcr_ = apply_reg(c); if (rcr_) return rcr_; }
  if (grad) HIPCHK(hipMemcpyAsync(grad, c->grad, sizeof(float) * (size_t)c->P, hipMemcpyDeviceToHost, c->st));
  if (loss) HIPCHK(hipMemcpyAsync(loss, c->grad + c->P, sizeof(float), hipMemcpyDeviceToHost, c->st));
  HIPCHK(hipStreamSynchronize(c->st));
  return NIF_OK;
}

extern "C" int nif_train_step(nif_ctx* c, const float* xin, const float* y, const float* sw, int64_t B,
                              const nif_adam* opt, float* loss) {
  if (!c || !xin || !y || !opt || B <= 0) return fail(NIF_ERR_INVALID, "bad argument");
  HIPCHK(hipSetDevice(c->dev));
  TAIL_FLUSH(c)
  int rc = stage_batch(c, xin, y, sw, B); if (rc) return rc;
  rc = nif_loss_grad_dev(c, c->d_a, c->d_b, sw ? c->d_c : nullptr, B, B); if (rc) return rc;
  rc = nif_adam_step_dev(c, opt); if (rc) return rc;
  if (loss) HIPCHK(hipMemcpyAsync(loss, c->grad + c->P, sizeof(float), hipMemcpyDeviceToHost, c->st));
  HIPCHK(hipStreamSynchronize(c->st));
  return NIF_OK;
}

static int drain_profile(nif_ctx* c) {
  HIPCHK(hipStreamSynchronize(c->st));
  for (auto& r : c->recs) {
    float ms = 0.f;
    HIPCHK(hipEventElapsedTime(&ms, r.a, r.b));
    c->prof_ms[r.id] += ms; c->prof_cnt[r.id] += 1;
    c->ev_pool.push_back(r.a); c->ev_pool.push_back(r.b);
  }
  c->recs.clear();
  return NIF_OK;
}
extern "C" int nif_profile_enable(nif_ctx* c, int on) {
  if (!c) return fail(NIF_ERR_INVALID, "null");
  HIPCHK(hipSetDevice(c->dev));
  TAIL_FLUSH(c)
  int rc = drain_profile(c); if (rc) return rc;
  c->prof_on = on != 0;
  return NIF_OK;
}
extern "C" int nif_profile_read(nif_ctx* c, float* ms, int64_t* cnt, int n, int reset) {
  if (!c || !ms || !cnt || n < NIF_PROF_N) return fail(NIF_ERR_INVALID, "bad argument");
  HIPCHK(hipSetDevice(c->dev));
  TAIL_FLUSH(c)
  int rc = drain_profile(c); if (rc) return rc;
  for (int i = 0; i < NIF_PROF_N; ++i) { ms[i] = (float)c->prof_ms[i]; cnt[i] = c->prof_cnt[i]; }
  if (reset) for (int i = 0; i < NIF_PROF_N; ++i) { c->prof_ms[i] = 0; c->prof_cnt[i] = 0; }
  return NIF_OK;
}
extern "C" int nif_debug_timeline(nif_ctx* c, int64_t* out, int32_t n_pairs) {
  if (!c || n_pairs < 0 || n_pairs > 2048) return fail(NIF_ERR_INVALID, "bad argument");
  HIPCHK(hipSetDevice(c->dev));
  TAIL_FLUSH(c)
  HIPCHK(hipStreamSynchronize(c->st));
  if (!c->tl) {
    DevBuf<long long> tl;
    const int rc = tl.alloc(4096); if (rc) return rc;
    HIPCHK(hipMemset(tl, 0, 4096 * sizeof(long long)));
    c->tl = std::move(tl);
    return NIF_OK;
  }
  if (out && n_pairs > 0) HIPCHK(hipMemcpy(out, c->tl, sizeof(long long) * 2 * n_pairs, hipMemcpyDeviceToHost));
  HIPCHK(hipMemset(c->tl, 0, 4096 * sizeof(long long)));
  return NIF_OK;
}
extern "C" int nif_timer_start(nif_ctx* c) {
  if (!c) return fail(NIF_ERR_INVALID, "null");
  HIPCHK(hipSetDevice(c->dev));
  TAIL_FLUSH(c)
  if (!c->t0) { HIPCHK(hipEventCreate(&c->t0)); HIPCHK(hipEventCreate(&c->t1)); }
  HIPCHK(hipEventRecord(c->t0, c->st));
  return NIF_OK;
}
extern "C" int nif_timer_stop(nif_ctx* c, float* ms) {
  if (!c || !ms || !c->t0) return fail(NIF_ERR_INVALID, "timer not started");
  HIPCHK(hipSetDevice(c->dev));
  TAIL_FLUSH(c)
  HIPCHK(hipEventRecord(c->t1, c->st));
// ... 5 lines not shown
```

### nif_amd/csrc/nif_ctx.h

```cpp
#pragma once
#include "../../include/nif_hip.h"
#include "nif_internal.h"
#include <string>
#include <vector>

int nif_fail(int code, const std::string& msg);
static inline int fail(int code, const std::string& msg) { return nif_fail(code, msg); }
#define HIPCHK(expr)                                                                              \
  do {                                                                                            \
    hipError_t e_ = (expr);                                                                       \
    if (e_ != hipSuccess) {                                                                       \
      (void)hipGetLastError();  \
      return fail(NIF_ERR_HIP, std::string(#expr) + ": " + hipGetErrorString(e_));                 \
    }                                                                                             \
  } while (0)

struct nif_ctx;
template <class T, bool Pinned = false>
struct DevBuf {
  T* p = nullptr; long n = 0;
  DevBuf() = default;
  DevBuf(const DevBuf&) = delete;
  DevBuf& operator=(const DevBuf&) = delete;
  DevBuf(DevBuf&& o) noexcept : p(o.p), n(o.n) { o.p = nullptr; o.n = 0; }
  DevBuf& operator=(DevBuf&& o) noexcept { if (this != &o) { drop(); p = o.p; n = o.n; o.p = nullptr; o.n = 0; } return *this; }
  ~DevBuf() { drop(); }
  operator T*() const { return p; }
  void drop() {
    if (p) (void)(Pinned ? hipHostFree(p) : hipFree(p));
    p = nullptr; n = 0;
  }
  int alloc(long count) {
    drop();
    T* q = nullptr;
    if (Pinned) HIPCHK(hipHostMalloc(&q, sizeof(T) * (size_t)count));
    else HIPCHK(hipMalloc(&q, sizeof(T) * (size_t)count));
    p = q; n = count;
    return NIF_OK;
  }
  int release(nif_ctx* c);
  int reserve(nif_ctx* c, long count);
};

struct NifF64;

struct nif_ctx {
  nif_cfg cfg;
  NifF64* f64 = nullptr;
  int dev = 0;
  hipStream_t st = nullptr;
  int kind, pi, si, so, n, L, nst, lst, r, nh, nm, NB, NSTB;
  long po, P;
  std::vector<nif_tensor_desc> layout;
  long first_w, first_b, hid_w[NIF_MAX_HID], hid_b[NIF_MAX_HID], hid_w2[NIF_MAX_HID], hid_b2[NIF_MAX_HID];
  long bott_w, bott_b, last_w, last_b;
  long s_first_w = 0, s_first_b = 0, s_hid_w[NIF_MAX_HID], s_hid_b[NIF_MAX_HID], s_hid_w2[NIF_MAX_HID], s_hid_b2[NIF_MAX_HID];
  long s_bott_w = 0, s_bott_b = 0, ll_bias = 0;
  int RB = 1;
  DevBuf<float> theta, grad, m, v;
  long step = 0;
  bool have_params = false, packed = false, packed32 = false, packed_p32 = false, use_snet3 = false, use_snet4 = false;
  bool jac_ok = false;
  DevBuf<char> sWF4, sWB4;
  DevBuf<char> sWF4x, sWB4x;
  DevBuf<float> sWscale;
  DevBuf<char> sWF4h, sWB4h;
  bool use_ll4 = false;
  DevBuf<float> ll_slots;
  DevBuf<char> ll_wpf, ll_wpb;
  DevBuf<f32x4> pWF, pWB, sWF, sWB, lWF, lWB;
  long cap = 0;
  DevBuf<float> stash_s, stash_p, Z, DZ, DU, ZL;
  long slot_s = 0, slot_p = 0;
  DevBuf<float> partial; long pstride = 0;
  int rows_cap() const { return (int)(partial.n / pstride); }
  DevBuf<float> loss_partial;
  DevBuf<float> dring;
  DevBuf<long long> tl;
  float reg_l1 = 0.f, reg_l2 = 0.f; long reg_lo = 0, reg_hi = 0; bool reg_applied = false;
  float sreg_l1 = 0.f, sreg_l2 = 0.f;
  DevBuf<double> metric;
  bool ll_packed32 = false;
  DevBuf<float> zt_par, dzt_par;
  DevBuf<float> dat_par, ztl_par;
  float jac_l1 = 0.f; DevBuf<float> jac_mu, jac_tmp;
  std::vector<hipGraphExec_t> graphs; std::vector<int> graph_steps; bool capturing = false; int cap_steps = 0; long cap_step0 = 0;
  DevBuf<OptDev> opt_dev; DevBuf<OptDev, true> opt_host;
  DevBuf<float> vhat;
  bool slots_fresh = true;
  int cap_kind = -1; bool cap_ams = false; std::vector<int> graph_kind; std::vector<char> graph_ams;
  std::vector<PruneSeg> prune_segs; long prune_nblk = 0, prune_lo = 0, prune_hi = 0;
  DevBuf<PruneSeg> prune_segs_dev; DevBuf<unsigned char> prune_mask; DevBuf<float> prune_thr;
  DevBuf<unsigned> prune_hist; DevBuf<PruneSel> prune_sel;
  nif_grad_transform gt = {}; bool gt_on = false, gt_norm = false; int gt_ran = 0;
  DevBuf<GtBlk> gt_blk; int gt_nblk = 0; DevBuf<float> gt_part, gt_norms; DevBuf<GtDev> gt_dev;
  int cap_gt = 0; std::vector<char> graph_gt;
  bool ll_mlp_packed = false;
  int loss_kind = 0;
  DevBuf<float> sob2_acc;
  DevBuf<float> sob_acc;
  float act_l1 = 0.f, act_l2 = 0.f; DevBuf<float> act_part, act_loss;
  DevBuf<float> PHI, DPHI, DA, DZL;
  bool prof_on = false;
  std::vector<hipEvent_t> ev_pool;
  struct Rec { int id; hipEvent_t a, b; };
  std::vector<Rec> recs;
  double prof_ms[NIF_PROF_N] = {0};
  long prof_cnt[NIF_PROF_N] = {0};
  hipEvent_t t0 = nullptr, t1 = nullptr;
  DevBuf<float> d_a, d_b, d_c, d_d;
  void* comm = nullptr; int comm_rank = 0, comm_world = 1;
  DevBuf<float> comm_scratch;
  hipStream_t st2 = nullptr; hipEvent_t ev_start = nullptr, ev_done = nullptr; std::vector<hipEvent_t> ev_chunk;
  DevBuf<float> chunk_grad;
  bool opt_side_pnet = false;
  long opt_pipe_chunk = -1; int opt_pipe_wgs = 512;
  hipStream_t st_copy = nullptr; hipEvent_t ev_copied[2] = {nullptr, nullptr}, ev_consumed[2] = {nullptr, nullptr};
  bool opt_fp32_mfma = false;
  DevBuf<int> small_idx, small_desc;
  bool metric_pending = false; float metric_pending_w = 0.f;
  bool last_step_small = false;
  bool tail_pending = false; int tail_rows = 0, tail_nloss = 0; bool opt_fuse_tail = true;
  bool opt_small_step = true;
  bool opt_fuse_gw = true;
  nif_ctx() = default;
  nif_ctx(const nif_ctx&) = delete;
  ~nif_ctx();
};

template <class T, bool Pinned> int DevBuf<T, Pinned>::release(nif_ctx* c) {
  HIPCHK(hipStreamSynchronize(c->st));
  if (c->st2) HIPCHK(hipStreamSynchronize(c->st2));
  drop();
  return NIF_OK;
}
template <class T, bool Pinned> int DevBuf<T, Pinned>::reserve(nif_ctx* c, long count) {
  if (count <= n) return NIF_OK;
  const int rc = release(c); if (rc) return rc;
  return alloc(count);
}

struct ProfScope {
  nif_ctx* c; int id; hipEvent_t a = nullptr, b = nullptr;
  hipStream_t s;
  ProfScope(nif_ctx* c_, int id_, hipStream_t s_ = nullptr) : c(c_), id(id_), s(s_ ? s_ : c_->st) {
    if (!c->prof_on || c->capturing) return;
    auto get = [&]() { hipEvent_t e; if (!c->ev_pool.empty()) { e = c->ev_pool.back(); c->ev_pool.pop_back(); } else { (void)hipEventCreate(&e); } return e; };
    a = get(); b = get();
    (void)hipEventRecord(a, s);
  }
  ~ProfScope() {
    if (!a) return;
    (void)hipEventRecord(b, s);
    c->recs.push_back({id, a, b});
  }
};

int nif_stage_batch(nif_ctx* c, const float* xin, const float* y, const float* sw, int64_t B, float** dx, float** dy, float** dsw);
int nif_tail_flush(nif_ctx* c);
int nif_metric_flush(nif_ctx* c);
int nif_f64_set_params_impl(nif_ctx* c, const double* host, int64_t n);
int nif_f64_get_params_impl(nif_ctx* c, double* host, int64_t n);
int nif_f64_forward_dev_impl(nif_ctx* c, const double* xin, int64_t B, double* u);
int nif_f64_loss_grad_dev_impl(nif_ctx* c, const double* xin, const double* y, const double* sw, int64_t B, int64_t Bg);
int nif_f64_grad_read_impl(nif_ctx* c, double* loss, double* grad);
void nif_f64_release(nif_ctx* c);
#define TAIL_FLUSH(c_) { const int rct_ = nif_tail_flush(c_); if (rct_) return rct_; }
```

### nif_amd/csrc/nif_internal.h

```cpp
#pragma once
#include <vector>
#include <hip/hip_runtime.h>
#include <stdint.h>

#define NIF_MAX_HID 16
#define NIF_TP 32

typedef float f32x16 __attribute__((ext_vector_type(16)));
typedef float f32x4 __attribute__((ext_vector_type(4)));
typedef float f32x4u __attribute__((ext_vector_type(4), aligned(4)));

enum { ACT_LINEAR = 0, ACT_SINE = 1, ACT_SWISH = 2, ACT_TANH = 3, ACT_RELU = 4, ACT_SIGMOID = 5,
       ACT_ELU = 6, ACT_SOFTPLUS = 7, ACT_GELU = 8,
       ACT_SELU = 9, ACT_SOFTSIGN = 10, ACT_EXPONENTIAL = 11, ACT_HARD_SIGMOID = 12 };
#define NIF_SELU_ALPHA 1.6732632423543772f
#define NIF_SELU_SCALE 1.0507009873554805f

struct MatRef {
  int r;
  long base_k, kstride, base_last;
  int ld, nin, nout;
};
__host__ __device__ inline long matref_index(const MatRef& m, int k, int in, int out) {
  return (k < m.r ? m.base_k + (long)k * m.kstride : m.base_last) + (long)in * m.ld + out;
}

struct PNetArgs {
  const float* theta;
  const float* xin; int ncol; int col0;
  long B;
  int pi, nst, lst, r;
  int act, res, siren; float omega;
  long first_w, first_b;
  long hid_w[NIF_MAX_HID], hid_b[NIF_MAX_HID], hid_w2[NIF_MAX_HID], hid_b2[NIF_MAX_HID];
  long bott_w, bott_b;
  int ll_kind; long last_w, last_b;
  int pbf2;
  const f32x4* WF; const f32x4* WB;
  float* stash; long slot_stride;
  float* Z;
  float* DZ;
  float* ZL;
  int zl_rows;
};

enum { NIF_LOSS_MSE = 0, NIF_LOSS_MAE = 1, NIF_LOSS_HUBER = 2, NIF_LOSS_LOGCOSH = 3 };
__device__ __forceinline__ void nif_loss_vd(int kind, float e, float* v, float* d) {
  if (kind == NIF_LOSS_MAE) { *v = fabsf(e); *d = e > 0.f ? 1.0f : (e < 0.f ? -1.0f : 0.0f); }
  else if (kind == NIF_LOSS_HUBER) {
    const float a = fabsf(e);
    *v = a <= 1.0f ? 0.5f * e * e : a - 0.5f;
    *d = a <= 1.0f ? e : (e > 0.f ? 1.0f : -1.0f);
  } else {
    const float t = -2.0f * e;
    *v = e + (fmaxf(t, 0.f) + log1pf(expf(-fabsf(t)))) - 0.69314718055994531f;
    *d = tanhf(e);
  }
}
#define NIF_LOSS_ACC(KIND_, E_, SE_, DFAC_)                                   \
  float DFAC_;                                                                \
  if ((KIND_) == NIF_LOSS_MSE) { SE_ = fmaf(E_, E_, SE_); DFAC_ = 2.0f * (E_); } \
  else { float v_; nif_loss_vd(KIND_, E_, &v_, &DFAC_); SE_ += v_; }

struct SNetArgs {
  int loss_kind;
  const float* theta;
  const float* xin; int ncol; int col0;
  long B;
  int si, so, n, nh, r; long po;
  int act, res, nif_skip; float omega;
  long off_Wh, off_bh;
  const float* Z;
  const f32x4* WF; const f32x4* WB;
  float* stash; long slot_stride;
  float* DU;
  float* DZ;
  const float* y; const float* sw;
  float* u_out;
  float* loss_partial;
  float inv_bg;
  float* dring;
  int nsm;
  long long* tl;
  const void* WF4; const void* WB4;
  const void* WF4h; const void* WB4h;
  const void* WF4x; const void* WB4x;
  const float* wscale;
  int ll, rl, so_u;
  const void* WPF; const void* WPB;
  float* DPHI;
  float* DA_ll;
  float* DZL;
  int prec;
  int da_bf16;
  int h_ph16;
  int wg_cap;
};
struct LLSlotSeg { long src, dst, len; };
struct LLSlotMap { int nseg; LLSlotSeg seg[48]; };
void launch_ll_slots(const float* theta, const LLSlotMap& m, float* slots, hipStream_t st);
long snet4_phi_fwd_elems(int n);
long snet4_phi_bwd_elems(int n);
void launch_pack_phi(const float* theta, long w_off, int n, int sop, void* WPF, void* WPB, hipStream_t st);
__host__ __device__ inline long slot_w1(const SNetArgs& a) { return 0; }
__host__ __device__ inline long slot_wh(const SNetArgs& a, int j) { return (long)a.si * a.n + (long)j * a.n * a.n; }
__host__ __device__ inline long slot_wl(const SNetArgs& a) { return (long)a.si * a.n + (long)a.nh * a.n * a.n; }
__host__ __device__ inline long slot_b1(const SNetArgs& a) { return slot_wl(a) + (long)a.n * a.so; }
__host__ __device__ inline long slot_bh(const SNetArgs& a, int j) { return slot_b1(a) + a.n + (long)j * a.n; }
__host__ __device__ inline long slot_bl(const SNetArgs& a) { return slot_b1(a) + a.n + (long)a.nh * a.n; }

__host__ __device__ inline int stash_fp(int n) { return n <= 32 ? 32 : (n <= 64 ? 64 : 128); }

struct GwArgs {
  const float* IN;
  const float* DA;
  const float* SM;
  const float* xin; int ncol; int col0; int nd;
  int nc;
  const float* Z; int r;
  long ntiles; long B;
  float scale;
  MatRef W;
  MatRef Bv;
  float* partial; long pstride;
  int has_bias;
  long zt_mod, bias_ntiles;
  int seed[3];
  int in_ph16;
  int da_bf16;
};
bool gw_da_bf16_ok(int NBI, int NBO, int r);
bool sobw_supported(const SNetArgs& a, int ns, bool any_par);

void launch_pack(const float* theta, const MatRef& m, int NBI, int NBO, f32x4* WF, f32x4* WB, hipStream_t st);
void launch_pnet(const PNetArgs& a, int NSTB, bool train, hipStream_t st);
void launch_pnet_bwd(const PNetArgs& a, int NSTB, hipStream_t st);
void launch_snet(const SNetArgs& a, int NB, bool train, hipStream_t st);
int launch_snet3(const SNetArgs& a, bool train, bool query_only, int* waves_out, hipStream_t st);
bool pnet_bwg_supported(const PNetArgs& a);
void launch_pnet_bwg(const PNetArgs& a, float* partial, long pstride, int rows, hipStream_t st, const float* touch = nullptr,
                     long touch_floats = 0);
bool snet4_supported(const SNetArgs& a);
long snet4_fwd_elems(int n, int r);
long snet4_bwd_elems(int n, int r);
void launch_pack16b(const float* theta, const MatRef& m, int NBL, void* WF, void* WB, float scale, hipStream_t st, int mode = 0);
void launch_pack16b_dual(const float* theta, const MatRef& m0, long mstride, int nmat, int NBL, void* WF, void* WB, long fstride_elems,
                         long bstride_elems, void* WFx, void* WBx, long fxstride_elems, long bxstride_elems, float scale, float* pscale,
                         hipStream_t st);
void launch_snet4_f16(const SNetArgs& a, bool train, int nblk, size_t shm, hipStream_t st);
void launch_snet4_x16(const SNetArgs& a, bool train, int nblk, size_t shm, hipStream_t st);
void launch_pack16b_batch(const float* theta, const MatRef& m0, long mstride, int nmat, int NBL, void* WF, void* WB,
                          long fstride_elems, long bstride_elems, float scale, hipStream_t st, int mode = 0, float* pscale = nullptr);
int launch_snet4(const SNetArgs& a, bool train, bool query_only, hipStream_t st);
#define NIF_SMALL_MAX_B 2048
bool small_supported(const PNetArgs& p, const SNetArgs& s);
int small_rows(long B);
void small_tables(const PNetArgs& p, const SNetArgs& s, std::vector<int>& idx, std::vector<int>& desc);
void launch_small(const PNetArgs& p, const SNetArgs& s, float* partial, long pstride, long P, const int* idx_dev, const int* desc_dev,
                  double* metric, float metric_w, const float* g_loss, hipStream_t st);
bool snet4_writes_h_ph16(const SNetArgs& a);
bool gw_in_ph16_ok(int NBI, int NBO, int r);
bool snet4_writes_da_bf16(const SNetArgs& a);
bool sob_writes_da_bf16(const SNetArgs& a, int ns, bool any_par);
bool snet6_supported(const SNetArgs& a);
int snet6_rows(const SNetArgs& a);
long snet6_ring_floats(long B, int nh);
int launch_snet6(const SNetArgs& a, float* partial, long pstride, hipStream_t st);
int snet4_nsm_ll(int si, int sop, int nh, int n, int sou, int rl);
long sob_ring_floats_per_wave(int n, int nh);
bool sob_ll_supported(const SNetArgs& a);
struct SobPar {
  int par[3]; int gcol[3]; const float* ZT; float* DZT;
  int npar; int parc[3]; int pcol[3]; float* DAT; float* ZTL; int zl_rows;
  int gstride, nx_all, ny, no_primal; unsigned ymask;
  int hess;
};
int launch_sob(const SNetArgs& a, bool train, int ns, const int* seeds, const float* gt, float wj, float* ring, float* ju,
               bool query_only, hipStream_t st, const SobPar* par = nullptr);
bool snet3_supported(const SNetArgs& a);
int snet3_nbl(int n);
int snet3_nsm(int si, int so, int nh, int n);
long snet3_plane_floats(int n);
long snet3_ring_floats_per_wave(int n, int nh);
bool jac_supported(const SNetArgs& a);
void launch_jac(const SNetArgs& a, int ns, const int* seeds, const float* const* zd, int nx_total, int x0, float* dydx,
                hipStream_t st);
void launch_hess(const SNetArgs& a, int seed_j, int seed_k, int hj, int hk, int nx_total, float* dydx, float* d2ydx2, hipStream_t st,
                 const float* zd_j = nullptr, const float* zd_k = nullptr, const float* zdd = nullptr);
void launch_mlp_jac(const PNetArgs& a, int NB, int seed, float* ZD, hipStream_t st);
void launch_ll_jac_out(const float* PHI, const float* Z, const float* PHID, const float* ZD, long B, int r, int so,
                       int nx_total, int xcol, float* dydx, hipStream_t st);
void launch_pack16(const float* theta, const MatRef& m, int NBL, f32x4* WF, f32x4* WB, hipStream_t st);
int launch_gw_mfma(const GwArgs& a, int NBI, int NBO, int rows, hipStream_t st);
void launch_gw_first(const GwArgs& a, int NBO, int rows, hipStream_t st);
void launch_gw_out(const GwArgs& a, int NBI, int rows, hipStream_t st);
void launch_reduce(const float* partial, long pstride, int rows, const float* loss_partial, int nloss,
                   float* g, long P, hipStream_t st);
void launch_reg(const float* theta, float* g, long lo, long hi, long P, float l1, float l2, hipStream_t st);
void launch_metric(const float* g, long P, float weight, double* acc, hipStream_t st);
enum { OPT_ADAM = 0, OPT_LION = 1, OPT_ADABELIEF = 2, OPT_SGD = 3, OPT_RMSPROP = 4, OPT_ADAGRAD = 5, OPT_ADAMAX = 6, OPT_ADAMW = 7 };
enum { OPT_RECTIFY = 1, OPT_AMSGRAD = 2, OPT_NESTEROV = 4, OPT_CENTERED = 8, OPT_DECOUPLED_WD = 16 };
enum { SCHED_NONE = 0, SCHED_EXPONENTIAL = 1, SCHED_INVERSE_TIME = 2, SCHED_COSINE = 3, SCHED_POLYNOMIAL = 4, SCHED_KIND_MASK = 0xff,
       SCHED_STAIRCASE = 0x100, SCHED_CYCLE = 0x200 };
struct OptDev {
  int kind, flags; float lr, beta1, beta2, eps, wd, decay, sma_threshold, warmup_proportion, min_lr; long total_steps; long step;
  int sched, decay_steps; float sched_a, sched_b;
};
struct OptScalars { double lr, bc1, bc2, r; int div; };
__host__ __device__ inline int kernel_kind(int kind, int flags) { return kind == OPT_ADAM && (flags & OPT_DECOUPLED_WD) ? OPT_ADAMW : kind; }
__host__ __device__ inline bool third_slot(int kind, int flags) {
  return ((kind == OPT_ADAM || kind == OPT_ADABELIEF) && (flags & OPT_AMSGRAD)) || (kind == OPT_RMSPROP && (flags & OPT_CENTERED));
}
__host__ __device__ inline double sched_lr(const OptDev& o, double lr, double step) {
  const int k = o.sched & SCHED_KIND_MASK;
  const double ds = (double)o.decay_steps, a = (double)o.sched_a, b = (double)o.sched_b;
  if (k == SCHED_EXPONENTIAL || k == SCHED_INVERSE_TIME) {
    double p = step / ds;
    if (o.sched & SCHED_STAIRCASE) p = floor(p);
    return k == SCHED_EXPONENTIAL ? lr * pow(a, p) : lr / (1.0 + a * p);
  }
  if (k == SCHED_COSINE) {
    const double q = fmin(step, ds) / ds;
    return lr * ((1.0 - a) * 0.5 * (1.0 + cos(3.14159265358979323846 * q)) + a);
  }
  if (k == SCHED_POLYNOMIAL) {
    const double dsc = (o.sched & SCHED_CYCLE) ? ds * fmax(1.0, ceil(step / ds)) : ds;
    const double q = fmin(step, dsc) / dsc;
    return (lr - a) * pow(1.0 - q, b) + a;
  }
  return lr;
}
__host__ __device__ inline OptScalars opt_scalars(const OptDev& o, long t_) {
  OptScalars s;
  const double t = (double)t_;
  double lr = (double)o.lr;
  if (o.decay != 0.f) lr = lr / (1.0 + (double)o.decay * (t - 1.0));
  if (o.sched) lr = sched_lr(o, lr, t - 1.0);
  const double b2 = (double)o.beta2, b2t = pow(b2, t);
  s.bc1 = 1.0 - pow((double)o.beta1, t);
  s.bc2 = 1.0 - b2t;
  s.r = 1.0; s.div = 1;
  if (o.kind == OPT_ADABELIEF) {
    if (o.total_steps > 0) {
      const double ts = (double)o.total_steps, w = ts * (double)o.warmup_proportion;
      const double ds = fmax(ts - w, 1.0), rate = ((double)o.min_lr - lr) / ds;
      lr = t <= w ? lr * (t / w) : lr + rate * fmin(t - w, ds);
    }
    if (o.flags & OPT_RECTIFY) {
      const double sma_inf = 2.0 / (1.0 - b2) - 1.0;
      const double sma_t = sma_inf - 2.0 * t * b2t / (1.0 - b2t);
      if (sma_t >= (double)o.sma_threshold)
        s.r = sqrt((sma_t - 4.0) / (sma_inf - 4.0) * (sma_t - 2.0) / (sma_inf - 2.0) * sma_inf / sma_t);
      else
        s.div = 0;
    }
  }
  s.lr = lr;
  return s;
}
struct OptArgs { float lr, b1, b2, eps, wd, bc1, bc2, r; int div; float lr0; };
__host__ __device__ inline OptArgs opt_args(const OptDev& o, const OptScalars& s) {
  OptArgs a;
  a.lr = (float)(o.kind == OPT_ADAM ? s.lr * sqrt(s.bc2) / s.bc1 : o.kind == OPT_ADAMAX ? s.lr / s.bc1 : s.lr);
  a.b1 = o.beta1; a.b2 = o.beta2; a.eps = o.eps; a.wd = o.wd;
  a.bc1 = (float)s.bc1; a.bc2 = (float)s.bc2; a.r = (float)s.r; a.div = s.div;
  if (o.kind == OPT_SGD) a.div = o.beta1 != 0.f ? ((o.flags & OPT_NESTEROV) ? 2 : 1) : 0;
  if (o.kind == OPT_RMSPROP) a.div = o.beta1 > 0.f ? 1 : 0;
  a.lr0 = (float)s.lr;
  return a;
}
void launch_opt(int kind, bool ams, float* theta, const float* g, float* m, float* v, float* vhat, long P, const OptArgs& a,
                hipStream_t st);
void launch_reduce_opt(int kind, bool ams, const float* partial, long pstride, int rows, const float* loss_partial, int nloss, float* g,
                       long P, float* theta, float* m, float* v, float* vhat, const OptArgs& a, hipStream_t st);
void launch_opt_dev(int kind, bool ams, float* theta, const float* g, float* m, float* v, float* vhat, long P, OptDev* od,
                    hipStream_t st);
enum { GT_CENTRALIZE = 1, GT_GTCF = 2 };
#define GT_VEC_CHUNK 4096
struct GtDev { int flags; float clipnorm, clipvalue, global_clipnorm; };
struct GtBlk { long base, lim; int stride, rows, nc, tensor, matrix, pb0, pbn, pad; };
void launch_gt_reduce(float* g, const GtBlk* blks, int nblk, float* part, const GtDev* gd, hipStream_t st);
void launch_gt_apply(float* g, const GtBlk* blks, int nblk, int ntensor, const float* part, float* norms, const GtDev* gd, bool write,
                     hipStream_t st);
#define PRUNE_CHUNK 4096
#define PRUNE_BINS 2048
struct PruneSeg { long off, size, k, blk0; };
struct PruneSel { unsigned prefix, krem; };
void launch_prune_update(const float* theta, const PruneSeg* segs, int nseg, long nblk, unsigned* hist, PruneSel* sel, float* thr,
                         unsigned char* mask, hipStream_t st);
void launch_prune_apply(float* theta, const unsigned char* mask, long lo, long hi, long P, hipStream_t st);
void launch_latent_to_w(const float* theta, long off_Wh, long off_bh, int r, long po, const float* lr, long B,
                        float* w, hipStream_t st);
void launch_given_w(const float* x, const float* w, float* u, long B, int si, int so, int n, int nh, long po,
                    int act, int res, int nif_skip, float omega, hipStream_t st);
struct LLArgs {
  int loss_kind;
  const float* theta; long bias_off; long last_w;
  const float* PHI;
  const float* Z;
  long B; int r, so;
  const float* y; const float* sw; float inv_bg;
// ... 287 lines not shown
```

Measured before the change: 938.5 million.

## Fuse hypernet weight packing into pnet forward launch and pipeline pnet bwd first layer

```diff
diff --git a/nif_amd/csrc/k_nets.hip b/nif_amd/csrc/k_nets.hip
--- a/nif_amd/csrc/k_nets.hip
+++ b/nif_amd/csrc/k_nets.hip
@@ -1,5 +1,6 @@
 #include "nif_internal.h"
 #include "k_pnet_bf16.h"
+#include "k_pack16_dev.h"
 
 
 __global__ void k_pack(const float* __restrict__ theta, MatRef m, int NBI, int NBO, float* __restrict__ WF,
@@ -60,7 +61,12 @@
 __host__ __device__ inline int pnet_tail_floats(const PNetArgs& A) { return A.r + (A.ll_kind ? A.r + A.r * A.r : 0); }
 
 template <int NB, bool TRAIN, int ACT>
-__global__ __launch_bounds__(256) void k_pnet(PNetArgs A) {
+__global__ __launch_bounds__(256) void k_pnet(PNetArgs A, PackDualArgs K) {
+  if ((int)blockIdx.x < K.blk0) {
+    pack16b_dual_body(K, (int)blockIdx.x % K.gx, (int)blockIdx.x / K.gx);
+    return;
+  }
+  const int nblk = (int)gridDim.x - K.blk0, bid = (int)blockIdx.x - K.blk0;
   const int lane = threadIdx.x & 63, wid = threadIdx.x >> 6;
   const int p = lane & 31, hf = lane >> 5;
   const long ntiles = (A.B + 31) / 32;
@@ -90,7 +96,7 @@
       }
   }
   __syncthreads();
-  for (long tile = (long)blockIdx.x * 4 + wid; tile < ntiles; tile += (long)gridDim.x * 4) {
+  for (long tile = (long)bid * 4 + wid; tile < ntiles; tile += (long)nblk * 4) {
   long pt = tile * 32 + p;
   const long ptc = pt < A.B ? pt : A.B - 1;
 
@@ -241,7 +247,7 @@
   stash_store<NB>(da0, tile, ga, p, hf);
 }
 
-void launch_pnet(const PNetArgs& a_, int NSTB, bool train, hipStream_t st) {
+void launch_pnet(const PNetArgs& a_, int NSTB, bool train, hipStream_t st, const PackDualArgs* pack) {
   PNetArgs a = a_;
   const long ntiles = (a.B + 31) / 32;
   long nblk = (ntiles + 3) / 4;
@@ -253,13 +259,20 @@
   const size_t tailb = (size_t)pnet_tail_floats(a) * sizeof(float);
   a.pbf2 = (NSTB == 2 && bf2_on && shm0 + tailb + (size_t)nmat * 4 * PBF_FWD_U4 * 16 <= 64u * 1024u) ? 1 : 0;
   if (a.pbf2 && nblk > 512) nblk = 512;
-  dim3 grid((unsigned)nblk), block(256);
+  PackDualArgs pk{};
+  if (pack && pack->gx > 0) {
+    pk = *pack;
+    const int cap = (256 + pk.nmat - 1) / pk.nmat;
+    if (pk.gx > cap) pk.gx = cap;
+    pk.blk0 = pk.gx * pk.nmat;
+  }
+  dim3 grid((unsigned)(nblk + pk.blk0)), block(256);
   const size_t shm = shm0 + (size_t)pnet_plane_floats(a, NSTB) * sizeof(float) + tailb;
 #define PNL(NB_, TR_, ACT_)                                                                                             \
   {                                                                                                                     \
     if (shm > 48 * 1024)                                                                                                \
       (void)hipFuncSetAttribute((const void*)k_pnet<NB_, TR_, ACT_>, hipFuncAttributeMaxDynamicSharedMemorySize, (int)shm); \
-    hipLaunchKernelGGL((k_pnet<NB_, TR_, ACT_>), grid, block, shm, st, a);                                              \
+    hipLaunchKernelGGL((k_pnet<NB_, TR_, ACT_>), grid, block, shm, st, a, pk);                                          \
   }
 #define PNA(NB_, TR_)                              \
   if (a.act == ACT_SWISH) PNL(NB_, TR_, ACT_SWISH) \
diff --git a/nif_amd/csrc/k_pack16_dev.h b/nif_amd/csrc/k_pack16_dev.h
--- /dev/null
+++ b/nif_amd/csrc/k_pack16_dev.h
@@ -0,0 +1,79 @@
+#pragma once
+#include "nif_internal.h"
+
+__device__ __forceinline__ void pack16b_dual_body(const PackDualArgs& K, int bx, int by) {
+  MatRef m = K.m;
+  const float* __restrict__ theta = K.theta;
+  const long mstride = K.mstride;
+  const int NBL = K.NBL;
+  __bf16* __restrict__ WF = (__bf16*)K.WF; __bf16* __restrict__ WB = (__bf16*)K.WB;
+  _Float16* __restrict__ WFx = (_Float16*)K.WFx; _Float16* __restrict__ WBx = (_Float16*)K.WBx;
+  const long fstride = K.fstride, bstride = K.bstride, fxstride = K.fxstride, bxstride = K.bxstride;
+  const float scale = K.scale;
+  float* __restrict__ pscale = K.pscale;
+  m.base_k += (long)by * mstride; m.base_last += (long)by * mstride;
+  WF += (long)by * fstride; WB += (long)by * bstride;
+  WFx += (long)by * fxstride; WBx += (long)by * bxstride;
+  const int NCH = NBL / 2;
+  const long fwd0 = (long)NCH * NBL * 3 * 64 * 8, bwd0 = (long)NCH * NBL * 2 * 64 * 8, px = bwd0;
+  const long tot0 = (fwd0 + bwd0) * (m.r + 1), totx = 2 * px * (m.r + 1);
+  __shared__ float red[256];
+  int k_have = -1;
+  float s_have = 1.0f;
+  for (long idx = (long)bx * 256 + threadIdx.x; idx < tot0 + totx; idx += (long)K.gx * 256) {
+    const bool half = idx >= tot0;
+    const long i2 = half ? idx - tot0 : idx;
+    const long tf = half ? px * (m.r + 1) : fwd0 * (m.r + 1);
+    const bool fwd = i2 < tf;
+    const long e = fwd ? i2 : i2 - tf;
+    const int ns = half ? 2 : (fwd ? 3 : 2);
+    const long per_plane = half ? px : (fwd ? fwd0 : bwd0);
+    const int k = (int)(e / per_plane);
+    long rem = e - (long)k * per_plane;
+    const int t = rem & 7; rem >>= 3;
+    const int lane = rem & 63; rem >>= 6;
+    const int s = (int)(rem % ns); rem /= ns;
+    const int blk = (int)(rem % NBL);
+    const int ks = (int)(rem / NBL);
+    const int slot = 16 * (2 * ks + (t >> 2)) + 4 * (lane >> 4) + (t & 3);
+    const int row = 16 * blk + (lane & 15);
+    const int in = fwd ? slot : row, out = fwd ? row : slot;
+    float x = (in < m.nin && out < m.nout) ? scale * theta[matref_index(m, k, in, out)] : 0.f;
+    if (half) {
+      if (k != k_have) {
+        float mx = 0.f;
+        for (int q = threadIdx.x; q < m.nin * m.nout; q += 256) {
+          const int qi = q / m.nout, qo = q - qi * m.nout;
+          mx = fmaxf(mx, fabsf(scale * theta[matref_index(m, k, qi, qo)]));
+        }
+        __syncthreads();
+        red[threadIdx.x] = mx;
+        __syncthreads();
+        for (int o = 128; o > 0; o >>= 1) {
+          if ((int)threadIdx.x < o) red[threadIdx.x] = fmaxf(red[threadIdx.x], red[threadIdx.x + o]);
+          __syncthreads();
+        }
+        mx = red[0];
+        int ex = 0;
+        if (mx > 0.f && mx < 3.0e38f) (void)frexpf(mx, &ex); else ex = 14;
+        int sh = 14 - ex;
+        sh = sh > 60 ? 60 : (sh < -60 ? -60 : sh);
+        s_have = ldexpf(1.0f, sh); k_have = k;
+        if (fwd && e == (long)k * per_plane && pscale) {
+          pscale[(by * (m.r + 1) + k) * 2] = s_have;
+          pscale[(by * (m.r + 1) + k) * 2 + 1] = ldexpf(1.0f, -sh);
+        }
+      }
+      x *= s_have;
+      const _Float16 h0 = (_Float16)__builtin_amdgcn_fmed3f(x, -65504.0f, 65504.0f);
+      const _Float16 h1 = (_Float16)(x - (float)h0);
+      (fwd ? WFx : WBx)[e] = s == 0 ? h0 : h1;
+      continue;
+    }
+    const __bf16 x0 = (__bf16)x;
+    const float r1 = x - (float)x0;
+    const __bf16 x1 = (__bf16)r1;
+    const __bf16 x2 = (__bf16)(r1 - (float)x1);
+    (fwd ? WF : WB)[e] = s == 0 ? x0 : (s == 1 ? x1 : x2);
+  }
+}
diff --git a/nif_amd/csrc/k_pnetbw.hip b/nif_amd/csrc/k_pnetbw.hip
--- a/nif_amd/csrc/k_pnetbw.hip
+++ b/nif_amd/csrc/k_pnetbw.hip
@@ -91,10 +91,43 @@
   auto dense_b = [&](int m, const f32x16 (&x)[1], f32x16 (&y)[1]) { pbf_dense_bwd(bpl + m * (PBF_FWD_U4 + PBF_BWD_U4) + PBF_FWD_U4, x[0], y[0], lane); };
   __syncthreads();
 
-  for (long tile = (long)blockIdx.x * WV + wid; tile < ntiles; tile += (long)gridDim.x * WV) {
+  constexpr bool PIPE = SMALL && ACT == ACT_SWISH;
+  const long tstride = (long)gridDim.x * WV;
+  float* park = hs + NM * 1024;
+  float x_c = 0.f, dz_c = 0.f;
+  f32x16 h_c;
+  auto first_layer = [&](float x, f32x16 (&hh)[1], f32x16 (&dd)[1]) {
+    f32x16 acc;
+#pragma unroll
+    for (int v = 0; v < 16; ++v) acc[v] = 0.f;
+    acc += x * psmall_get(S.fw, 0, hf);
+    hh[0] = A.omega * acc + psmall_get(S.fb, 0, hf);
+    act_tile_sel<1, ACT>(A.act, hh, hh, dd, A.nst, hf);
+  };
+  if (PIPE) {
+    const long t0 = (long)blockIdx.x * WV + wid;
+    if (t0 < ntiles) {
+      const long pt0 = t0 * 32 + p;
+      x_c = A.xin[(pt0 < A.B ? pt0 : A.B - 1) * A.ncol + A.col0];
+      dz_c = A.DZ[t0 * 32 + p];
+      f32x16 h0[1], d0[1];
+      first_layer(x_c, h0, d0);
+      h_c = h0[0];
+#pragma unroll
+      for (int v = 0; v < 16; ++v) park[v * 64 + lane] = d0[0][v];
+    }
+  }
+  for (long tile = (long)blockIdx.x * WV + wid; tile < ntiles; tile += tstride) {
     const long pt = tile * 32 + p;
     const long ptc = pt < A.B ? pt : A.B - 1;
     const float* prow = A.xin + ptc * A.ncol + A.col0;
+    float x_n = 0.f, dz_n = 0.f;
+    if (PIPE) {
+      const long tn = tile + tstride < ntiles ? tile + tstride : tile;
+      const long ptn = tn * 32 + p;
+      x_n = A.xin[(ptn < A.B ? ptn : A.B - 1) * A.ncol + A.col0];
+      dz_n = A.DZ[tn * 32 + p];
+    }
     float dzr[NIF_PBW_DZR];
     if (!SMALL) {
       const float* dzg = A.DZ + tile * A.r * 32;
@@ -103,18 +136,19 @@
       for (int q = 0; q < NIF_PBW_DZR; ++q) { const int e = lane + 64 * q; dzr[q] = e < nd ? dzg[e] : 0.f; }
     }
     f32x16 h[1], T[1], d[NM + 1][1];
-    {
+    if (PIPE) {
+      h[0] = h_c;
+    } else {
       f32x16 acc;
 #pragma unroll
       for (int v = 0; v < 16; ++v) acc[v] = 0.f;
       for (int dd = 0; dd < A.pi; ++dd) acc += prow[dd] * psmall_get(S.fw + dd * 32, 0, hf);
       h[0] = A.omega * acc + psmall_get(S.fb, 0, hf);
-    }
-    act_tile_sel<1, ACT>(A.act, h, h, d[0], A.nst, hf);
-    float* park = hs + NM * 1024;
-    if (SMALL) {
-#pragma unroll
-      for (int v = 0; v < 16; ++v) park[v * 64 + lane] = d[0][0][v];
+      act_tile_sel<1, ACT>(A.act, h, h, d[0], A.nst, hf);
+      if (SMALL) {
+#pragma unroll
+        for (int v = 0; v < 16; ++v) park[v * 64 + lane] = d[0][0][v];
+      }
     }
     if (!SMALL && hf == 0) {
       for (int dd = 0; dd < A.pi; ++dd) xT[pswz(dd, p)] = prow[dd];
@@ -158,10 +192,10 @@
       }
       for (int c = 0; c < A.r; ++c) gh[0] += gaT[pswz(c, p)] * psmall_get(S.bw + c * 32, 0, hf);
     } else {
-      gh[0] += A.DZ[tile * 32 + p] * psmall_get(S.bw, 0, hf);
+      gh[0] += (PIPE ? dz_c : A.DZ[tile * 32 + p]) * psmall_get(S.bw, 0, hf);
     }
     if (SMALL) {
-      const float dz = A.DZ[tile * 32 + p];
+      const float dz = PIPE ? dz_c : A.DZ[tile * 32 + p];
       Cb += dz * h[0];
       gbb += hf == 0 ? dz : 0.f;
     } else {
@@ -200,16 +234,25 @@
       dense_b(0, ga, U);
       gh[0] = skip + A.omega * U[0];
     }
-    if (SMALL) {
+    if (PIPE) {
+      f32x16 hn[1], dn[1];
+      first_layer(x_n, hn, dn);
 #pragma unroll
       for (int v = 0; v < 16; ++v) ga[0][v] = gh[0][v] * park[v * 64 + lane];
-    } else {
-      ga[0] = gh[0] * d[0][0];
-    }
-    if (SMALL) {
+#pragma unroll
+      for (int v = 0; v < 16; ++v) park[v * 64 + lane] = dn[0][v];
+      C1 += x_c * ga[0];
+      CB1 += ga[0];
+      h_c = hn[0]; x_c = x_n; dz_c = dz_n;
+    } else if (SMALL) {
+#pragma unroll
+      for (int v = 0; v < 16; ++v) ga[0][v] = gh[0][v] * park[v * 64 + lane];
       C1 += prow[0] * ga[0];
       CB1 += ga[0];
     } else {
+      ga[0] = gh[0] * d[0][0];
+    }
+    if (!SMALL) {
       tile_store(gaT, ga[0], p, hf);
       grad_mfma(xT, gaT, C1, i, hf, 8);
     }
diff --git a/nif_amd/csrc/k_snet4.hip b/nif_amd/csrc/k_snet4.hip
--- a/nif_amd/csrc/k_snet4.hip
+++ b/nif_amd/csrc/k_snet4.hip
@@ -1,4 +1,5 @@
 #include "k_snet4_dev.h"
+#include "k_pack16_dev.h"
 
 __global__ void k_pack16b(const float* __restrict__ theta, MatRef m, long mstride, int NBL, __bf16* __restrict__ WF,
                           __bf16* __restrict__ WB, long fstride, long bstride, float scale, int mode, const float* __restrict__ pscale) {
@@ -67,84 +68,26 @@
     pscale[(blockIdx.y * (m.r + 1) + k) * 2 + 1] = ldexpf(1.0f, -sh);
   }
 }
-__global__ __launch_bounds__(256) void k_pack16b_dual(const float* __restrict__ theta, MatRef m, long mstride, int NBL,
-                                                     __bf16* __restrict__ WF, __bf16* __restrict__ WB, long fstride, long bstride,
-                                                     _Float16* __restrict__ WFx, _Float16* __restrict__ WBx, long fxstride, long bxstride,
-                                                     float scale, float* __restrict__ pscale) {
-  m.base_k += (long)blockIdx.y * mstride; m.base_last += (long)blockIdx.y * mstride;
-  WF += (long)blockIdx.y * fstride; WB += (long)blockIdx.y * bstride;
-  WFx += (long)blockIdx.y * fxstride; WBx += (long)blockIdx.y * bxstride;
-  const int NCH = NBL / 2;
-  const long fwd0 = (long)NCH * NBL * 3 * 64 * 8, bwd0 = (long)NCH * NBL * 2 * 64 * 8, px = bwd0;
-  const long tot0 = (fwd0 + bwd0) * (m.r + 1), totx = 2 * px * (m.r + 1);
-  __shared__ float red[256];
-  int k_have = -1;
-  float s_have = 1.0f;
-  for (long idx = (long)blockIdx.x * blockDim.x + threadIdx.x; idx < tot0 + totx; idx += (long)gridDim.x * blockDim.x) {
-    const bool half = idx >= tot0;
-    const long i2 = half ? idx - tot0 : idx;
-    const long tf = half ? px * (m.r + 1) : fwd0 * (m.r + 1);
-    const bool fwd = i2 < tf;
-    const long e = fwd ? i2 : i2 - tf;
-    const int ns = half ? 2 : (fwd ? 3 : 2);
-    const long per_plane = half ? px : (fwd ? fwd0 : bwd0);
-    const int k = (int)(e / per_plane);
-    long rem = e - (long)k * per_plane;
-    const int t = rem & 7; rem >>= 3;
-    const int lane = rem & 63; rem >>= 6;
-    const int s = (int)(rem % ns); rem /= ns;
-    const int blk = (int)(rem % NBL);
-    const int ks = (int)(rem / NBL);
-    const int slot = 16 * (2 * ks + (t >> 2)) + 4 * (lane >> 4) + (t & 3);
-    const int row = 16 * blk + (lane & 15);
-    const int in = fwd ? slot : row, out = fwd ? row : slot;
-    float x = (in < m.nin && out < m.nout) ? scale * theta[matref_index(m, k, in, out)] : 0.f;
-    if (half) {
-      if (k != k_have) {
-        float mx = 0.f;
-        for (int q = threadIdx.x; q < m.nin * m.nout; q += 256) {
-          const int qi = q / m.nout, qo = q - qi * m.nout;
-          mx = fmaxf(mx, fabsf(scale * theta[matref_index(m, k, qi, qo)]));
-        }
-        __syncthreads();
-        red[threadIdx.x] = mx;
-        __syncthreads();
-        for (int o = 128; o > 0; o >>= 1) {
-          if ((int)threadIdx.x < o) red[threadIdx.x] = fmaxf(red[threadIdx.x], red[threadIdx.x + o]);
-          __syncthreads();
-        }
-        mx = red[0];
-        int ex = 0;
-        if (mx > 0.f && mx < 3.0e38f) (void)frexpf(mx, &ex); else ex = 14;
-        int sh = 14 - ex;
-        sh = sh > 60 ? 60 : (sh < -60 ? -60 : sh);
-        s_have = ldexpf(1.0f, sh); k_have = k;
-        if (fwd && e == (long)k * per_plane && pscale) {
-          pscale[(blockIdx.y * (m.r + 1) + k) * 2] = s_have;
-          pscale[(blockIdx.y * (m.r + 1) + k) * 2 + 1] = ldexpf(1.0f, -sh);
-        }
-      }
-      x *= s_have;
-      const _Float16 h0 = (_Float16)__builtin_amdgcn_fmed3f(x, -65504.0f, 65504.0f);
-      const _Float16 h1 = (_Float16)(x - (float)h0);
-      (fwd ? WFx : WBx)[e] = s == 0 ? h0 : h1;
-      continue;
-    }
-    const __bf16 x0 = (__bf16)x;
-    const float r1 = x - (float)x0;
-    const __bf16 x1 = (__bf16)r1;
-    const __bf16 x2 = (__bf16)(r1 - (float)x1);
-    (fwd ? WF : WB)[e] = s == 0 ? x0 : (s == 1 ? x1 : x2);
-  }
+__global__ __launch_bounds__(256) void k_pack16b_dual(PackDualArgs K) { pack16b_dual_body(K, blockIdx.x, blockIdx.y); }
+PackDualArgs pack16b_dual_args(const float* theta, const MatRef& m0, long mstride, int nmat, int NBL, void* WF, void* WB, long fstride_elems,
+                               long bstride_elems, void* WFx, void* WBx, long fxstride_elems, long bxstride_elems, float scale, float* pscale) {
+  const long total = (long)(NBL / 2) * NBL * (5 + 4) * 64 * 8 * (m0.r + 1);
+  int grid = (int)((total + 255) / 256);
+  if (grid > 4096) grid = 4096;
+  PackDualArgs K;
+  K.theta = theta; K.m = m0; K.mstride = mstride; K.NBL = NBL; K.WF = WF; K.WB = WB; K.fstride = fstride_elems; K.bstride = bstride_elems;
+  K.WFx = WFx; K.WBx = WBx; K.fxstride = fxstride_elems; K.bxstride = bxstride_elems; K.scale = scale; K.pscale = pscale;
+  K.gx = grid; K.nmat = nmat; K.blk0 = 0;
+  return K;
+}
+void launch_pack16b_dual(const PackDualArgs& K, hipStream_t st) {
+  hipLaunchKernelGGL(k_pack16b_dual, dim3(K.gx, K.nmat), dim3(256), 0, st, K);
 }
 void launch_pack16b_dual(const float* theta, const MatRef& m0, long mstride, int nmat, int NBL, void* WF, void* WB, long fstride_elems,
                          long bstride_elems, void* WFx, void* WBx, long fxstride_elems, long bxstride_elems, float scale, float* pscale,
                          hipStream_t st) {
-  const long total = (long)(NBL / 2) * NBL * (5 + 4) * 64 * 8 * (m0.r + 1);
-  int grid = (int)((total + 255) / 256);
-  if (grid > 4096) grid = 4096;
-  hipLaunchKernelGGL(k_pack16b_dual, dim3(grid, nmat), dim3(256), 0, st, theta, m0, mstride, NBL, (__bf16*)WF, (__bf16*)WB, fstride_elems,
-                     bstride_elems, (_Float16*)WFx, (_Float16*)WBx, fxstride_elems, bxstride_elems, scale, pscale);
+  launch_pack16b_dual(pack16b_dual_args(theta, m0, mstride, nmat, NBL, WF, WB, fstride_elems, bstride_elems, WFx, WBx, fxstride_elems,
+                                        bxstride_elems, scale, pscale), st);
 }
 void launch_pack16b(const float* theta, const MatRef& m, int NBL, void* WF, void* WB, float scale, hipStream_t st, int mode) {
   launch_pack16b_batch(theta, m, 0, 1, NBL, WF, WB, 0, 0, scale, st, mode);
diff --git a/nif_amd/csrc/nif_api.hip b/nif_amd/csrc/nif_api.hip
--- a/nif_amd/csrc/nif_api.hip
+++ b/nif_amd/csrc/nif_api.hip
@@ -175,6 +175,7 @@
   c->cfg = *cfg;
   { const char* e = getenv("NIF_FP32_MFMA"); c->opt_fp32_mfma = e && e[0] == '1'; }
   { const char* e = getenv("NIF_FUSE_GW"); c->opt_fuse_gw = !(e && e[0] == '0'); }
+  { const char* e = getenv("NIF_FUSE_PACK"); c->opt_fuse_pack = !(e && e[0] == '0'); }
   { const char* e = getenv("NIF_SMALL_STEP"); c->opt_small_step = !(e && e[0] == '0'); }
   { const char* e = getenv("NIF_FUSE_TAIL"); c->opt_fuse_tail = !(e && e[0] == '0'); }
   { const char* e = getenv("NIF_PIPE_CHUNK"); if (e && e[0]) c->opt_pipe_chunk = atol(e); }
@@ -544,8 +545,26 @@
   c->packed_p32 = true;
   return NIF_OK;
 }
-static int ensure_packed(nif_ctx* c) {
+static PackDualArgs hyper_pack_dual_args(nif_ctx* c, float omega) {
+  return pack16b_dual_args(c->theta, hyper_w(c, 1), hyper_wslot(c, 2) - hyper_wslot(c, 1), c->nh, snet3_nbl(c->n), c->sWF4, c->sWB4,
+                           snet4_fwd_elems(c->n, c->r), snet4_bwd_elems(c->n, c->r), c->sWF4x, c->sWB4x, snet4_bwd_elems(c->n, c->r),
+                           snet4_bwd_elems(c->n, c->r), omega, c->sWscale);
+}
+static int pack_flush(nif_ctx* c) {
+  if (!c->pack_pending) return NIF_OK;
+  c->pack_pending = false;
+  ProfScope ps_(c, NIF_PROF_PACK);
+  SNetArgs probe; fill_snet(c, probe, nullptr, 0, 0, 32);
+  launch_pack16b_dual(hyper_pack_dual_args(c, probe.omega), c->st);
+  HIPCHK(hipGetLastError());
+  return NIF_OK;
+}
+static int ensure_packed(nif_ctx* c, bool may_defer = false) {
   if (!c->have_params) return fail(NIF_ERR_STATE, "parameters not set (call nif_set_params first)");
+  if (c->pack_pending) {
+    if (!c->packed) c->pack_pending = false;
+    else if (!may_defer) { const int rcf = pack_flush(c); if (rcf) return rcf; }
+  }
   if (c->packed) return NIF_OK;
   c->packed_p32 = false;
   if (c->NSTB > 1) { const int rcp = ensure_packed_p32(c); if (rcp) return rcp; }
@@ -599,11 +618,10 @@
   const bool fp32_only = c->opt_fp32_mfma;
   c->use_snet4 = c->sWF4 && !fp32_only && snet4_supported(probe);
   c->packed32 = false;
-  if (c->use_snet4 && c->nh > 0 && c->sWF4x)
-    launch_pack16b_dual(c->theta, hyper_w(c, 1), hyper_wslot(c, 2) - hyper_wslot(c, 1), c->nh, snet3_nbl(c->n),
-                        c->sWF4, c->sWB4, snet4_fwd_elems(c->n, c->r), snet4_bwd_elems(c->n, c->r),
-                        c->sWF4x, c->sWB4x, snet4_bwd_elems(c->n, c->r), snet4_bwd_elems(c->n, c->r), probe.omega, c->sWscale, c->st);
-  else if (c->use_snet4 && c->nh > 0)
+  if (c->use_snet4 && c->nh > 0 && c->sWF4x) {
+    if (may_defer && c->opt_fuse_pack && !c->capturing) c->pack_pending = true;
+    else launch_pack16b_dual(hyper_pack_dual_args(c, probe.omega), c->st);
+  } else if (c->use_snet4 && c->nh > 0)
     launch_pack16b_batch(c->theta, hyper_w(c, 1), hyper_wslot(c, 2) - hyper_wslot(c, 1), c->nh, snet3_nbl(c->n),
                          c->sWF4, c->sWB4, snet4_fwd_elems(c->n, c->r), snet4_bwd_elems(c->n, c->r), probe.omega, c->st);
   if (c->use_snet4 && c->nh > 0 && c->sWF4h)
@@ -1254,7 +1272,6 @@
   if (pa.stash) pa.stash += t0 * 32 * 32 * c->NSTB;
   const bool fused_p = !pnet_force_stash() && pnet_bwg_supported(pa);
   if (!fused_p) { const int rcp = ensure_packed_p32(c); if (rcp) return rcp; }
-  { ProfScope p_(c, NIF_PROF_PNET_FWD, sa_st); launch_pnet(pa, c->NSTB, !fused_p, sa_st); }
   SNetArgs sa; fill_snet(c, sa, xin, ncol, c->pi, B);
   sa.Z = pa.Z; sa.DZ = pa.DZ; sa.DU = c->DU + t0 * 32 * c->so;
   sa.stash = c->stash_s + t0 * 32 * 32 * c->NB;
@@ -1266,6 +1283,13 @@
                         snet6_rows(sa) == rows_for(c, ntiles);
   if (fused_gw) nloss = snet6_rows(sa);
   *nloss_out = nloss;
+  {
+    PackDualArgs pk{};
+    if (c->pack_pending && fused_gw && sa_st == c->st) { pk = hyper_pack_dual_args(c, sa.omega); c->pack_pending = false; }
+    else { rc = pack_flush(c); if (rc) return rc; }
+    ProfScope p_(c, NIF_PROF_PNET_FWD, sa_st);
+    launch_pnet(pa, c->NSTB, !fused_p, sa_st, pk.gx > 0 ? &pk : nullptr);
+  }
   {
     const int nbl = snet3_nbl(c->n);
     bool dab = sa.prec == 1 && (nbl == 2 || nbl == 4 || nbl == 8) && gw_da_bf16_ok(c->NB, c->NB, c->r);
@@ -1394,7 +1418,7 @@
     }
   }
   int rc = nif_metric_flush(c); if (rc) return rc;
-  rc = ensure_packed(c); if (rc) return rc;
+  rc = ensure_packed(c, ns == 0 && !sp); if (rc) return rc;
   const long ntiles = (B + 31) / 32;
   if (ns > 0) { rc = ensure_packed32(c); if (rc) return rc; }
   if (ns > 0) {
@@ -2261,6 +2285,7 @@
 
 extern "C" int nif_set_option(nif_ctx* c, const char* key, int32_t value) {
   if (!c || !key) return fail(NIF_ERR_INVALID, "null");
+  if (strcmp(key, "fuse_pack") == 0) { c->opt_fuse_pack = value != 0; return NIF_OK; }
   if (strcmp(key, "fuse_gw") == 0) { c->opt_fuse_gw = value != 0; return NIF_OK; }
   if (strcmp(key, "fuse_tail") == 0) { c->opt_fuse_tail = value != 0; return NIF_OK; }
   if (strcmp(key, "small_step") == 0) { c->opt_small_step = value != 0; return NIF_OK; }
diff --git a/nif_amd/csrc/nif_ctx.h b/nif_amd/csrc/nif_ctx.h
--- a/nif_amd/csrc/nif_ctx.h
+++ b/nif_amd/csrc/nif_ctx.h
@@ -123,6 +123,7 @@
   bool tail_pending = false; int tail_rows = 0, tail_nloss = 0; bool opt_fuse_tail = true;
   bool opt_small_step = true;
   bool opt_fuse_gw = true;
+  bool opt_fuse_pack = true; bool pack_pending = false;
   nif_ctx() = default;
   nif_ctx(const nif_ctx&) = delete;
   ~nif_ctx();
diff --git a/nif_amd/csrc/nif_internal.h b/nif_amd/csrc/nif_internal.h
--- a/nif_amd/csrc/nif_internal.h
+++ b/nif_amd/csrc/nif_internal.h
@@ -132,8 +132,16 @@
 bool gw_da_bf16_ok(int NBI, int NBO, int r);
 bool sobw_supported(const SNetArgs& a, int ns, bool any_par);
 
+struct PackDualArgs {
+  const float* theta; MatRef m; long mstride; int NBL;
+  void* WF; void* WB; long fstride, bstride;
+  void* WFx; void* WBx; long fxstride, bxstride;
+  float scale; float* pscale;
+  int gx, nmat, blk0;
+};
+
 void launch_pack(const float* theta, const MatRef& m, int NBI, int NBO, f32x4* WF, f32x4* WB, hipStream_t st);
-void launch_pnet(const PNetArgs& a, int NSTB, bool train, hipStream_t st);
+void launch_pnet(const PNetArgs& a, int NSTB, bool train, hipStream_t st, const PackDualArgs* pack = nullptr);
 void launch_pnet_bwd(const PNetArgs& a, int NSTB, hipStream_t st);
 void launch_snet(const SNetArgs& a, int NB, bool train, hipStream_t st);
 int launch_snet3(const SNetArgs& a, bool train, bool query_only, int* waves_out, hipStream_t st);
@@ -147,6 +155,9 @@
 void launch_pack16b_dual(const float* theta, const MatRef& m0, long mstride, int nmat, int NBL, void* WF, void* WB, long fstride_elems,
                          long bstride_elems, void* WFx, void* WBx, long fxstride_elems, long bxstride_elems, float scale, float* pscale,
                          hipStream_t st);
+PackDualArgs pack16b_dual_args(const float* theta, const MatRef& m0, long mstride, int nmat, int NBL, void* WF, void* WB, long fstride_elems,
+                               long bstride_elems, void* WFx, void* WBx, long fxstride_elems, long bxstride_elems, float scale, float* pscale);
+void launch_pack16b_dual(const PackDualArgs& K, hipStream_t st);
 void launch_snet4_f16(const SNetArgs& a, bool train, int nblk, size_t shm, hipStream_t st);
 void launch_snet4_x16(const SNetArgs& a, bool train, int nblk, size_t shm, hipStream_t st);
 void launch_pack16b_batch(const float* theta, const MatRef& m0, long mstride, int nmat, int NBL, void* WF, void* WB,
```

Result: no change. 944.1 million, median of 6 (+0.6%).
